# PraveenVora/pinot

Hardware: AMD Instinct MI355X
Metric: rows/sec scanned + %HBM roofline, filter+GROUP BY SUM at 1/2/4/8 GPUs (higher is better)
Workload: dtype int64; 1 GPU; adanalytics_readme_query; rows_per_gpu=1000000000, segments_per_gpu=100, parallelism=segment-sharded dp1, RCCL reduce of partial aggregates, groups=8, matched_docs_rank0=118

## Files before the change

include/pinot_amd.h:

```cpp
#ifndef PINOT_AMD_H_
#define PINOT_AMD_H_

#include <stdint.h>

#ifdef __cplusplus
extern "C" {
#endif

#define PA_ABI_VERSION 5

#define PA_MAX_LEAVES 16
#define PA_MAX_OPS 48
#define PA_MAX_GROUP_BY 8
#define PA_MAX_AGGS 16

#define PA_OK 0
#define PA_EINVAL (-1)
#define PA_EHIP (-2)
#define PA_ENOMEM (-3)
#define PA_EUNSUPPORTED (-4)

#define PA_INT 0
#define PA_LONG 1
#define PA_FLOAT 2
// ... 75 lines not shown
  int64_t group_by_cardinality[PA_MAX_GROUP_BY];
  int32_t num_aggs;
  pa_agg_spec aggs[PA_MAX_AGGS];
  int32_t flags;
  int32_t num_groups_limit;
  int64_t hash_keys_bound;
  int32_t flags2;
  int32_t reserved2;
} pa_query_spec;

#define PA_QF_STAGE_ALL 1
#define PA_QF_FORCE_GLOBAL 2
#define PA_QF_STEPS16 (1 << 4)
#define PA_QF_STEPS32 (1 << 5)
#define PA_QF_NO_LAZY (1 << 6)
#define PA_QF_FORCE_LDS (1 << 7)
#define PA_QF_RING_SHIFT 8
#define PA_QF_WG_SHIFT 12
#define PA_QF_NO_GDENSE_LM (1 << 15)
#define PA_QF_NO_JIT (1u << 31)
#define PA_QF_GD_DRAIN_EACH_TILE (1 << 2)
#define PA_QF_NO_GD_PACK (1 << 3)
#define PA_QF_DEBUG_STREAM_ONLY (1 << 16)
#define PA_QF_NO_LANE_MAJOR (1 << 17)
#define PA_QF_NO_REG_STAGE (1 << 18)
#define PA_QF_NO_BOX_FILTER (1 << 19)
#define PA_QF_BOX_FILTER (1 << 20)
#define PA_QF_NO_PARTITION (1 << 21)
#define PA_QF_NO_SPLIT_EMIT (1 << 24)
#define PA_QF_NO_LIMIT_WALK (1 << 25)
#define PA_QF_NO_LANE_ACC (1 << 26)
#define PA_QF_NO_LANE_HIST (1 << 27)
#define PA_QF_LAZY_POST (1 << 28)
#define PA_QF_NO_DENSE_GROUP (1 << 29)
#define PA_QF_NO_FILTER_STATS (1 << 30)
#define PA_QF2_NO_COUNT_FREE 1
#define PA_QF_PART_SHIFT 22

typedef struct {
  int32_t lo, hi;
  int32_t negate;
  int32_t reserved;
  const uint32_t* lut;
  int64_t ilo, ihi;
  double dlo, dhi;
  const void* values;
  int64_t num_values;
} pa_leaf_params;

typedef struct pa_query pa_query;

pa_query* pa_query_create(const pa_query_spec* spec, int32_t num_segments);

int pa_query_bind_segment(pa_query* q, int32_t index, const pa_segment* seg,
                          const pa_leaf_params* leaf_params, const int32_t* const* group_remaps);

int pa_query_bind_value_remap(pa_query* q, int32_t index, int32_t agg, const int32_t* remap);

int pa_query_set_tuning(pa_query* q, const char* name, int32_t value);
int32_t pa_query_results_invalid(const pa_query* q);

int pa_query_prepare(pa_query* q);

int64_t pa_query_num_keys(const pa_query* q);

int pa_query_execute(pa_query* q, void* stream);
int pa_query_reset(pa_query* q, void* stream);
int pa_query_scan(pa_query* q, void* stream);

#define PA_ACC_COUNT_U64 0
#define PA_ACC_SUM_I64 1
#define PA_ACC_SUM_F64 2
#define PA_ACC_MIN_I64 3
#define PA_ACC_MAX_I64 4
#define PA_ACC_HLL_U8 5
#define PA_ACC_SUM_I64X2 6
#define PA_ACC_DOCS_U64 7
#define PA_ACC_KEYS_I64 8
#define PA_ACC_PRESENCE_U8 9
#define PA_ACC_HIST_U64 10
uint64_t pa_query_accumulator_bytes(const pa_query* q);
int pa_query_set_accumulator_buffer(pa_query* q, void* device_buffer, uint64_t bytes);
int32_t pa_query_num_sections(const pa_query* q);
void* pa_query_section(const pa_query* q, int32_t section, int32_t* kind, int64_t* num_elements);

int64_t pa_query_fetch(pa_query* q, void* stream, int64_t capacity, int64_t* out_keys,
                       int64_t* out_counts, void* const* out_aggs);

int64_t pa_query_fetch_histogram(pa_query* q, void* stream, int32_t agg, int64_t num_groups, int64_t capacity,
                                 int64_t* out_row_ends, int32_t* out_value_ids, int64_t* out_value_counts);

#define PA_MAX_PERCENTILES 64
int pa_query_percentiles(pa_query* q, void* stream, int32_t agg, int64_t num_groups, int32_t num_percentiles,
                         const double* percentiles, int32_t* out_value_ids);

int64_t pa_query_matched_docs(const pa_query* q);

int32_t pa_query_limit_trimming(const pa_query* q);
int64_t pa_query_num_groups_limit_reached(const pa_query* q);

int64_t pa_query_leaf_bitmap_words(const pa_query* q, int32_t segment);
int pa_query_leaf_bitmaps(pa_query* q, int32_t segment, uint32_t* device_out, void* stream);

#define PA_BIT_AND (-1)
#define PA_BIT_OR (-2)
#define PA_BIT_NOT (-3)
#define PA_BIT_PROG_MAX 64
int64_t pa_bitmap_counts_scratch_bytes(int64_t words);
int pa_bitmap_counts(const uint32_t* device_bitmaps, int64_t words, int32_t num_leaves, int64_t num_docs,
                     const int32_t* prog_a, int32_t len_a, const int32_t* prog_b, int32_t len_b, void* device_scratch,
                     int64_t* device_out, void* stream);
int pa_query_filter_counts(pa_query* q, int32_t num_requests, const int32_t* segments, const int32_t* programs,
                           const int32_t* lengths, int64_t* out, void* stream);
int32_t pa_query_leap_leaf(const pa_query* q);
int pa_query_leap_counts(pa_query* q, int64_t* out, void* stream);

#define PA_FOP_EMPTY 0
#define PA_FOP_MATCH_ALL 1
#define PA_FOP_SORTED 2
#define PA_FOP_BITMAP 3
#define PA_FOP_SCAN 4
#define PA_FOP_AND 5
#define PA_FOP_OR 6
#define PA_FOP_NOT 7
#define PA_STATS_NON_SCAN (-1)
#define PA_STATS_HOST (-2)
typedef struct {
  int32_t kind;
  int32_t num_children;
  int32_t mv_column;
  int32_t prog_len;
  int32_t prog[PA_BIT_PROG_MAX];
} pa_filter_op;
int pa_query_execution_stats(pa_query* q, int32_t num_ops, const pa_filter_op* ops, int32_t num_trees,
                             const int32_t* tree_root, const int32_t* segment_tree, int32_t projected_columns,
                             int64_t docs_scanned, int64_t* out, int64_t* segment_in_filter, void* stream);

int64_t pa_query_row_bytes(const pa_query* q);
int pa_query_pack_rows(pa_query* q, int32_t world, void* device_rows, int64_t* counts, void* stream);
int pa_query_merge_rows(pa_query* q, const void* device_rows, int64_t num_rows, int64_t* groups, int64_t* overflow,
                        void* stream);

int pa_query_key_layout(const pa_query* q, int32_t* hashed, int32_t* shifts);
int32_t pa_query_key_words(const pa_query* q);

int pa_query_stats(const pa_query* q, uint64_t* staged_bytes, uint64_t* num_docs,
                   uint64_t* num_tiles);

int32_t pa_query_column_staged(const pa_query* q, int32_t column_id);
int32_t pa_query_num_eager_literals(const pa_query* q);
int32_t pa_query_lane_major(const pa_query* q);
int32_t pa_query_dense_packed(const pa_query* q);
int32_t pa_query_count_free_emit(const pa_query* q);
int32_t pa_query_partition_keys(const pa_query* q);
int pa_query_plan(const pa_query* q, int32_t* strategy, int32_t* steps, int32_t* dma_slots, int32_t* ring,
                  int32_t* wg_per_cu, int32_t* grid, int32_t* lds_bytes);

void pa_query_destroy(pa_query* q);

#ifdef __cplusplus
}
#endif

#endif
```

pinot_amd/_lib.py:

```python
import ctypes
import os

HERE = os.path.dirname(os.path.abspath(__file__))
LIB_PATH = os.path.join(HERE, "libpinot_amd.so")

PA_MAX_LEAVES = 16
PA_MAX_OPS = 48
PA_MAX_GROUP_BY = 8
PA_MAX_AGGS = 16

PA_INT, PA_LONG, PA_FLOAT, PA_DOUBLE, PA_STRING, PA_BYTES = range(6)
PA_LEAF_DICT_RANGE, PA_LEAF_DICT_SET, PA_LEAF_RAW_RANGE, PA_LEAF_MV_DICT_RANGE, PA_LEAF_MV_DICT_SET, PA_LEAF_RAW_SET = range(6)
PA_OP_LEAF, PA_OP_AND, PA_OP_OR, PA_OP_NOT = range(4)
PA_AGG_COUNT, PA_AGG_SUM, PA_AGG_MIN, PA_AGG_MAX, PA_AGG_DISTINCTCOUNTHLL, PA_AGG_COUNT_MV, PA_AGG_DISTINCTCOUNT, \
    PA_AGG_VALUE_HISTOGRAM = range(8)
PA_QF_STAGE_ALL = 1
PA_QF_FORCE_GLOBAL = 2
PA_QF_STEPS16 = 1 << 4
PA_QF_STEPS32 = 1 << 5
PA_QF_NO_LAZY = 1 << 6
PA_QF_FORCE_LDS = 1 << 7
PA_QF_RING_SHIFT = 8
PA_QF_WG_SHIFT = 12
PA_QF_DEBUG_STREAM_ONLY = 1 << 16
PA_QF_NO_LANE_MAJOR = 1 << 17
PA_QF_NO_REG_STAGE = 1 << 18
PA_QF_NO_GDENSE_LM = 1 << 15
PA_QF_NO_GD_PACK = 1 << 3
PA_QF_GD_DRAIN_EACH_TILE = 1 << 2
PA_QF_NO_JIT = 1 << 31
PA_QF_NO_BOX_FILTER = 1 << 19
PA_QF_BOX_FILTER = 1 << 20
PA_QF_NO_PARTITION = 1 << 21
PA_QF_PART_SHIFT = 22
PA_QF_NO_SPLIT_EMIT = 1 << 24
PA_QF_NO_LIMIT_WALK = 1 << 25
PA_QF_NO_LANE_ACC = 1 << 26
PA_QF_NO_LANE_HIST = 1 << 27
PA_QF_LAZY_POST = 1 << 28
PA_QF_NO_DENSE_GROUP = 1 << 29
PA_QF_NO_FILTER_STATS = 1 << 30
PA_QF2_NO_COUNT_FREE = 1 << 32
PA_FOP_EMPTY, PA_FOP_MATCH_ALL, PA_FOP_SORTED, PA_FOP_BITMAP, PA_FOP_SCAN, PA_FOP_AND, PA_FOP_OR, PA_FOP_NOT = range(8)
PA_STATS_NON_SCAN, PA_STATS_HOST = -1, -2
PA_BIT_AND, PA_BIT_OR, PA_BIT_NOT = -1, -2, -3
PA_BIT_PROG_MAX = 64
PA_ACC_COUNT_U64, PA_ACC_SUM_I64, PA_ACC_SUM_F64, PA_ACC_MIN_I64, PA_ACC_MAX_I64, PA_ACC_HLL_U8, \
    PA_ACC_SUM_I64X2, PA_ACC_DOCS_U64, PA_ACC_KEYS_I64, PA_ACC_PRESENCE_U8, PA_ACC_HIST_U64 = range(11)
PA_MAX_PERCENTILES = 64
ABI_VERSION = 5

EXPORTED = [
    "pa_abi_version", "pa_device_count", "pa_set_device", "pa_last_error", "pa_host_alloc", "pa_host_free",
    "pa_segment_create", "pa_segment_add_sv_dict_column", "pa_segment_add_mv_dict_column",
    "pa_segment_add_raw_column", "pa_segment_num_docs", "pa_segment_device_bytes", "pa_segment_destroy",
    "pa_query_create", "pa_query_set_tuning", "pa_query_results_invalid", "pa_query_bind_segment",
    "pa_query_bind_value_remap", "pa_query_prepare", "pa_query_num_keys",
    "pa_query_execute", "pa_query_reset", "pa_query_scan", "pa_query_num_eager_literals", "pa_query_lane_major",
    "pa_query_dense_packed", "pa_query_count_free_emit", "pa_query_partition_keys",
    "pa_query_accumulator_bytes", "pa_query_set_accumulator_buffer", "pa_query_num_sections", "pa_query_section",
    "pa_query_fetch", "pa_query_fetch_histogram", "pa_query_percentiles", "pa_query_matched_docs", "pa_query_key_layout", "pa_query_limit_trimming",
    "pa_query_num_groups_limit_reached", "pa_query_stats", "pa_query_leaf_bitmap_words", "pa_query_leaf_bitmaps",
    "pa_bitmap_counts_scratch_bytes", "pa_bitmap_counts", "pa_query_filter_counts",
    "pa_query_plan", "pa_query_column_staged", "pa_query_leap_leaf", "pa_query_leap_counts",
    "pa_query_execution_stats",
    "pa_query_row_bytes", "pa_query_pack_rows", "pa_query_merge_rows", "pa_query_key_words", "pa_query_destroy",
]


class PinotAmdError(RuntimeError):
    pass


class LeafSpec(ctypes.Structure):
    _fields_ = [("column_id", ctypes.c_int32), ("kind", ctypes.c_int32)]


class AggSpec(ctypes.Structure):
    _fields_ = [("type", ctypes.c_int32), ("column_id", ctypes.c_int32), ("log2m", ctypes.c_int32),
                ("flags", ctypes.c_int32), ("num_values", ctypes.c_int64)]


PA_AGGF_WIDE_SUM = 1


class QuerySpec(ctypes.Structure):
    _fields_ = [
        ("num_leaves", ctypes.c_int32),
        ("leaves", LeafSpec * PA_MAX_LEAVES),
        ("num_ops", ctypes.c_int32),
        ("ops", ctypes.c_int32 * PA_MAX_OPS),
        ("num_group_by", ctypes.c_int32),
        ("group_by_columns", ctypes.c_int32 * PA_MAX_GROUP_BY),
        ("group_by_cardinality", ctypes.c_int64 * PA_MAX_GROUP_BY),
        ("num_aggs", ctypes.c_int32),
        ("aggs", AggSpec * PA_MAX_AGGS),
        ("flags", ctypes.c_int32),
        ("num_groups_limit", ctypes.c_int32),
        ("hash_keys_bound", ctypes.c_int64),
        ("flags2", ctypes.c_int32),
        ("reserved2", ctypes.c_int32),
    ]


class LeafParams(ctypes.Structure):
    _fields_ = [
        ("lo", ctypes.c_int32), ("hi", ctypes.c_int32), ("negate", ctypes.c_int32), ("reserved", ctypes.c_int32),
        ("lut", ctypes.POINTER(ctypes.c_uint32)),
        ("ilo", ctypes.c_int64), ("ihi", ctypes.c_int64),
        ("dlo", ctypes.c_double), ("dhi", ctypes.c_double),
        ("values", ctypes.c_void_p), ("num_values", ctypes.c_int64),
    ]


_lib = None


def _declare(lib):
    vp, i32, i64, u64 = ctypes.c_void_p, ctypes.c_int32, ctypes.c_int64, ctypes.c_uint64
    sig = {
        "pa_abi_version": (ctypes.c_int, []),
        "pa_device_count": (ctypes.c_int, []),
        "pa_set_device": (ctypes.c_int, [ctypes.c_int]),
        "pa_last_error": (ctypes.c_char_p, []),
        "pa_host_alloc": (vp, [u64]),
        "pa_host_free": (None, [vp]),
        "pa_segment_create": (vp, [i32]),
        "pa_segment_add_sv_dict_column": (ctypes.c_int, [vp, i32, vp, u64, i32, i32, i32, vp, vp]),
        "pa_segment_add_mv_dict_column": (ctypes.c_int, [vp, i32, vp, u64, i32, i32, i64, i32, vp, vp]),
        "pa_segment_add_raw_column": (ctypes.c_int, [vp, i32, i32, vp]),
        "pa_segment_num_docs": (i32, [vp]),
        "pa_segment_device_bytes": (u64, [vp]),
        "pa_segment_destroy": (None, [vp]),
        "pa_query_create": (vp, [ctypes.POINTER(QuerySpec), i32]),
        "pa_query_set_tuning": (ctypes.c_int, [vp, ctypes.c_char_p, i32]),
        "pa_query_results_invalid": (i32, [vp]),
        "pa_query_bind_segment": (ctypes.c_int, [vp, i32, vp, ctypes.POINTER(LeafParams), vp]),
        "pa_query_bind_value_remap": (ctypes.c_int, [vp, i32, i32, vp]),
        "pa_query_prepare": (ctypes.c_int, [vp]),
        "pa_query_num_keys": (i64, [vp]),
        "pa_query_execute": (ctypes.c_int, [vp, vp]),
        "pa_query_reset": (ctypes.c_int, [vp, vp]),
        "pa_query_scan": (ctypes.c_int, [vp, vp]),
        "pa_query_num_eager_literals": (i32, [vp]),
        "pa_query_lane_major": (i32, [vp]),
        "pa_query_dense_packed": (i32, [vp]),
        "pa_query_count_free_emit": (i32, [vp]),
        "pa_query_partition_keys": (i32, [vp]),
        "pa_query_accumulator_bytes": (u64, [vp]),
        "pa_query_set_accumulator_buffer": (ctypes.c_int, [vp, vp, u64]),
        "pa_query_num_sections": (i32, [vp]),
        "pa_query_section": (vp, [vp, i32, ctypes.POINTER(i32), ctypes.POINTER(i64)]),
        "pa_query_fetch": (i64, [vp, vp, i64, vp, vp, vp]),
        "pa_query_fetch_histogram": (i64, [vp, vp, i32, i64, i64, vp, vp, vp]),
        "pa_query_percentiles": (ctypes.c_int, [vp, vp, i32, i64, i32, vp, vp]),
        "pa_query_matched_docs": (i64, [vp]),
        "pa_query_key_layout": (ctypes.c_int, [vp, ctypes.POINTER(i32), ctypes.POINTER(i32)]),
        "pa_query_limit_trimming": (i32, [vp]),
        "pa_query_num_groups_limit_reached": (ctypes.c_int64, [vp]),
        "pa_query_stats": (ctypes.c_int, [vp, ctypes.POINTER(u64), ctypes.POINTER(u64), ctypes.POINTER(u64)]),
        "pa_query_leaf_bitmap_words": (ctypes.c_int64, [vp, i32]),
        "pa_query_leaf_bitmaps": (ctypes.c_int, [vp, i32, vp, vp]),
        "pa_bitmap_counts_scratch_bytes": (i64, [i64]),
        "pa_bitmap_counts": (ctypes.c_int, [vp, i64, i32, i64, vp, i32, vp, i32, vp, vp, vp]),
        "pa_query_filter_counts": (ctypes.c_int, [vp, i32, vp, vp, vp, vp, vp]),
        "pa_query_plan": (ctypes.c_int, [vp] + [ctypes.POINTER(i32)] * 7),
        "pa_query_column_staged": (i32, [vp, i32]),
        "pa_query_leap_leaf": (i32, [vp]),
        "pa_query_leap_counts": (ctypes.c_int, [vp, vp, vp]),
        "pa_query_execution_stats": (ctypes.c_int, [vp, i32, vp, i32, vp, vp, i32, i64, vp, vp, vp]),
        "pa_query_row_bytes": (i64, [vp]),
        "pa_query_key_words": (i32, [vp]),
        "pa_query_pack_rows": (ctypes.c_int, [vp, i32, vp, vp, vp]),
        "pa_query_merge_rows": (ctypes.c_int, [vp, vp, i64, vp, vp, vp]),
        "pa_query_destroy": (None, [vp]),
    }
    for name, (res, args) in sig.items():
        f = getattr(lib, name)
        f.restype = res
        f.argtypes = args


def lib():
    global _lib
    if _lib is None:
        if not os.path.exists(LIB_PATH):
            raise PinotAmdError("%s is missing: run `python -m pinot_amd.build` (hipcc, gfx950)" % LIB_PATH)
        _lib = ctypes.CDLL(LIB_PATH)
        _declare(_lib)
        if _lib.pa_abi_version() != ABI_VERSION:
            raise PinotAmdError("ABI version mismatch: %s is stale, rebuild it" % LIB_PATH)
    return _lib


def check(rc, what=""):
    if rc < 0:
        raise PinotAmdError("%s failed (%d): %s" % (what, rc, lib().pa_last_error().decode(errors="replace")))
    return rc


def check_ptr(p, what=""):
    if not p:
        raise PinotAmdError("%s failed: %s" % (what, lib().pa_last_error().decode(errors="replace")))
    return p
```

pinot_amd/csrc/pa_capi.hip:

```cpp
#include "pa_host.h"

extern "C" {

pa_query* pa_query_create(const pa_query_spec* spec, int32_t num_segments) {
  if (!spec || num_segments < 0) {
    fail(PA_EINVAL, "bad query spec");
    return nullptr;
  }
  if (spec->num_leaves < 0 || spec->num_leaves > PA_MAX_LEAVES || spec->num_ops < 0 || spec->num_ops > PA_MAX_OPS ||
      spec->num_group_by < 0 || spec->num_group_by > PA_MAX_GROUP_BY || spec->num_aggs < 0 ||
      spec->num_aggs > PA_MAX_AGGS) {
    fail(PA_EINVAL, "query spec counts out of range");
    return nullptr;
  }
  pa_query* q = new pa_query();
  q->spec = *spec;
  q->nseg = num_segments;
  q->segs.assign(num_segments, nullptr);
  q->leaf_params.resize(num_segments);
  q->luts.resize(num_segments);
  q->remaps.resize(num_segments);
  q->has_remap.resize(num_segments);
  q->vremaps.assign(num_segments, std::vector<std::vector<int32_t>>(spec->num_aggs));
  return q;
}

int pa_query_set_tuning(pa_query* q, const char* name, int32_t value) {
  if (!q) return fail(PA_EINVAL, "null query");
  if (q->prepared) return fail(PA_EINVAL, "query already prepared");
  const TuningDef* d = tuning_named(name);
  if (!d) return fail(PA_EINVAL, std::string("unknown tuning: ") + (name ? name : "(null)"));
  if (value != d->def && (value < d->lo || value > d->hi))
    return fail(PA_EINVAL, std::string("tuning ") + d->name + ": " + std::to_string(value) + " outside " +
                               std::to_string(d->lo) + ".." + std::to_string(d->hi));
  q->tune.*d->value = value;
  return PA_OK;
}

int32_t pa_query_results_invalid(const pa_query* q) { return q ? (tuning_invalidating(q->tune) ? 1 : 0) : -1; }

int pa_query_bind_segment(pa_query* q, int32_t index, const pa_segment* seg, const pa_leaf_params* leaf_params,
                          const int32_t* const* group_remaps) {
  if (!q || !seg || index < 0 || index >= q->nseg) return fail(PA_EINVAL, "bad bind arguments");
  if (q->prepared) return fail(PA_EINVAL, "query already prepared");
  const pa_query_spec& s = q->spec;
  q->segs[index] = seg;
  q->leaf_params[index].assign(leaf_params, leaf_params + s.num_leaves);
  q->luts[index].assign(s.num_leaves, {});
  for (int l = 0; l < s.num_leaves; ++l) {
    const int kind = s.leaves[l].kind;
    if (kind == PA_LEAF_DICT_SET || kind == PA_LEAF_MV_DICT_SET) {
      auto it = seg->cols.find(s.leaves[l].column_id);
      if (it == seg->cols.end()) return fail(PA_EINVAL, "leaf column missing in segment");
      if (!leaf_params[l].lut) return fail(PA_EINVAL, "DICT_SET leaf without lut");
      const size_t words = ((size_t)it->second->cardinality + 31) / 32;
      q->luts[index][l].assign(leaf_params[l].lut, leaf_params[l].lut + words);
    } else if (kind == PA_LEAF_RAW_SET) {
      auto it = seg->cols.find(s.leaves[l].column_id);
      if (it == seg->cols.end()) return fail(PA_EINVAL, "leaf column missing in segment");
      const int64_t n = leaf_params[l].num_values;
      if (n < 0 || n > (int64_t(1) << 30) || (n > 0 && !leaf_params[l].values))
        return fail(PA_EINVAL, "RAW_SET leaf: bad value list");
      const bool integral = it->second->vtype == PA_INT || it->second->vtype == PA_LONG;
      const int64_t* vi = (const int64_t*)leaf_params[l].values;
      const double* vd = (const double*)leaf_params[l].values;
      for (int64_t i = 1; i < n; ++i)
        if (integral ? !(vi[i - 1] < vi[i]) : !(vd[i - 1] < vd[i]))
          return fail(PA_EINVAL, "RAW_SET leaf: values must be strictly ascending");
      const uint32_t* w = (const uint32_t*)leaf_params[l].values;
      q->luts[index][l].assign(w, w + 2 * n);
    }
  }
  q->remaps[index].assign(s.num_group_by, {});
  q->has_remap[index].assign(s.num_group_by, 0);
  for (int j = 0; j < s.num_group_by; ++j) {
    if (group_remaps && group_remaps[j]) {
      auto it = seg->cols.find(s.group_by_columns[j]);
      if (it == seg->cols.end()) return fail(PA_EINVAL, "group-by column missing in segment");
      const int32_t card = it->second->cardinality;
      q->remaps[index][j].assign(group_remaps[j], group_remaps[j] + card);
      for (int32_t v : q->remaps[index][j])
        if (v < 0 || v >= s.group_by_cardinality[j]) return fail(PA_EINVAL, "group remap id outside the key space");
      q->has_remap[index][j] = 1;
    }
  }
  return PA_OK;
}

int pa_query_bind_value_remap(pa_query* q, int32_t index, int32_t agg, const int32_t* remap) {
  if (!q || index < 0 || index >= q->nseg || agg < 0 || agg >= q->spec.num_aggs) return fail(PA_EINVAL, "bad remap arguments");
  if (q->prepared) return fail(PA_EINVAL, "query already prepared");
  if (!q->segs[index]) return fail(PA_EINVAL, "bind the segment before its value remaps");
  const pa_agg_spec& A = q->spec.aggs[agg];
  if (!value_id_agg(A.type))
    return fail(PA_EINVAL, "value remaps belong to DISTINCTCOUNT and VALUE_HISTOGRAM aggregations");
  auto it = q->segs[index]->cols.find(A.column_id);
  if (it == q->segs[index]->cols.end()) return fail(PA_EINVAL, "aggregation column missing in segment");
  q->vremaps[index][agg].clear();
  if (!remap) return PA_OK;
  const int32_t card = it->second->cardinality;
  q->vremaps[index][agg].assign(remap, remap + card);
  for (int32_t v : q->vremaps[index][agg])
    if (v < 0 || v >= A.num_values) return fail(PA_EINVAL, "value remap id outside the table-wide value dictionary");
  return PA_OK;
}

int pa_query_prepare(pa_query* q) {
  if (!q) return fail(PA_EINVAL, "null query");
  if (q->prepared) return PA_OK;
  for (int i = 0; i < q->nseg; ++i)
    if (!q->segs[i]) return fail(PA_EINVAL, "segment " + std::to_string(i) + " not bound");
  Prep P;
  std::memset(&q->hq, 0, sizeof(q->hq));
  int rc = plan_filter(q, P);
  if (!rc) rc = plan_slots(q, P);
  if (!rc) rc = plan_key_space(q, P);
  if (!rc) rc = plan_limit(q, P);
  if (!rc) rc = plan_gdense(q, P);
  if (!rc) rc = build_segments(q, P);
  if (!rc) rc = plan_walk(q, P);
  if (!rc) rc = plan_accumulators(q, P);
  TilePlan plan, count_plan;
  if (!rc) rc = plan_kernels(q, P, plan, count_plan);
  if (rc) return rc;

  void* dummy = nullptr;
  {
    std::vector<char> z(256, 0);
    rc = upload_owned(q, z.data(), z.size(), &dummy);
    if (rc) return rc;
  }
  const int nslots = (int)q->slot_cols.size();
  int64_t total_tiles = 0;
  apply_layout(q->hsegs, plan.steps, nslots, (int)q->literals.size(), dummy, &q->staged_bytes, &total_tiles);
  q->num_tiles = (uint64_t)total_tiles;
  q->lane_major = P.lm ? 1 : 0;
  q->dense_packed = P.gd_packed ? 1 : 0;
  q->plan_ring = plan.ring;
  q->plan_wg = plan.wg_per_cu;
  fill_devquery(q, P, plan, total_tiles);
  rc = plan_leaps(q, P);
  if (rc) return rc;

  int dev = 0, cus = 256;
  if (hipGetDevice(&dev) == hipSuccess) {
    hipDeviceProp_t prop;
    if (hipGetDeviceProperties(&prop, dev) == hipSuccess && prop.multiProcessorCount > 0) cus = prop.multiProcessorCount;
  }
  const int wg_cu = q->split_emit ? std::min(plan.wg_per_cu, q->emit_h_wg) : plan.wg_per_cu;
  const int64_t max_wg = (int64_t)cus * std::max(1, wg_cu);
  const int wpw = q->partitioned ? scan_waves(q->emit_strat) : scan_waves(q->strategy);
  const int64_t want = (total_tiles + wpw - 1) / wpw;
  q->grid = (int)std::max<int64_t>(1, std::min(max_wg, want));

  if (q->partitioned) {
    int64_t ct = 0;
    apply_layout(q->hsegs_count, plan.steps, nslots, (int)q->literals.size(), dummy, nullptr, &ct);
    if (ct != total_tiles) return fail(PA_EINVAL, "internal: count pass tiles differ");
    DevQuery& c = q->hq_count;
    c = q->hq;
    c.strategy = q->count_strat;
    c.count_skip_gb = q->count_skip;
    c.image_dwords_max = count_plan.img_dw;
    c.ring = count_plan.ring;
    c.dma_per_tile = count_plan.dma;
    c.num_staged = 0;
    for (int sl = 0; sl < nslots; ++sl) {
      bool st = false;
      for (const DevSeg& d : q->hsegs_count) st |= d.cols[sl].lds_off >= 0;
      if (st) c.staged_slots[c.num_staged++] = sl;
    }
    c.lds_acc_bytes = (uint32_t)(((size_t)q->hq.num_parts * 4 + 15) & ~(size_t)15);
    q->count_lds = (int)count_plan.lds;
    q->count_ring = count_plan.ring;
    q->count_k = std::max(1, count_plan.wg_per_cu / std::max(1, wg_cu));
    while (q->count_k > 1 && (int64_t)q->grid * q->count_k * kWavesPerWG > total_tiles) --q->count_k;
    q->hq.lds_acc_bytes = (uint32_t)(plan.lds - (size_t)wpw * plan.ring * plan.img_dw * 4);
    if (q->split_emit) {
      DevQuery& e = q->hq_h;
      e = q->hq;
      e.strategy = STRAT_PEMIT;
      e.ring = q->emit_h_ring;
      e.lds_acc_bytes = (uint32_t)((size_t)q->emit_h_lds -
                                   (size_t)scan_waves(q->emit_h_strat) * q->emit_h_ring * plan.img_dw * 4);
      e.part_lo = q->hq.pv;
      e.part_hi = q->hq.num_parts;
    }
    rc = plan_scratch(q, P);
    if (rc) return rc;
  }
  if (q->limit_mode) {
    rc = plan_limit_buffers(q, P, cus, total_tiles);
    if (rc) return rc;
  }
  rc = alloc_leaps(q, P);
  if (rc) return rc;
  rc = upload_descriptors(q);
  if (rc) return rc;
  rc = jit_plan(q, P, cus);
  if (rc) return rc;
  rc = pve_plan(q, P, cus);
  if (rc) return rc;
  PA_HIP(hipDeviceSynchronize());
  q->prepared = true;
  return PA_OK;
}

int64_t pa_query_num_keys(const pa_query* q) { return q ? q->num_keys : -1; }

int pa_query_reset(pa_query* q, void* stream) {
  if (!q || !q->prepared) return fail(PA_EINVAL, "query not prepared");
  hipStream_t st = (hipStream_t)stream;
  PA_HIP(hipMemsetAsync(q->external_acc ? q->external_acc : q->acc.p, 0, q->acc.n, st));
  if (q->hq.leap_mode) PA_HIP(hipMemsetAsync(q->leap_buf.p, 0, leap_header_bytes(q), st));
  for (const Section& sc : q->sections) {
    if (sc.kind == PA_ACC_MIN_I64 || sc.kind == PA_ACC_KEYS_I64) PA_HIP(launch_fill_i64((int64_t*)sc.ptr, sc.n, INT64_MAX, st));
    else if (sc.kind == PA_ACC_MAX_I64) PA_HIP(launch_fill_i64((int64_t*)sc.ptr, sc.n, INT64_MIN, st));
  }
  return PA_OK;
}

int pa_query_scan(pa_query* q, void* stream) {
  if (!q || !q->prepared) return fail(PA_EINVAL, "query not prepared");
  q->scanned_since_fetch = true;
  if (q->num_tiles == 0) return PA_OK;
  hipStream_t st = (hipStream_t)stream;
  if (q->limit_walk) {
    if (q->walk_words > kWalkMaxWords) PA_HIP(hipMemsetAsync(q->lim_admit.p, 0, q->lim_admit.n, st));
    PA_HIP(launch_limit_walk((const DevQuery*)q->dq.p, (const DevSeg*)q->dsegs.p, q->nseg, q->walk_words,
                             q->hq.gb_mv >= 0, q->tune.walk_tab != 0, st));
  }
  if (q->limit_mode) {
    const DevQuery* dq = (const DevQuery*)q->dq.p;
    const DevSeg* ds = (const DevSeg*)q->dsegs.p;
    const LimitDesc& F = q->limit;
    const int64_t H = F.fmask + 1;
    PA_HIP(launch_fill_i64((int64_t*)F.fkeys, H, INT64_MAX, st));
    PA_HIP(launch_fill_i64((int64_t*)F.fpos, H, -1, st));
    PA_HIP(launch_fill_i64((int64_t*)F.thresh, std::max(1, q->nseg), -1, st));
    PA_HIP(launch_fill_i64((int64_t*)F.hist, std::max(1, q->nseg) * 128, 0, st));
    PA_HIP(launch_limit_passes(dq, ds, F, q->limit_grid, 0, st));
    PA_HIP(launch_limit_passes(dq, ds, F, q->limit_grid, 1, st));
    PA_HIP(launch_limit_passes(dq, ds, F, q->limit_grid, 2, st));
    return PA_OK;
  }
  if (q->pve.fn) {
    if (q->part_vk == kVkGeneric) return fail(PA_EINVAL, "internal: chunk lists need a specialised pass C");
    PartScratch ps{};
    char* vb = (char*)q->pve.buf.p;
    ps.base = (uint64_t*)(vb + q->pve.o_base);
    for (pa_query::PveStream* S : {&q->pve, &q->pvh}) {
      if (!S->fn) continue;
      void* pa = S->args.p;
      void* psg = S->segs.p;
      void* params[] = {&pa, &psg};
      PA_HIP(hipModuleLaunchKernel(S->fn, S->grid, 1, 1, S->waves * kWave, 1, 1, S->lds, st, params, nullptr));
      char* b = (char*)S->buf.p;
      uint64_t* base = S == &q->pve ? ps.base : ps.base + q->hq.pv + 1;
      PA_HIP(launch_pve_lists((const uint32_t*)(b + S->o_hist), (uint32_t*)(b + S->o_off), base,
                              (const uint32_t*)(b + S->o_table), (const uint32_t*)(b + S->o_used),
                              (uint32_t*)(b + S->o_index), (uint32_t*)(b + S->o_tot), S->grid, S->parts, S->chunks,
                              S->cr, st));
      if (S == &q->pve) {
        ps.recs_v = (uint32_t*)b;
        ps.chunk_index = (const uint32_t*)(b + S->o_index);
        ps.chunk_shift = __builtin_ctz((unsigned)S->cr);
        ps.chunk_bin_shift = S->bin_shift;
      } else {
        ps.recs_h = (uint32_t*)b;
        ps.chunk_index_h = (const uint32_t*)(b + S->o_index);
        ps.chunk_shift_h = __builtin_ctz((unsigned)S->cr);
        ps.chunk_bin_shift_h = S->bin_shift;
      }
    }
    PA_HIP(launch_part_agg(q->part_vk, (const DevQuery*)q->dq.p, ps, q->pvh.fn ? q->hq.num_parts : q->hq.pv,
                           q->hq.pv, q->hq.v_fmt <= V_FMT_ID, q->tune.passc_v16, q->part_lds_c, st));
    return PA_OK;
  }
  if (q->partitioned) {
    ScratchArena* a = arena_for(q->scratch_dev);
    std::lock_guard<std::mutex> g(a->mu);
    int rc = arena_grow(a, q->sc_bytes);
    if (rc) return rc;
    if (a->used && a->last_stream != st) PA_HIP(hipStreamWaitEvent(st, a->last, 0));
    const PartScratch ps = scratch_of(q, a->p);
    const LmSegPlan* plans = (const LmSegPlan*)q->dplans.p;
    PA_HIP(launch_scan(q->count_strat, q->steps, 0, q->grid * q->count_k, q->count_lds, (const DevQuery*)q->dq_count.p,
                       (const DevSeg*)q->dsegs_count.p, plans, ps, st));
    PA_HIP(launch_part_offsets(&q->hq, ps, q->grid, q->count_k, st));
    PA_HIP(launch_scan(q->emit_strat, q->steps, 0, q->grid, q->lds_bytes, (const DevQuery*)q->dq.p,
                       (const DevSeg*)q->dsegs.p, plans, ps, st));
    if (q->split_emit)
      PA_HIP(launch_scan(q->emit_h_strat, q->steps, 0, q->grid, q->emit_h_lds, (const DevQuery*)q->dq_h.p,
                         (const DevSeg*)q->dsegs.p, plans, ps, st));
    PA_HIP(launch_part_agg(q->part_vk, (const DevQuery*)q->dq.p, ps, q->hq.num_parts, q->hq.pv, q->hq.v_fmt <= V_FMT_ID,
                           q->tune.passc_v16, q->part_lds_c, st));
    PA_HIP(hipEventRecord(a->last, st));
    a->last_stream = st;
    a->used = true;
    return PA_OK;
  }
  if (q->jit_fn) {
    void* pa = q->jit_args.p;
    void* ps = q->jit_segs.p;
    void* params[] = {&pa, &ps};
    PA_HIP(hipModuleLaunchKernel(q->jit_fn, q->jit_grid, 1, 1, q->jit_waves * kWave, 1, 1, q->jit_lds, st, params,
                                 nullptr));
    return PA_OK;
  }
  PartScratch none{};
  PA_HIP(launch_scan(q->strategy, q->steps, q->lane_major, q->grid, q->lds_bytes, (const DevQuery*)q->dq.p,
                     (const DevSeg*)q->dsegs.p, (const LmSegPlan*)q->dplans.p, none, st));
  q->leap_searched = false;
  return PA_OK;
}

int pa_query_execute(pa_query* q, void* stream) {
  const int rc = pa_query_reset(q, stream);
  return rc ? rc : pa_query_scan(q, stream);
}

uint64_t pa_query_accumulator_bytes(const pa_query* q) { return q ? (uint64_t)q->acc.n : 0; }

int pa_query_set_accumulator_buffer(pa_query* q, void* device_buffer, uint64_t bytes) {
  if (!q || !q->prepared) return fail(PA_EINVAL, "query not prepared");
  if (!device_buffer || bytes < q->acc.n) return fail(PA_EINVAL, "accumulator buffer too small");
  if (((uintptr_t)device_buffer & 255) != 0) return fail(PA_EINVAL, "accumulator buffer must be 256-byte aligned");
  char* old = (char*)(q->external_acc ? q->external_acc : q->acc.p);
  char* nb = (char*)device_buffer;
  for (Section& s : q->sections) s.ptr = nb + ((char*)s.ptr - old);
  auto relocate = [&](DevQuery& h) {
    h.count = (unsigned long long*)(nb + ((char*)h.count - old));
    h.matched_docs = (unsigned long long*)(nb + ((char*)h.matched_docs - old));
    if (q->hashed) h.ht_keys = (long long*)(nb + ((char*)h.ht_keys - old));
    for (int a = 0; a < h.num_aggs; ++a) {
      if (q->agg_section[a] < 0) continue;
      void* p = q->sections[q->agg_section[a]].ptr;
      h.aggs[a].acc_i64 = (int64_t*)p;
      h.aggs[a].acc_f64 = (double*)p;
      h.aggs[a].acc_hll = (uint8_t*)p;
    }
  };
  relocate(q->hq);
  if (q->limit_mode) q->limit.reached = q->hq.matched_docs + 2;
  PA_HIP(hipMemcpy(q->dq.p, &q->hq, sizeof(DevQuery), hipMemcpyHostToDevice));
  if (q->jit_fn) {
    JitArgs a;
    PA_HIP(hipMemcpy(&a, q->jit_args.p, sizeof(a), hipMemcpyDeviceToHost));
    jit_fill_pointers(q, a);
    PA_HIP(hipMemcpy(q->jit_args.p, &a, sizeof(a), hipMemcpyHostToDevice));
  }
  for (pa_query::PveStream* S : {&q->pve, &q->pvh}) {
    if (!S->fn) continue;
    PveArgs a;
    PA_HIP(hipMemcpy(&a, S->args.p, sizeof(a), hipMemcpyDeviceToHost));
    pve_fill_pointers(*S, q->hq.matched_docs, a);
    PA_HIP(hipMemcpy(S->args.p, &a, sizeof(a), hipMemcpyHostToDevice));
  }
  if (q->partitioned) {
    relocate(q->hq_count);
    PA_HIP(hipMemcpy(q->dq_count.p, &q->hq_count, sizeof(DevQuery), hipMemcpyHostToDevice));
    if (q->split_emit) {
      relocate(q->hq_h);
      PA_HIP(hipMemcpy(q->dq_h.p, &q->hq_h, sizeof(DevQuery), hipMemcpyHostToDevice));
    }
  }
  if (!q->external_acc) {
    const size_t n = q->acc.n;
    dev_free(q->acc);
    q->acc.n = n;
  }
  q->external_acc = device_buffer;
  return PA_OK;
}

int32_t pa_query_num_sections(const pa_query* q) { return q ? (int32_t)q->sections.size() : -1; }

void* pa_query_section(const pa_query* q, int32_t section, int32_t* kind, int64_t* num_elements) {
  if (!q || section < 0 || section >= (int32_t)q->sections.size()) {
    fail(PA_EINVAL, "bad section");
    return nullptr;
  }
  if (kind) *kind = q->sections[section].kind;
  if (num_elements) *num_elements = q->sections[section].n;
  return q->sections[section].ptr;
}

int pa_query_stats(const pa_query* q, uint64_t* staged_bytes, uint64_t* num_docs, uint64_t* num_tiles) {
  if (!q) return fail(PA_EINVAL, "null query");
  if (staged_bytes) *staged_bytes = q->staged_bytes;
  if (num_docs) *num_docs = q->num_docs;
  if (num_tiles) *num_tiles = q->num_tiles;
  return PA_OK;
}

int pa_query_plan(const pa_query* q, int32_t* strategy, int32_t* steps, int32_t* dma_slots, int32_t* ring,
                  int32_t* wg_per_cu, int32_t* grid, int32_t* lds_bytes) {
  if (!q || !q->prepared) return fail(PA_EINVAL, "query not prepared");
  if (strategy)
    *strategy = q->jit_fn ? (q->jit_waves >= 16 ? STRAT_GDENSE_LM16 : STRAT_GDENSE_LM8)
                          : (q->partitioned ? STRAT_PEMIT : q->strategy);
  if (steps) *steps = q->steps;
  if (dma_slots) *dma_slots = q->dma_slots;
  if (ring) *ring = q->plan_ring;
  if (wg_per_cu) *wg_per_cu = q->plan_wg;
  if (grid) *grid = q->grid;
  if (lds_bytes) *lds_bytes = q->lds_bytes;
  return PA_OK;
}

int32_t pa_query_num_eager_literals(const pa_query* q) { return q && q->prepared ? q->num_eager : -1; }

int32_t pa_query_lane_major(const pa_query* q) { return q && q->prepared ? q->lane_major : -1; }
int32_t pa_query_count_free_emit(const pa_query* q) { return q && q->prepared ? (q->pve.fn ? (q->pvh.fn ? 2 : 1) : 0) : -1; }
int32_t pa_query_partition_keys(const pa_query* q) {
  if (!q || !q->prepared) return -1;
  if (!q->partitioned || q->hq.pv == 0) return 0;
  return q->hq.part_kr_v ? q->hq.part_kr_v : (int32_t)1 << q->hq.kshift_v;
}
int32_t pa_query_dense_packed(const pa_query* q) {
  return q && q->prepared ? (q->jit_fn ? 2 : (q->dense_packed ? 1 : 0)) : -1;
}

int32_t pa_query_column_staged(const pa_query* q, int32_t column_id) {
  if (!q || !q->prepared || q->nseg == 0) return -1;
  for (size_t sl = 0; sl < q->slot_cols.size(); ++sl)
    if (q->slot_cols[sl] == column_id) {
      if (q->jit_fn) return std::count(q->jit_cols.begin(), q->jit_cols.end(), (int)sl) ? 1 : 0;
      return q->hsegs[0].cols[sl].lds_off >= 0 ? 1 : 0;
    }
  return -1;
}

int64_t pa_query_matched_docs(const pa_query* q) { return q && q->prepared ? q->last_matched : -1; }

int32_t pa_query_limit_trimming(const pa_query* q) {
  return q && q->prepared ? (q->limit_mode ? 1 : (q->limit_walk ? 2 : 0)) : -1;
}

int64_t pa_query_num_groups_limit_reached(const pa_query* q) { return q && q->prepared ? q->last_reached : -1; }

int pa_query_key_layout(const pa_query* q, int32_t* hashed, int32_t* shifts) {
  if (!q || !q->prepared) return fail(PA_EINVAL, "query not prepared");
  if (hashed) *hashed = q->hashed ? 1 : 0;
  if (shifts)
    for (int j = 0; j < q->spec.num_group_by; ++j) shifts[j] = q->hashed ? q->key_shift[j] : 0;
  return PA_OK;
}

int32_t pa_query_key_words(const pa_query* q) { return q && q->prepared ? (q->hashed ? q->key_words : 1) : -1; }

void pa_query_destroy(pa_query* q) { delete q; }

}
```

pinot_amd/csrc/pa_device.h:

```cpp
#pragma once
#include <stdint.h>
#include "../../include/pinot_amd.h"

namespace pa {

constexpr int kWave = 64;
constexpr int kWavesPerWG = 4;
constexpr int kWGSize = kWave * kWavesPerWG;
constexpr int kSteps = 32;
constexpr int kWTileDocs = kWave * kSteps;
constexpr int kMaxSlots = 12;
constexpr int kGuardWords = 4;

enum ColKind : int32_t { COL_NONE = 0, COL_SV_DICT = 1, COL_SV_RAW = 2, COL_MV_DICT = 3 };
enum Strategy : int32_t {
  STRAT_LDS = 0, STRAT_GLOBAL = 1, STRAT_PEMIT = 2, STRAT_PCOUNT = 3, STRAT_LANE = 4,
  STRAT_LANE_CNT = 5, STRAT_LANE_RAW = 6, STRAT_LANE_DICT = 7, STRAT_GDENSE = 8, STRAT_GDENSE8 = 9,
  STRAT_GDENSE12 = 10,
  STRAT_GDENSE_RS12 = 11, STRAT_GDENSE_RS8 = 12,
  STRAT_PCOUNT_MV = 13,
  STRAT_GDENSE_LM8 = 14, STRAT_GDENSE_LM16 = 15
};
__host__ __device__ constexpr bool is_pcount(int s) { return s == STRAT_PCOUNT || s == STRAT_PCOUNT_MV; }
__host__ __device__ constexpr bool is_gdense(int s) {
// ... 153 lines not shown
  int32_t has_mv;
  int32_t xcd_major;
  unsigned long long* matched_docs;
  int32_t hashed;
  int32_t key_words;
  int32_t gb_word[PA_MAX_GROUP_BY];
  int64_t ht_mask;
  long long* ht_keys;
  int32_t num_parts;
  int32_t pv;
  int32_t kshift_v;
  int32_t kshift_h;
  int32_t part_kr_v;
  int32_t v_fmt;
  int32_t rec_words_v;
  int32_t bs_v, bs_h;
  int32_t h_first;
  int32_t hll_agg;
  int32_t emit_val_agg;
  int32_t gb_mv;
  int32_t count_skip_gb;
  int32_t part_lo, part_hi;
  int32_t debug_emit;
  uint32_t lds_cnt, lds_done, lds_front, lds_back, lds_start;
  uint32_t lds_slack, pad_slack;
  uint32_t lds_bins_v, lds_bins_h;
  const uint64_t* vdict;
  int32_t staged_slots[kMaxSlots];
  int32_t gb_slot[PA_MAX_GROUP_BY];
  int64_t gb_stride[PA_MAX_GROUP_BY];
  int64_t num_keys;
  int64_t total_wtiles;
  unsigned long long* count;
  uint32_t lds_count_off;
  uint32_t lds_acc_bytes;
  DevAgg aggs[PA_MAX_AGGS];
  int64_t num_groups_limit;
  int32_t vop_sum, vop_min, vop_max;
  int32_t v_id_order;
  int32_t v_affine, pad_affine;
  int64_t v_base, v_step;
  uint64_t v_maxabs;
  int32_t lds_raw_slot, pad_raw;
  int32_t gd_rp_log2;
  int32_t gd_nkeys;
  int32_t gd_lo[PA_MAX_GROUP_BY];
  int32_t gd_span[PA_MAX_GROUP_BY];
  int32_t gd_ls[PA_MAX_GROUP_BY];
  int32_t gd_tab[PA_MAX_GROUP_BY];
  int32_t gd_tab_n[PA_MAX_GROUP_BY];
  int32_t gd_tables;
  int32_t gd_pk_base;
  int32_t gd_lut[PA_MAX_LEAVES];
  int32_t gd_lut_words[PA_MAX_LEAVES];
  const uint32_t* gd_plans;
  int32_t leap_mode;
  int32_t leap_lds_cap;
  unsigned long long* leap_out;
  int64_t leap_cap;
  int64_t leap_slices;
};
constexpr int kGdMaxGb = 3;
constexpr int kGdMaxAgg = 6;
constexpr int kGdRs12MaxGb = 2, kGdRs12MaxAgg = 2;
constexpr int kGdPlanDw = 192;
struct GdSegPlan {
  int32_t ngb, nagg, rpl, pad;
  struct {
    int32_t reg, nbits;
    int32_t tab;
    int32_t lo, span, ls;
  } gb[kGdMaxGb];
  struct {
    int32_t vs, op;
    int32_t reg, nbits;
    int32_t acc, tab;
  } ag[kGdMaxAgg];
  int32_t box;
  int32_t pad1[5];
};
static_assert(sizeof(GdSegPlan) == 256, "one dword per lane");
constexpr int kGdBoxDword = 58;
constexpr int kGdRsMaxIns = 12;
struct GdRsPlan {
  int32_t ins, pad;
  struct {
    uint32_t src_lo, src_hi;
    uint32_t stride;
    uint32_t lanes;
    uint32_t dst;
  } in[kGdRsMaxIns];
  int32_t pad1[2];
};
static_assert(sizeof(GdRsPlan) == 256, "one dword per lane");
struct GdLmIssue {
  int32_t ncols;
  struct {
    uint32_t src_lo, src_hi;
    uint32_t stride;
    uint32_t chunks;
    uint32_t dst;
  } col[kMaxSlots];
  int32_t pad1[3];
};
static_assert(sizeof(GdLmIssue) == 256, "one dword per lane");

constexpr int kGdLmLeaves = 6;
constexpr int kGdlMaxCols = 6;
struct GdLmPlan {
  int32_t nleaves;
  int32_t num_docs;
  int32_t packed;
  int32_t pk_cnt;
  int32_t pk_drain;
  int32_t pk_base;
  int32_t pk_off[kGdMaxAgg];
  int32_t key_leaf;
  int32_t key_in_box;
  int32_t pad0[2];
  struct {
    uint32_t code;
    uint32_t region;
    uint32_t lo_t, hi_t;
    int32_t lut_lds;
    uint32_t lut_lo, lut_hi;
  } lf[kGdLmLeaves];
  int32_t pad1[6];
};
static_assert(sizeof(GdLmPlan) == 256, "one dword per lane");

constexpr int kVkGeneric = -1;
__host__ __device__ constexpr int vk_code(int sum_kind, bool mn, bool mx) { return sum_kind | (mn ? 4 : 0) | (mx ? 8 : 0); }

struct PartScratch {
  uint32_t* hist;
  uint32_t* off;
  uint64_t* base;
  uint32_t* recs_v;
  uint32_t* recs_h;
  const uint32_t* chunk_index;
  int32_t chunk_shift, chunk_bin_shift;
  const uint32_t* chunk_index_h;
  int32_t chunk_shift_h, chunk_bin_shift_h;
};

constexpr int kLmStaged = 4;
constexpr int kLmEager = 4;
struct LmSegPlan {
  int32_t nstaged;
  int32_t neager;
  int32_t num_docs;
  int32_t num_wtiles;
  uint32_t dummy_lo, dummy_hi;
  int32_t pad0[2];
  struct {
    uint32_t lo, hi;
    int32_t nbits;
    int32_t lds_off;
  } st[kLmStaged];
  struct {
    int32_t kind;
    int32_t nbits;
    int32_t lds_off;
    uint32_t lo, span;
    int32_t flags;
    uint32_t lut_lo, lut_hi;
  } lf[kLmEager];
  int32_t pad1[8];
};
static_assert(sizeof(LmSegPlan) == 256, "one dword per lane");

__host__ __device__ inline int64_t f64_order_encode(double d) {
  int64_t b = __builtin_bit_cast(int64_t, d);
  return b >= 0 ? b : (b ^ 0x7FFFFFFFFFFFFFFFLL);
}
__host__ __device__ inline double f64_order_decode(int64_t e) {
  int64_t b = e >= 0 ? e : (e ^ 0x7FFFFFFFFFFFFFFFLL);
  return __builtin_bit_cast(double, b);
}

__host__ __device__ inline int32_t murmur_hash_long(int64_t data) {
  const uint32_t m = 0x5bd1e995u;
  const int r = 24;
  uint32_t h = 0;
  uint32_t k = (uint32_t)data * m;
  k ^= k >> r;
  h ^= k * m;
  k = (uint32_t)(data >> 32) * m;
  k ^= k >> r;
  h *= m;
  h ^= k * m;
  h ^= h >> 13;
  h *= m;
  h ^= h >> 15;
  return (int32_t)h;
}

__host__ __device__ inline uint32_t hll_slot_rank(int32_t hashed, int32_t log2m) {
  uint32_t h = (uint32_t)hashed;
  uint32_t j = h >> (32 - log2m);
  uint32_t x = (h << log2m) | ((1u << (log2m - 1)) + 1u);
  uint32_t r = (uint32_t)__builtin_clz(x) + 1u;
  return (j << 8) | r;
}

}
```

pinot_amd/csrc/pa_host.h:

```cpp
#pragma once
#include <hip/hip_runtime.h>
#include <hip/hiprtc.h>

#include <algorithm>
#include <array>
#include <cstdio>
#include <cstdlib>
#include <cmath>
#include <cstring>
#include <functional>
#include <map>
#include <mutex>
#include <numeric>
#include <string>
#include <utility>
#include <vector>

#include "pa_device.h"
#include "pa_launch.h"
#include "pa_jit_abi.h"
#include "pa_tuning.h"

using namespace pa;


inline thread_local std::string g_err;

inline int fail(int code, const std::string& msg) {
  g_err = msg;
  return code;
}

enum { LOG_PLAN = 1, LOG_JIT = 2 };
inline bool log_on(int what) {
  static const int on = (std::getenv("PA_DEBUG_PLAN") ? LOG_PLAN : 0) | (std::getenv("PA_JIT_LOG") ? LOG_JIT : 0);
  return (on & what) != 0;
}
#define PLAN_LOG(...)                                  \
  do {                                                 \
    if (log_on(LOG_PLAN)) {                            \
      std::fprintf(stderr, "[pa plan] " __VA_ARGS__); \
      std::fputc('\n', stderr);                       \
    }                                                  \
  } while (0)

#define PA_HIP(call)                                                                  \
  do {                                                                                \
    hipError_t e_ = (call);                                                           \
    if (e_ != hipSuccess) return fail(PA_EHIP, std::string(#call ": ") + hipGetErrorString(e_)); \
  } while (0)

#define PA_HIP_NULL(call)                                                             \
  do {                                                                                \
    hipError_t e_ = (call);                                                           \
    if (e_ != hipSuccess) { fail(PA_EHIP, std::string(#call ": ") + hipGetErrorString(e_)); return nullptr; } \
  } while (0)

struct DevBuf {
  void* p = nullptr;
  size_t n = 0;
};

inline int dev_alloc(DevBuf& b, size_t bytes) {
  b.n = bytes;
  if (bytes == 0) bytes = 16;
  hipError_t e = hipMalloc(&b.p, bytes);
  if (e != hipSuccess) return fail(PA_ENOMEM, std::string("hipMalloc(") + std::to_string(bytes) + "): " + hipGetErrorString(e));
  return PA_OK;
}

inline void dev_free(DevBuf& b) {
  if (b.p) (void)hipFree(b.p);
  b.p = nullptr;
  b.n = 0;
}

inline int64_t wtiles_for(int64_t num_docs) { return (num_docs + kWTileDocs - 1) / kWTileDocs; }

struct Column {
  int32_t kind = COL_NONE;
  int32_t vtype = PA_INT;
  int32_t nbits = 0;
  int32_t cardinality = 0;
  int64_t total_values = 0;
  int32_t max_values = 1;
  bool fits_int32 = false;
  bool dict_sorted = false;
  std::vector<uint64_t> hvals;
  uint64_t dict_hash = 0;
  DevBuf words;
  DevBuf raw;
  DevBuf dict;
  DevBuf hashes;
  DevBuf mv_off;
  ~Column() {
    dev_free(mv_off);
    dev_free(words);
    dev_free(raw);
    dev_free(dict);
    dev_free(hashes);
  }
};


struct pa_segment {
  int32_t num_docs = 0;
  std::map<int32_t, Column*> cols;
  uint64_t bytes = 0;
  ~pa_segment() {
    for (auto& kv : cols) delete kv.second;
  }
};

inline int64_t value_order_key(uint64_t bits, int32_t vtype) {
  return (vtype == PA_FLOAT || vtype == PA_DOUBLE) ? f64_order_encode(__builtin_bit_cast(double, bits))
                                                    : (int64_t)bits;
}

struct Literal {
  int leaf;
  bool neg;
};
using Clause = std::vector<Literal>;

constexpr size_t kFetchWholeBlockBytes = 1 << 20;
constexpr size_t kPartLdsChoices[4] = {144 * 1024, 64 * 1024, 96 * 1024, 144 * 1024};
constexpr int64_t kMinParts = 256;
constexpr int64_t kMaxParts = 4096;
constexpr int64_t kDirectMaxKeys = int64_t(1) << 27;
constexpr uint64_t kMaxHashSlots = uint64_t(1) << 28;
constexpr uint64_t kWalkMaxBitmapBytes = uint64_t(4) << 30;
constexpr size_t kLdsBudget = 160 * 1024;

struct Section {
  int32_t kind;
  void* ptr;
  int64_t n;
};

struct ScratchArena {
  std::mutex mu;
  void* p = nullptr;
  size_t n = 0;
  hipEvent_t last = nullptr;
  hipStream_t last_stream = nullptr;
  bool used = false;
};

inline ScratchArena* arena_for(int dev) {
  static std::mutex m;
  static std::map<int, ScratchArena*> arenas;
  std::lock_guard<std::mutex> g(m);
  ScratchArena*& a = arenas[dev];
  if (!a) a = new ScratchArena();
  return a;
}

inline int arena_grow(ScratchArena* a, size_t bytes) {
  if (a->n >= bytes) return PA_OK;
  if (a->used) PA_HIP(hipEventSynchronize(a->last));
  if (a->p) PA_HIP(hipFree(a->p));
  a->p = nullptr;
  a->n = 0;
  hipError_t e = hipMalloc(&a->p, bytes);
  if (e != hipSuccess) {
    a->p = nullptr;
    return fail(PA_ENOMEM, "scratch arena hipMalloc(" + std::to_string(bytes) + "): " + hipGetErrorString(e));
  }
  a->n = bytes;
  if (!a->last) PA_HIP(hipEventCreateWithFlags(&a->last, hipEventDisableTiming));
  return PA_OK;
}

inline int64_t presence_stride(const pa_agg_spec& A) { return (A.num_values + 15) & ~int64_t(15); }
inline int64_t hist_stride(const pa_agg_spec& A) { return (A.num_values + 1) & ~int64_t(1); }
inline bool value_id_agg(int32_t type) { return type == PA_AGG_DISTINCTCOUNT || type == PA_AGG_VALUE_HISTOGRAM; }
inline size_t section_es(int32_t kind) { return (kind == PA_ACC_HLL_U8 || kind == PA_ACC_PRESENCE_U8) ? 1 : 8; }

struct pa_query {
  pa_query_spec spec;
  int32_t nseg = 0;
  std::vector<const pa_segment*> segs;
  std::vector<std::vector<pa_leaf_params>> leaf_params;
  std::vector<std::vector<std::vector<uint32_t>>> luts;
  std::vector<std::vector<std::vector<int32_t>>> remaps;
  std::vector<std::vector<char>> has_remap;
  std::vector<std::vector<std::vector<int32_t>>> vremaps;
  std::vector<std::vector<int32_t>> vremap_host;
  bool prepared = false;
  Tuning tune;

  std::vector<int32_t> slot_cols;
  std::vector<Literal> literals;
  std::vector<int> clause_end;
  int64_t num_keys = 1;
  int strategy = STRAT_GLOBAL;
  int grid = 0;
  int steps = 32;
  int dma_slots = 8;
  int num_eager = 0;
  int plan_ring = 2;
  int plan_wg = 1;
  int lds_bytes = 0;
  uint64_t staged_bytes = 0;
  uint64_t num_docs = 0;
  uint64_t num_tiles = 0;

  DevQuery hq;
  std::vector<DevSeg> hsegs;
  DevBuf dq, dsegs, dplans;
  void* host_acc = nullptr;
  DevBuf fetch_blocks, fetch_stage;
  void* fetch_host = nullptr;
  int lane_major = 0;
  int dense_packed = 0;
  hipFunction_t jit_fn = nullptr;
  int jit_waves = 0, jit_grid = 0, jit_lds = 0, jit_nd = 16, jit_nseg = 0, jit_classes = 0, jit_slots = 0;
  std::vector<int> jit_cols;
  DevBuf jit_args, jit_segs;
  struct PveStream {
    hipFunction_t fn = nullptr;
    int waves = 0, grid = 0, lds = 0, cr = 0, parts = 0, bin_shift = 5;
    int64_t chunks = 0;
    DevBuf args, segs, buf;
    size_t o_table = 0, o_hist = 0, o_used = 0, o_off = 0, o_base = 0, o_index = 0, o_tot = 0;
  } pve, pvh;
  int has_mv = 0;
  bool hashed = false;
  int key_words = 1;
  int64_t ht_slots = 0;
  int key_shift[PA_MAX_GROUP_BY] = {0};
  int keys_section = -1;
  bool partitioned = false;
  DevQuery hq_count;
  std::vector<DevSeg> hsegs_count;
  DevBuf dq_count, dsegs_count;
  int count_lds = 0, count_ring = 0, part_lds_c = 0;
  int part_vk = -1;
  int v_id_bits = 0;
  int emit_strat = 0;
  bool split_emit = false;
  DevQuery hq_h;
  DevBuf dq_h;
  int emit_h_strat = 0, emit_h_lds = 0, emit_h_ring = 0, emit_h_wg = 0;
  int count_k = 1;
  int count_skip = -1;
  int count_strat = STRAT_PCOUNT;
  size_t sc_hist = 0, sc_off = 0, sc_base = 0, sc_recs_v = 0, sc_recs_h = 0, sc_bytes = 0;
  int scratch_dev = 0;
  int64_t last_matched = -1;
  int64_t last_reached = -1;
  bool limit_mode = false;
  LimitDesc limit{};
  bool limit_walk = false;
  int64_t walk_words = 0;
  DevBuf lim_admit;
  int limit_grid = 0;
  DevBuf lim_keys, lim_pos, lim_hist, lim_sel, lim_thresh;
  DevBuf stat_buf;
  DevBuf hist_buf, hist_pairs;
  DevBuf merge_buf;
  DevBuf leap_buf;
  int leap_leaf = -1;
  bool leap_searched = true;
  bool scanned_since_fetch = false;
  int64_t leap_slices = 0;
  std::vector<LmSegPlan> hplans;
  std::vector<uint32_t> gdplans;
  DevBuf dgdplans;
  std::vector<DevBuf> owned;
  DevBuf acc;
  void* external_acc = nullptr;
  std::vector<Section> sections;
  std::vector<int> agg_section;

  ~pa_query() {
    dev_free(dq);
    dev_free(dsegs);
    dev_free(dplans);
    dev_free(dq_count);
    dev_free(dq_h);
    dev_free(dsegs_count);
    dev_free(lim_keys);
    dev_free(lim_pos);
    dev_free(lim_hist);
    dev_free(lim_sel);
    dev_free(lim_thresh);
    dev_free(stat_buf);
    dev_free(leap_buf);
    dev_free(merge_buf);
    dev_free(hist_buf);
    dev_free(hist_pairs);
    dev_free(lim_admit);
    dev_free(dgdplans);
    dev_free(jit_args);
    dev_free(jit_segs);
    for (PveStream* p : {&pve, &pvh}) {
      dev_free(p->args);
      dev_free(p->segs);
      dev_free(p->buf);
    }
    if (host_acc) (void)hipHostFree(host_acc);
    dev_free(fetch_blocks);
    dev_free(fetch_stage);
    if (fetch_host) (void)hipHostFree(fetch_host);
    dev_free(acc);
    for (auto& b : owned) dev_free(b);
  }
};

struct Prep {
  std::vector<char> clause_mv;
  double post_density = 1.0;
  double first_clause_sel = 1.0;
  bool has_filter = false;
  bool dense = true;
  bool stage_all = false, stage_post = false;
  std::vector<int> leaf_slot, gb_slot, agg_slot;
  std::vector<char> slot_eager, slot_post, slot_gb;
  std::vector<int64_t> stride;
  std::vector<int> gb_word;
  std::vector<char> gb_raw;
  uint64_t limit_pairs = 0;
  int limit_eb = 0;
  std::vector<char> limit_bind;
  std::vector<int> agg_src;
  std::vector<char> val_fast, agg_mv;
  bool gb_mv = false;
  bool lm = false;
  size_t lds_acc = 0;
  std::vector<size_t> agg_lds;
  bool gdense = false;
  std::vector<char> gd_stage_raw;
  size_t gd_lds = 0;
  int gd_rp_log2 = 0, gd_nkeys = 0, gd_tables = 0;
  bool gd_box = false;
  bool gd_box_ok = false;
  std::vector<int> gd_lut, gd_lut_words;
  int gd_lo[PA_MAX_GROUP_BY] = {0}, gd_span[PA_MAX_GROUP_BY] = {0}, gd_ls[PA_MAX_GROUP_BY] = {0};
  int gd_tab[PA_MAX_GROUP_BY] = {0}, gd_tab_n[PA_MAX_GROUP_BY] = {0};
  std::vector<int> gd_vs, gd_op, gd_acc, gd_tab_a, gd_tab_an;
  std::vector<int64_t> gd_base, gd_step;
  std::vector<std::vector<const void*>> gd_src;
  bool gd_pk_ok = false, gd_packed = false;
  int gd_pk_c = 0;
  std::vector<int> gd_pk_w;
  std::vector<char> gd_pk_t32u;
  std::vector<int64_t> gd_pk_base;
};

struct TilePlan {
  int steps = 0, dma = 0, ring = 0, wg_per_cu = 0, img_dw = 0;
  size_t lds = 0;
  double score = -1;
};

int upload_owned(pa_query* q, const void* host, size_t bytes, void** dev);
int mv_group_component(const pa_query* q);
int plan_filter(pa_query* q, Prep& P);
int plan_slots(pa_query* q, Prep& P);
int plan_key_space(pa_query* q, Prep& P);
int plan_limit(pa_query* q, Prep& P);
int plan_gdense(pa_query* q, Prep& P);
int build_segments(pa_query* q, Prep& P);
int plan_accumulators(pa_query* q, Prep& P);
bool affine_dictionary(const std::vector<uint64_t>& v, int32_t vtype, int64_t* base, int64_t* step);
void apply_layout(std::vector<DevSeg>& segs, int steps, int nslots, int nleaves, const void* dummy,
// ... 17 lines not shown
```

pinot_amd/csrc/pa_kernels.hip:

```cpp
#include "pa_scan.h"

namespace pa {


__device__ __forceinline__ bool doc_passes(const DevQuery* __restrict__ q, const DevSeg* __restrict__ seg, int64_t doc) {
  bool ok = true, any = false;
  for (int li = 0; li < q->num_leaves; ++li) {
    const DevLeaf& L = seg->leaves[li];
    if (ok && !any) any = leaf_match_doc(L, doc);
    if (L.clause_end) {
      ok = ok && any;
      any = false;
    }
  }
  return ok;
}

template <class F>
__device__ __forceinline__ void for_each_key(const DevQuery* __restrict__ q, const DevSeg* __restrict__ seg, int64_t doc,
                                             F&& f) {
  int64_t base[2] = {0, 0};
  int nmv = 0;
  int mv_gb[PA_MAX_GROUP_BY];
  int32_t mv_s[PA_MAX_GROUP_BY], mv_n[PA_MAX_GROUP_BY];
// ... 796 lines not shown

int64_t bit_count_blocks(int64_t num_docs) { return ((num_docs + 31) / 32 + kBitBlockWords - 1) / kBitBlockWords; }

int64_t bit_count_scratch_words(int64_t words) { return 10 * ((words + kBitBlockWords - 1) / kBitBlockWords); }

hipError_t launch_bit_counts_batch(const BitJob* jobs, int nj, int64_t total_blocks, bool any_b, int32_t* table,
                                   hipStream_t s) {
  if (nj == 0 || total_blocks == 0) return hipSuccess;
  if (total_blocks > INT32_MAX) return hipErrorInvalidValue;
  bit_block_table_kernel<<<nj, 256, 0, s>>>(jobs, table);
  if (any_b) {
    bit_last_batch_kernel<<<(int)total_blocks, 256, 0, s>>>(jobs, table);
    bit_carry_batch_kernel<<<nj, 1024, 0, s>>>(jobs);
  }
  bit_count_batch_kernel<<<(int)total_blocks, 256, 0, s>>>(jobs, table);
  bit_sum_batch_kernel<<<nj, 1024, 0, s>>>(jobs);
  return hipGetLastError();
}

constexpr int kLeafStepsPerWave = 128;
constexpr int kLeafBatch = 16;

__device__ __forceinline__ void leaf_bitmap_batch(const DevLeaf& L, int64_t n, int flip, uint32_t* out, int64_t s0,
                                                  int lane) {
  if (s0 * kWave >= n) return;
  if (L.kind == PA_LEAF_DICT_RANGE || L.kind == PA_LEAF_DICT_SET) {
    uint32_t id[kLeafBatch];
#pragma unroll
    for (int k = 0; k < kLeafBatch; ++k) id[k] = decode_global(L.words, (s0 + k) * kWave + lane, L.nbits);
    bool m[kLeafBatch];
    if (L.kind == PA_LEAF_DICT_RANGE) {
      const int sh = 32 - L.nbits;
      const uint32_t lo = (uint32_t)L.lo >> sh;
      const uint32_t span = (uint32_t)(((uint64_t)(uint32_t)L.span + 1u) >> sh);
#pragma unroll
      for (int k = 0; k < kLeafBatch; ++k) m[k] = (id[k] - lo) < span;
    } else {
#pragma unroll
      for (int k = 0; k < kLeafBatch; ++k) m[k] = (gp(L.lut)[id[k] >> 5] >> (id[k] & 31u)) & 1u;
    }
#pragma unroll
    for (int k = 0; k < kLeafBatch; ++k) {
      const int64_t st = s0 + k;
      const int64_t doc = st * kWave + lane;
      const uint64_t b = __ballot(doc < n && (m[k] != ((L.negate != 0) != (flip != 0))));
      if (st * kWave < n && lane < 2) gp(out)[2 * st + lane] = (uint32_t)(b >> (32 * lane));
    }
    return;
  }
  for (int k = 0; k < kLeafBatch; ++k) {
    const int64_t st = s0 + k;
    const int64_t doc = st * kWave + lane;
    if (st * kWave >= n) break;
    const bool m = doc < n && (leaf_match_doc(L, doc) != (flip != 0));
    const uint64_t b = __ballot(m);
    if (lane < 2) gp(out)[2 * st + lane] = (uint32_t)(b >> (32 * lane));
  }
}


constexpr int kLeafTilesPerWave = 4;

__device__ __forceinline__ void leaf_bitmap_tiles_lm(const DevLeaf& L, int64_t n, int flip, uint32_t* out,
                                                     int64_t t0, int lane, uint32_t* region) {
  const int nb = L.nbits;
  const uint32_t region_lds = lds_addr(region);
  for (int64_t t = t0; t < t0 + kLeafTilesPerWave; ++t) {
    const int64_t base = t * kWTileDocs;
    if (base >= n) return;
    const AS1 u32x4* src = (const AS1 u32x4*)(gp(L.words) + t * (int64_t)(kWave * nb));
    for (int c = lane; c < 16 * nb; c += kWave) ((lds_u32x4_t*)lds_ptr(region))[c] = src[c];
    asm volatile("s_waitcnt lgkmcnt(0)" ::: "memory");
    uint32_t bits = leaf_lm_any(nb, L.kind, region_lds, lane, (uint32_t)L.lo, (uint32_t)L.span, L.lut);
    if ((L.negate != 0) != (flip != 0)) bits = ~bits;
    const int64_t left = n - (base + 32 * lane);
    bits &= left >= 32 ? 0xffffffffu : (left <= 0 ? 0u : ((1u << left) - 1u));
    if (t * kWave + lane < (n + 127) / 128 * 4) gp(out)[t * kWave + lane] = bits;
    asm volatile("" ::: "memory");
  }
}

__global__ void __launch_bounds__(256) leaf_bitmaps_batch_kernel(const LeafJob* __restrict__ jobs, int nj) {
  __shared__ LeafJob SJ;
  __shared__ DevLeaf SL;
  __shared__ u32x4 regions[4][kWave * 32 / 4];
  if (threadIdx.x == 0) {
    int lo = 0, hi = nj - 1;
    while (lo < hi) {
      const int mid = (lo + hi + 1) >> 1;
      if (jobs[mid].first_block <= (int64_t)blockIdx.x) lo = mid;
      else hi = mid - 1;
    }
    SJ = jobs[lo];
  }
  __syncthreads();
  if (threadIdx.x < sizeof(DevLeaf) / 4)
    ((uint32_t*)&SL)[threadIdx.x] = gp((const uint32_t*)&SJ.seg->leaves[SJ.li])[threadIdx.x];
  __syncthreads();
  const DevLeaf L = SL;
  const int64_t n = SJ.num_docs;
  uint32_t* out = SJ.out;
  const int flip = SJ.flip;
  const int lane = threadIdx.x & 63;
  const int64_t blk = (int64_t)blockIdx.x - SJ.first_block;
  if (L.kind == PA_LEAF_DICT_RANGE || L.kind == PA_LEAF_DICT_SET) {
    leaf_bitmap_tiles_lm(L, n, flip, out, (blk * 4 + (threadIdx.x >> 6)) * kLeafTilesPerWave, lane,
                         (uint32_t*)regions[threadIdx.x >> 6]);
    return;
  }
  const int64_t sw = (blk * 4 + (threadIdx.x >> 6)) * kLeafStepsPerWave;
  for (int64_t s0 = sw; s0 < sw + kLeafStepsPerWave; s0 += kLeafBatch) leaf_bitmap_batch(L, n, flip, out, s0, lane);
}

static_assert(kLeafStepsPerWave * kWave == kLeafTilesPerWave * kWTileDocs, "one work split for both leaf paths");

int64_t leaf_bitmap_blocks(int64_t num_docs) {
  return ((num_docs + kWave - 1) / kWave + 4 * kLeafStepsPerWave - 1) / (4 * kLeafStepsPerWave);
}

hipError_t launch_leaf_bitmaps_batch(const LeafJob* jobs, int nj, int64_t total_blocks, hipStream_t s) {
  if (nj == 0 || total_blocks == 0) return hipSuccess;
  if (total_blocks > INT32_MAX) return hipErrorInvalidValue;
  leaf_bitmaps_batch_kernel<<<(int)total_blocks, 256, 0, s>>>(jobs, nj);
  return hipGetLastError();
}

__global__ void bswap_words_kernel(uint32_t* w, int64_t n) {
  for (int64_t i = blockIdx.x * (int64_t)blockDim.x + threadIdx.x; i < n; i += (int64_t)gridDim.x * blockDim.x)
    w[i] = __builtin_bswap32(w[i]);
}

__global__ void hll_lut_numeric_kernel(const int64_t* di, const double* dd, int32_t vtype, int32_t card,
                                       int32_t log2m, uint32_t* lut) {
  for (int i = blockIdx.x * blockDim.x + threadIdx.x; i < card; i += gridDim.x * blockDim.x) {
    int64_t x;
    switch (vtype) {
      case PA_INT: case PA_LONG: x = di[i]; break;
      case PA_FLOAT: x = __builtin_bit_cast(int32_t, (float)dd[i]); break;
      default: x = __builtin_bit_cast(int64_t, dd[i]); break;
    }
    lut[i] = hll_slot_rank(murmur_hash_long(x), log2m);
  }
}

__global__ void hll_lut_hashes_kernel(const int32_t* hashes, int32_t card, int32_t log2m, uint32_t* lut) {
  for (int i = blockIdx.x * blockDim.x + threadIdx.x; i < card; i += gridDim.x * blockDim.x)
    lut[i] = hll_slot_rank(hashes[i], log2m);
}

__global__ void fill_i64_kernel(int64_t* p, int64_t n, int64_t v) {
  for (int64_t i = blockIdx.x * (int64_t)blockDim.x + threadIdx.x; i < n; i += (int64_t)gridDim.x * blockDim.x) p[i] = v;
}

__global__ void gather_kernel(const void* src, int esize, int64_t per, const int64_t* keys, int64_t n, void* out) {
  const int64_t total = n * per;
  for (int64_t i = blockIdx.x * (int64_t)blockDim.x + threadIdx.x; i < total; i += (int64_t)gridDim.x * blockDim.x) {
    const int64_t r = i / per, j = i - r * per;
    const int64_t s = keys[r] * per + j;
    if (esize == 8) ((uint64_t*)out)[i] = ((const uint64_t*)src)[s];
    else ((uint32_t*)out)[i] = ((const uint32_t*)src)[s];
  }
}


constexpr int kCompactKeys = 2048;

__device__ __forceinline__ uint32_t block_exclusive_scan_256(uint32_t v, uint32_t* sh, uint32_t* total) {
  const int t = threadIdx.x;
  sh[t] = v;
  __syncthreads();
  for (int o = 1; o < 256; o <<= 1) {
    const uint32_t add = t >= o ? sh[t - o] : 0u;
    __syncthreads();
    sh[t] += add;
    __syncthreads();
  }
  const uint32_t incl = sh[t];
  if (total) *total = sh[255];
  __syncthreads();
  return incl - v;
}

__global__ void __launch_bounds__(256) compact_count_kernel(const unsigned long long* count, int64_t K, int all,
                                                            uint32_t* block_sums) {
  __shared__ uint32_t sh[256];
  const int64_t k0 = (int64_t)blockIdx.x * kCompactKeys + 8 * threadIdx.x;
  uint32_t c = 0;
  for (int j = 0; j < 8; ++j) c += (k0 + j < K) && (all || count[k0 + j] != 0);
  uint32_t total;
  block_exclusive_scan_256(c, sh, &total);
  if (threadIdx.x == 0) block_sums[blockIdx.x] = total;
}

__global__ void __launch_bounds__(256) compact_scan_kernel(uint32_t* v, int64_t n) {
  __shared__ uint32_t sh[256];
  uint32_t carry = 0;
  for (int64_t base = 0; base < n; base += 256) {
    const int64_t i = base + threadIdx.x;
    const uint32_t x = i < n ? v[i] : 0u;
    uint32_t tot;
    const uint32_t ex = block_exclusive_scan_256(x, sh, &tot);
    if (i < n) v[i] = carry + ex;
    carry += tot;
  }
  if (threadIdx.x == 0) v[n] = carry;
}

__global__ void __launch_bounds__(256) compact_gather_kernel(const unsigned long long* count, int64_t K, int all,
                                                             const uint32_t* block_off, int64_t cap,
                                                             CompactDesc d) {
  __shared__ uint32_t sh[256];
  const int64_t k0 = (int64_t)blockIdx.x * kCompactKeys + 8 * threadIdx.x;
  uint32_t c = 0;
  for (int j = 0; j < 8; ++j) c += (k0 + j < K) && (all || count[k0 + j] != 0);
  int64_t pos = (int64_t)block_off[blockIdx.x] + block_exclusive_scan_256(c, sh, nullptr);
  for (int j = 0; j < 8; ++j) {
    const int64_t k = k0 + j;
    if (k >= K || !(all || count[k] != 0)) continue;
    if (pos < cap) {
      d.keys[pos] = k;
      for (int si = 0; si < d.nsec; ++si) {
        const int64_t per = d.per[si];
        if (d.es[si] == 8) {
          const uint64_t* src = (const uint64_t*)d.src[si] + k * per;
          uint64_t* dst = (uint64_t*)d.dst[si] + pos * per;
          for (int64_t e = 0; e < per; ++e) dst[e] = src[e];
        } else if (d.es[si] == 1) {
          const u32x4* src = (const u32x4*)((const uint8_t*)d.src[si] + k * per);
          u32x4* dst = (u32x4*)((uint8_t*)d.dst[si] + pos * per);
          for (int64_t e = 0; e < per / 16; ++e) dst[e] = src[e];
        } else {
          const uint32_t* src = (const uint32_t*)d.src[si] + k * per;
          uint32_t* dst = (uint32_t*)d.dst[si] + pos * per;
          for (int64_t e = 0; e < per; ++e) dst[e] = src[e];
        }
      }
    }
    ++pos;
  }
}

__device__ double i128_to_double(int64_t hi, uint64_t lo) {
  const bool neg = hi < 0;
  uint64_t mh = (uint64_t)hi, ml = lo;
  if (neg) {
    ml = ~ml + 1ull;
    mh = ~mh + (ml == 0 ? 1ull : 0ull);
  }
  if (mh == 0 && ml < (1ull << 53)) return neg ? -(double)ml : (double)ml;
  const int msb = mh ? 127 - __builtin_clzll(mh) : 63 - __builtin_clzll(ml);
  const int s = msb - 52;
  auto bit = [&](int i) -> uint64_t { return i >= 64 ? (mh >> (i - 64)) & 1ull : (ml >> i) & 1ull; };
  uint64_t sig = s >= 64 ? mh >> (s - 64) : ((ml >> s) | (mh << (64 - s)));
  sig &= (1ull << 53) - 1ull;
  sig |= 1ull << 52;
  const uint64_t half = bit(s - 1);
  bool sticky;
  const int t = s - 1;
  if (t <= 0) sticky = false;
  else if (t >= 64) sticky = ml != 0 || (t > 64 && (mh & ((1ull << (t - 64)) - 1ull)) != 0);
  else sticky = (ml & ((1ull << t) - 1ull)) != 0;
  int e = s;
  if (half && (sticky || (sig & 1ull))) {
    ++sig;
    if (sig == (1ull << 53)) {
      sig >>= 1;
      ++e;
    }
  }
  const double d = ldexp((double)sig, e);
  return neg ? -d : d;
}

__global__ void __launch_bounds__(256) compact_final_kernel(const unsigned long long* count, int64_t K, int all,
                                                            const uint32_t* block_off, int64_t cap, FinalDesc d) {
  __shared__ uint32_t sh[256];
  __shared__ uint32_t pos[kCompactKeys];
  const int64_t kb = (int64_t)blockIdx.x * kCompactKeys;
  const int64_t k0 = kb + 8 * threadIdx.x;
  uint32_t c = 0;
  for (int j = 0; j < 8; ++j) c += (k0 + j < K) && (all || count[k0 + j] != 0);
  uint32_t p = block_exclusive_scan_256(c, sh, nullptr);
  for (int j = 0; j < 8; ++j) {
    const bool on = (k0 + j < K) && (all || count[k0 + j] != 0);
    pos[8 * threadIdx.x + j] = on ? p : 0xffffffffu;
    p += on ? 1u : 0u;
  }
  __syncthreads();
  const int64_t base = block_off[blockIdx.x];
  for (int j = 0; j < kCompactKeys / 256; ++j) {
    const int kl = threadIdx.x + 256 * j;
    const uint32_t pl = pos[kl];
    if (pl == 0xffffffffu) continue;
    const int64_t r = base + pl;
    if (r >= cap) continue;
    const int64_t k = kb + kl;
    const unsigned long long cnt = count[k];
    d.keys[r] = k;
    d.counts[r] = (int64_t)cnt;
    for (int a = 0; a < d.nagg; ++a) {
      const int t = d.type[a];
      if (t == PA_AGG_VALUE_HISTOGRAM) continue;
      if (t == PA_AGG_DISTINCTCOUNTHLL || t == PA_AGG_DISTINCTCOUNT) {
        const int64_t per = d.per[a];
        const u32x4* src = (const u32x4*)((const uint8_t*)d.sec[a] + k * per);
        u32x4* dst = (u32x4*)((uint8_t*)d.out[a] + r * per);
// ... 441 lines not shown
      pa[j] = ok[j] ? pi : 0ull;
    }
#pragma unroll
    for (int j = 0; j < kB; ++j) w[j] = __builtin_nontemporal_load(recs + pa[j]);
#pragma unroll
    for (int j = 0; j < kB; ++j)
      if (!ok[j]) w[j] = kSentinel;
    if (cix) cidv = load_cids(b0 + span);
    uint32_t rk[kB], sh[kB], old[kB];
    uint32_t* wp[kB];
#pragma unroll
    for (int j = 0; j < kB; ++j) {
      const bool ok = w[j] != kSentinel;
      const uint32_t lk = w[j] >> (lg + 6);
      rk[j] = ok ? (w[j] >> 1) & 31u : 0u;
      const uint32_t idx = (lk << lg) | ((w[j] >> 6) & rmask);
      wp[j] = regw + (rk[j] != 0 ? (idx >> 2) : 0u);
      sh[j] = (idx & 3u) * 8u;
      if (ok && first && (w[j] & 1u)) atomicAdd(cnt + lk, 1u);
    }
#pragma unroll
    for (int j = 0; j < kB; ++j) old[j] = rk[j] != 0 ? __hip_atomic_load(wp[j], WG_RLX) : 0u;
    bool done[kB];
#pragma unroll
    for (int j = 0; j < kB; ++j) {
      done[j] = ((old[j] >> sh[j]) & 0xffu) >= rk[j];
      if (!done[j]) {
        const uint32_t nw = (old[j] & ~(0xffu << sh[j])) | (rk[j] << sh[j]);
        done[j] = __hip_atomic_compare_exchange_strong(wp[j], &old[j], nw, __ATOMIC_RELAXED, __ATOMIC_RELAXED,
                                                       __HIP_MEMORY_SCOPE_WORKGROUP);
      }
    }
#pragma unroll
    for (int j = 0; j < kB; ++j) {
      if (done[j]) continue;
      uint32_t o = old[j];
      while (((o >> sh[j]) & 0xffu) < rk[j]) {
        const uint32_t nw = (o & ~(0xffu << sh[j])) | (rk[j] << sh[j]);
        if (__hip_atomic_compare_exchange_strong(wp[j], &o, nw, __ATOMIC_RELAXED, __ATOMIC_RELAXED,
                                                 __HIP_MEMORY_SCOPE_WORKGROUP))
          break;
      }
    }
  }
  __syncthreads();
  AS1 u32x4* g = (AS1 u32x4*)(H.acc_hll + ((size_t)kbase << lg));
  const u32x4* l = (const u32x4*)lds;
  for (int64_t i = threadIdx.x; i < (nk << lg) / 16; i += NT) g[i] = l[i];
  if (first)
    for (int64_t lk = threadIdx.x; lk < nk; lk += NT) gp(q->count)[kbase + lk] = cnt[lk];
}

template <int VK>
__global__ void __launch_bounds__(kPartAggThreads) part_agg_kernel(const DevQuery* __restrict__ q, PartScratch ps) {
  extern __shared__ __attribute__((aligned(16))) uint32_t smem[];
  if constexpr (VK == kVkGeneric) part_agg_v(q, ps, (int)blockIdx.x, (unsigned char*)smem);
  else part_agg_v_fast<VK>(q, ps, (int)blockIdx.x, (unsigned char*)smem);
}

constexpr int kPartAggHThreads = 1024;
__global__ void __launch_bounds__(kPartAggHThreads) part_agg_h_kernel(const DevQuery* __restrict__ q, PartScratch ps) {
  extern __shared__ __attribute__((aligned(16))) uint32_t smem[];
  part_agg_h<kPartAggHThreads, 16>(q, ps, (int)blockIdx.x, (unsigned char*)smem);
}
template <int VK>
__global__ void __launch_bounds__(kPartAggHThreads) part_agg_v16_kernel(const DevQuery* __restrict__ q, PartScratch ps) {
  extern __shared__ __attribute__((aligned(16))) uint32_t smem[];
  part_agg_v_fast<VK, kPartAggHThreads>(q, ps, (int)blockIdx.x, (unsigned char*)smem);
}
static const void* part_agg_v16_variant(int vk) {
  switch (vk) {
#define PA_VK(c) case c: return (const void*)part_agg_v16_kernel<c>;
    PA_VK(0) PA_VK(1) PA_VK(2) PA_VK(3) PA_VK(4) PA_VK(5) PA_VK(6) PA_VK(7)
    PA_VK(8) PA_VK(9) PA_VK(10) PA_VK(11) PA_VK(12) PA_VK(13) PA_VK(14) PA_VK(15)
#undef PA_VK
    default: return nullptr;
  }
}
template <int VK>
static const void* part_agg_fn() { return (const void*)part_agg_kernel<VK>; }
static const void* part_agg_variant(int vk) {
  switch (vk) {
#define PA_VK(c) case c: return part_agg_fn<c>();
    PA_VK(0) PA_VK(1) PA_VK(2) PA_VK(3) PA_VK(4) PA_VK(5) PA_VK(6) PA_VK(7)
    PA_VK(8) PA_VK(9) PA_VK(10) PA_VK(11) PA_VK(12) PA_VK(13) PA_VK(14) PA_VK(15)
#undef PA_VK
    default: return part_agg_fn<kVkGeneric>();
  }
}

hipError_t launch_part_offsets(const DevQuery* hq, const PartScratch& ps, int G, int k, hipStream_t s) {
  const int P = hq->num_parts, pv = hq->pv;
  part_scan_kernel<<<P, 256, 0, s>>>(ps.hist, ps.off, G, k, P, pv, (uint32_t)hq->bs_v, (uint32_t)hq->bs_h, ps.base);
  if (pv > 0) scan_u64_kernel<<<1, 256, 0, s>>>(ps.base, pv);
  if (P > pv) scan_u64_kernel<<<1, 256, 0, s>>>(ps.base + pv + 1, P - pv);
  return hipGetLastError();
}

hipError_t set_part_agg_lds_limit(int vk, int lds_bytes) {
  hipError_t e = hipFuncSetAttribute((const void*)part_agg_h_kernel, hipFuncAttributeMaxDynamicSharedMemorySize,
                                     lds_bytes);
  if (e != hipSuccess) return e;
  if (const void* f = part_agg_v16_variant(vk)) {
    e = hipFuncSetAttribute(f, hipFuncAttributeMaxDynamicSharedMemorySize, lds_bytes);
    if (e != hipSuccess) return e;
  }
  return hipFuncSetAttribute(part_agg_variant(vk), hipFuncAttributeMaxDynamicSharedMemorySize, lds_bytes);
}

hipError_t launch_part_agg(int vk, const DevQuery* q, const PartScratch& ps, int P, int pv, bool one_word,
                           int force_v16, int lds_bytes, hipStream_t s) {
  void* args[] = {(void*)&q, (void*)&ps};
  const bool v16 = (force_v16 < 0 ? one_word : force_v16 != 0) && part_agg_v16_variant(vk) != nullptr;
  if (pv > 0) {
    hipError_t e = v16 ? hipLaunchKernel(part_agg_v16_variant(vk), dim3(pv), dim3(kPartAggHThreads), args,
                                         (size_t)lds_bytes, s)
                       : hipLaunchKernel(part_agg_variant(vk), dim3(pv), dim3(kPartAggThreads), args, (size_t)lds_bytes, s);
    if (e != hipSuccess) return e;
  }
  if (pv >= P) return hipSuccess;
  return hipLaunchKernel((const void*)part_agg_h_kernel, dim3(P - pv), dim3(kPartAggHThreads), args, (size_t)lds_bytes,
                         s);
}

static int grid_for(int64_t n, int block) {
  int64_t g = (n + block - 1) / block;
  if (g < 1) g = 1;
  if (g > 4096) g = 4096;
  return (int)g;
}


hipError_t launch_bswap_words(uint32_t* w, int64_t n, hipStream_t s) {
  bswap_words_kernel<<<grid_for(n, 256), 256, 0, s>>>(w, n);
  return hipGetLastError();
}

hipError_t launch_hll_lut_numeric(const int64_t* di, const double* dd, int32_t vtype, int32_t card, int32_t log2m,
                                  uint32_t* lut, hipStream_t s) {
  hll_lut_numeric_kernel<<<grid_for(card, 256), 256, 0, s>>>(di, dd, vtype, card, log2m, lut);
  return hipGetLastError();
}

hipError_t launch_hll_lut_hashes(const int32_t* hashes, int32_t card, int32_t log2m, uint32_t* lut, hipStream_t s) {
  hll_lut_hashes_kernel<<<grid_for(card, 256), 256, 0, s>>>(hashes, card, log2m, lut);
  return hipGetLastError();
}

hipError_t launch_fill_i64(int64_t* p, int64_t n, int64_t v, hipStream_t s) {
  fill_i64_kernel<<<grid_for(n, 256), 256, 0, s>>>(p, n, v);
  return hipGetLastError();
}

hipError_t launch_gather(const void* src, int esize, int64_t per, const int64_t* keys, int64_t n, void* out,
                         hipStream_t s) {
  gather_kernel<<<grid_for(n * per, 256), 256, 0, s>>>(src, esize, per, keys, n, out);
  return hipGetLastError();
}

constexpr int kLeapThreads = 1024;

__global__ void __launch_bounds__(kLeapThreads) leap_search_kernel(const DevQuery* __restrict__ q,
                                                                   const DevSeg* __restrict__ segs) {
  extern __shared__ uint32_t pre[];
  __shared__ uint32_t part[kLeapThreads];
  const int t = threadIdx.x, lane = t & (kWave - 1);
  const int64_t nseg = q->num_segments, S = q->leap_slices, cap = q->leap_cap;
  const AS1 unsigned long long* hdr = gp(q->leap_out) + 3 * nseg;
  if (hdr[0]) return;
  const int64_t per = (S + kLeapThreads - 1) / kLeapThreads;
  const int64_t s0 = min(S, (int64_t)t * per), s1 = min(S, s0 + per);
  uint32_t sum = 0;
  for (int64_t w = s0; w < s1; ++w) sum += (uint32_t)hdr[1 + w];
  part[t] = sum;
  __syncthreads();
  for (int o = 1; o < kLeapThreads; o <<= 1) {
    const uint32_t v = t >= o ? part[t - o] : 0u;
    __syncthreads();
    part[t] += v;
    __syncthreads();
  }
  uint32_t run = part[t] - sum;
  for (int64_t w = s0; w < s1; ++w) {
    pre[w] = run;
    run += (uint32_t)hdr[1 + w];
  }
  if (t == kLeapThreads - 1) pre[S] = part[t];
  __syncthreads();
  const int64_t total = pre[S];
  const AS1 unsigned long long* lists = hdr + 1 + S;
  const int64_t waves = ((int64_t)gridDim.x * kLeapThreads) >> 6;
  for (int64_t g = (int64_t)blockIdx.x * (kLeapThreads >> 6) + (t >> 6); g < total + nseg; g += waves) {
    if (g < total) {
      int64_t lo = 0, hi = S;
      while (hi - lo > 1) {
        const int64_t mid = (lo + hi) >> 1;
        if ((int64_t)pre[mid] <= g) lo = mid;
        else hi = mid;
      }
      const uint64_t ent = lists[lo * cap + (g - (int64_t)pre[lo])];
      const int si = (int)(ent >> 40);
      const int64_t doc = (int64_t)((ent >> 1) & ((1ull << 39) - 1ull));
      uint32_t leaps = 0u, gave = 0u;
      const uint32_t succ = leap_search(segs + si, doc + 1, 1, lane);
      leaps += succ == 1u;
      gave |= succ == 4u;
      if (!(ent & 1ull)) {
        const uint32_t pred = leap_search(segs + si, doc - 1, -1, lane);
        leaps += pred == 1u;
        gave |= pred == 4u;
      }
      leap_add(q, si, 0u, leaps, gave, lane);
    } else {
      const int si = (int)(g - total);
      const uint32_t first = leap_search(segs + si, 0, 1, lane);
      leap_add(q, si, 0u, first == 1u ? 1u : 0u, first == 4u ? 1u : 0u, lane);
    }
  }
}

hipError_t launch_leap_search(const DevQuery* q, const DevSeg* segs, int64_t slices, hipStream_t s) {
  const size_t lds = (size_t)(slices + 1) * 4;
  hipError_t e = hipFuncSetAttribute((const void*)leap_search_kernel, hipFuncAttributeMaxDynamicSharedMemorySize, (int)lds);
  if (e != hipSuccess) return e;
  hipLaunchKernelGGL(leap_search_kernel, dim3(512), dim3(kLeapThreads), lds, s, q, segs);
  return hipGetLastError();
}

static const void* scan_fn(int strategy, int steps, int lm) {
  if (const void* f = scan_fn_std(strategy, steps, lm)) return f;
  if (const void* f = scan_fn_gdense(strategy, lm)) return f;
  if (const void* f = scan_fn_part_a(strategy)) return f;
  if (const void* f = scan_fn_part_mv(strategy)) return f;
  return scan_fn_part_b(strategy);
}

hipError_t set_scan_lds_limit(int strategy, int steps, int lm, int bytes) {
  return hipFuncSetAttribute(scan_fn(strategy, steps, lm), hipFuncAttributeMaxDynamicSharedMemorySize, bytes);
}

hipError_t scan_occupancy(int strategy, int steps, int lm, int lds_bytes, int* blocks_per_cu) {
  return hipOccupancyMaxActiveBlocksPerMultiprocessor(blocks_per_cu, scan_fn(strategy, steps, lm), scan_waves(strategy) * kWave,
                                                      (size_t)lds_bytes);
}

hipError_t launch_scan(int strategy, int steps, int lm, int grid, int lds_bytes, const DevQuery* q, const DevSeg* segs,
                       const LmSegPlan* plans, const PartScratch& ps, hipStream_t s) {
  PartScratch pcopy = ps;
  void* args[] = {(void*)&q, (void*)&segs, (void*)&plans, (void*)&pcopy};
  return hipLaunchKernel(scan_fn(strategy, steps, lm), dim3(grid), dim3(scan_waves(strategy) * kWave), args,
                         (size_t)lds_bytes, s);
}

}
```

pinot_amd/csrc/pa_launch.h:

```cpp
#pragma once
#include <hip/hip_runtime.h>
#include "pa_device.h"

namespace pa {
constexpr int kMaxCompactSections = PA_MAX_AGGS + 2;
struct CompactDesc {
  int32_t nsec;
  int32_t es[kMaxCompactSections];
  int64_t per[kMaxCompactSections];
  const void* src[kMaxCompactSections];
  void* dst[kMaxCompactSections];
  int64_t* keys;
};
struct FinalDesc {
  int32_t nagg;
  int32_t type[PA_MAX_AGGS];
  int32_t src[PA_MAX_AGGS];
  int64_t per[PA_MAX_AGGS];
  const void* sec[PA_MAX_AGGS];
  void* out[PA_MAX_AGGS];
  int64_t* keys;
  int64_t* counts;
};
hipError_t launch_compact_final(const unsigned long long* count, int64_t K, int all, const uint32_t* block_off,
                                int64_t cap, const FinalDesc* d, hipStream_t s);
hipError_t launch_leaf_bitmap(const DevSeg* seg, int li, int flip, int64_t num_docs, uint32_t* out, hipStream_t s);
constexpr int kBitProgMax = 64;
constexpr int kBitProgStack = 16;
constexpr int kBitGroups = 2;
struct BitJob {
  const uint32_t* bm;
  int64_t words, num_docs;
  int64_t first_block, nb;
  const int32_t* tok;
  int32_t len_a, len_b;
  int32_t nu, pad;
  int32_t uleaf[4];
  uint32_t* scratch;
  unsigned long long* part;
  unsigned long long* out;
};
struct LeafJob {
  const DevSeg* seg;
  uint32_t* out;
  int64_t num_docs, first_block;
  int32_t li, flip;
};
int64_t leaf_bitmap_blocks(int64_t num_docs);
int64_t bit_count_blocks(int64_t num_docs);
int64_t bit_count_scratch_words(int64_t words);
hipError_t launch_bit_counts_batch(const BitJob* jobs, int nj, int64_t total_blocks, bool any_b, int32_t* table,
                                   hipStream_t s);
hipError_t launch_leaf_bitmaps_batch(const LeafJob* jobs, int nj, int64_t total_blocks, hipStream_t s);
hipError_t launch_compact(const unsigned long long* count, int64_t K, int all, uint32_t* block_sums, int64_t cap,
                          const CompactDesc* d, int phase, hipStream_t s);
struct LimitDesc {
  long long* fkeys;
  unsigned long long* fpos;
  int64_t fmask;
  uint32_t* hist;
  unsigned long long* prefix;
  long long* rank;
  unsigned long long* thresh;
  unsigned long long* reached;
  int64_t limit;
  int32_t eb;
  int32_t pos_bits;
  int32_t nseg;
  int32_t pad;
};
hipError_t launch_limit_passes(const DevQuery* q, const DevSeg* segs, const LimitDesc& F, int grid, int phase,
                               hipStream_t s);
constexpr int64_t kWalkMaxWords = 40000;
hipError_t launch_limit_walk(const DevQuery* q, const DevSeg* segs, int nseg, int64_t words, bool mv, bool use_tab,
                             hipStream_t s);
hipError_t launch_bswap_words(uint32_t* w, int64_t n, hipStream_t s);
hipError_t launch_hll_lut_numeric(const int64_t* di, const double* dd, int32_t vtype, int32_t card, int32_t log2m,
                                  uint32_t* lut, hipStream_t s);
hipError_t launch_hll_lut_hashes(const int32_t* hashes, int32_t card, int32_t log2m, uint32_t* lut, hipStream_t s);
hipError_t launch_fill_i64(int64_t* p, int64_t n, int64_t v, hipStream_t s);
hipError_t launch_gather(const void* src, int esize, int64_t per, const int64_t* keys, int64_t n, void* out,
                         hipStream_t s);
hipError_t launch_part_offsets(const DevQuery* hq, const PartScratch& ps, int G, int k, hipStream_t s);
hipError_t set_part_agg_lds_limit(int vk, int lds_bytes);
hipError_t launch_part_agg(int vk, const DevQuery* q, const PartScratch& ps, int P, int pv, bool one_word,
                           int force_v16, int lds_bytes, hipStream_t s);
enum RowOp : int32_t { ROW_ADD_U64 = 0, ROW_ADD_F64 = 1, ROW_MIN_I64 = 2, ROW_MAX_I64 = 3, ROW_MAX_U8 = 4, ROW_KEY = 5 };
constexpr int kMaxRowSecs = PA_MAX_AGGS + 2;
struct RowSec {
  int32_t op;
  int32_t pad;
  int64_t slot_bytes;
  int64_t row_off;
  void* base;
};
struct RowDesc {
  int32_t nsec;
  int32_t key_words;
  int64_t row_bytes;
  int64_t num_slots;
  int64_t ht_mask;
  int64_t key_off;
  const unsigned long long* count;
  long long* keys;
  RowSec sec[kMaxRowSecs];
};
hipError_t launch_pack_index(const RowDesc& d, int world, int phase, unsigned long long* counts,
                             unsigned long long* cursor, int64_t* row_slot, hipStream_t s);
hipError_t launch_pack_copy(const RowDesc& d, const int64_t* row_slot, int64_t rows, unsigned char* out, hipStream_t s);
hipError_t launch_merge_rows(const RowDesc& d, const unsigned char* rows, int64_t n, int64_t* row_slot,
                             unsigned long long* counters, hipStream_t s);
hipError_t launch_leap_search(const DevQuery* q, const DevSeg* segs, int64_t slices, hipStream_t s);
constexpr int64_t kLeapMaxSlices = 16384;
constexpr int kStatMaskWordsPerThread = 4;
constexpr int kLfMaxK = 8;
constexpr int kLfMaxSub = 8;
constexpr int64_t kLfChunkDocs = 2048;
enum : int32_t { LF_DOCS = 0, LF_SCAN = 1, LF_OR = 2 };
struct StatMaskJob {
  const uint32_t* bm;
  uint32_t* out;
  int64_t words, num_docs, first_block;
  int32_t tok_off, len;
};
struct StatCountJob {
  const uint32_t* mask;
  const int32_t* wt;
  unsigned long long* out;
  int64_t words, first_block;
};
struct LfJob {
  int32_t K, nsub;
  int32_t kind[kLfMaxK];
  int32_t sub_first[kLfMaxK], sub_count[kLfMaxK];
  int32_t sub_kind[kLfMaxSub];
  int32_t cell_words, pad;
  const uint32_t* emask[kLfMaxK];
  const int32_t* ewt[kLfMaxK];
  const uint32_t* smask[kLfMaxSub];
  const int32_t* swt[kLfMaxSub];
  int64_t num_docs, nchunks, first_lane;
  uint32_t* cells;
  unsigned long long* out;
};
constexpr int kRpMaxNodes = 24;
constexpr int kRpMaxDepth = 6;
enum : int32_t { RP_EMPTY = 0, RP_ALL = 1, RP_DOCS = 2, RP_SCAN = 3, RP_AND = 4, RP_OR = 5, RP_NOT = 6 };
struct RpNode {
  int32_t kind, nchild, first, depth;
  const uint32_t* mask;
  const int32_t* wt;
};
struct RpJob {
  int64_t num_docs;
  int32_t nnodes, root;
  int32_t kids[kRpMaxNodes];
  RpNode node[kRpMaxNodes];
  unsigned long long* out;
};
hipError_t launch_stat_replay(const RpJob* jobs, int nj, hipStream_t s);
int64_t stat_mask_blocks(int64_t words);
hipError_t launch_stat_masks(const StatMaskJob* jobs, int nj, int64_t blocks, const int32_t* toks, hipStream_t s);
hipError_t launch_stat_counts(const StatCountJob* jobs, int nj, int64_t blocks, hipStream_t s);
hipError_t launch_leapfrogs(const LfJob* jobs, int nj, int64_t lanes, hipStream_t s);
hipError_t launch_pve_lists(const uint32_t* hist, uint32_t* off, uint64_t* base, const uint32_t* table,
                            const uint32_t* used, uint32_t* index, uint32_t* tot, int G, int P, int64_t C, int cr,
                            hipStream_t s);
hipError_t set_scan_lds_limit(int strategy, int steps, int lm, int bytes);
hipError_t scan_occupancy(int strategy, int steps, int lm, int lds_bytes, int* blocks_per_cu);
hipError_t launch_scan(int strategy, int steps, int lm, int grid, int lds_bytes, const DevQuery* q, const DevSeg* segs,
                       const LmSegPlan* plans, const PartScratch& ps, hipStream_t s);
}
```

pinot_amd/csrc/pa_plan_kernels.hip:

```cpp
#include "pa_host.h"


TilePlan plan_tiles(const pa_query* q, const std::vector<DevSeg>& segs, int strat, bool use_lm, size_t acc_b,
                    bool only16) {
  const int wpw = scan_waves(strat);
  const pa_query_spec& s = q->spec;
  const int force_ring = (s.flags >> PA_QF_RING_SHIFT) & 15;
  const int force_wg = (s.flags >> PA_QF_WG_SHIFT) & 7;
  TilePlan best;
  for (int steps : {32, 16}) {
    if (use_lm && steps != 32) continue;
    if (only16 && steps != 16) continue;
    if ((s.flags & PA_QF_STEPS16) && steps != 16) continue;
    if ((s.flags & PA_QF_STEPS32) && steps != 32) continue;
    int img_dw = kGuardWords, dma = 0;
    for (const DevSeg& d : segs) {
      int dw = kGuardWords, n = 0;
      for (int k = 0; k < d.num_staged; ++k) {
        const int nb = d.stage[k].nbits;
        dw += 2 * steps * nb + kGuardWords;
        n += ((steps / 2) * nb + 63) / 64;
      }
      img_dw = std::max(img_dw, dw);
      dma = std::max(dma, n);
    }
    const size_t img_bytes = (size_t)img_dw * 4;
    for (int wg : {4, 3, 2, 1}) {
      if (force_wg && wg != force_wg) continue;
      const size_t per_wg = kLdsBudget / wg;
      if (per_wg <= acc_b) continue;
      int ring = (int)((per_wg - acc_b) / (wpw * img_bytes));
      ring = std::min(ring, 8);
      if (force_ring) {
        if (force_ring > ring) continue;
        ring = force_ring;
      }
      if (ring < 2) continue;
      const size_t lds = acc_b + (size_t)wpw * ring * img_bytes;
      int resident = 0;
      if (set_scan_lds_limit(strat, steps, use_lm, (int)kLdsBudget) != hipSuccess ||
          scan_occupancy(strat, steps, use_lm, (int)lds, &resident) != hipSuccess)
        resident = wg;
      if (resident < wg) continue;
      const double inflight = (double)wg * wpw * (ring - 1) * img_bytes;
      const double score = 1e7 * wg * wpw / kWavesPerWG + (steps == 32 ? 1e6 : 0) + std::min(inflight, 128.0 * 1024);
      if (score > best.score) best = TilePlan{steps, dma, ring, wg, img_dw, lds, score};
    }
  }
  return best;
}

uint64_t max_abs_value(const std::vector<uint64_t>& v, int32_t vtype) {
  if (vtype != PA_INT && vtype != PA_LONG) return 0;
  uint64_t m = 0;
  for (uint64_t x : v) {
    const int64_t y = (int64_t)x;
    if (y == INT64_MIN) return 0;
    m = std::max<uint64_t>(m, (uint64_t)(y < 0 ? -y : y));
  }
  return m;
}

bool affine_dictionary(const std::vector<uint64_t>& v, int32_t vtype, int64_t* base, int64_t* step) {
  if (v.empty() || (vtype != PA_INT && vtype != PA_LONG)) return false;
  const int64_t b = (int64_t)v[0];
  const int64_t st = v.size() > 1 ? (int64_t)(v[1] - v[0]) : 0;
  for (size_t i = 1; i < v.size(); ++i)
    if ((uint64_t)v[i] - (uint64_t)v[i - 1] != (uint64_t)st) return false;
  *base = b;
  *step = st;
  return true;
}

int value_dictionary(pa_query* q, const Prep& P, int a, const uint64_t** vdict) {
  const pa_query_spec& s = q->spec;
  const int32_t cid = s.aggs[a].column_id;
  const Column* c0 = q->segs[0]->cols.at(cid);
  if (c0->kind != COL_SV_DICT || c0->hvals.empty()) return -1;
  bool same = true;
  for (int si = 0; si < q->nseg; ++si) {
    const Column* c = q->segs[si]->cols.at(cid);
    if (c->kind != COL_SV_DICT || c->hvals.empty() || c->vtype != c0->vtype) return -1;
    same = same && (c == c0 || (c->dict_hash == c0->dict_hash && c->hvals == c0->hvals));
  }
  for (int si = 0; si < q->nseg; ++si) q->hsegs[si].vremap = nullptr;
  q->vremap_host.assign(q->nseg, {});
  q->hq.v_affine = 0;
  q->hq.v_maxabs = 0;
  if (same) {
    *vdict = (const uint64_t*)c0->dict.p;
    q->hq.v_maxabs = max_abs_value(c0->hvals, c0->vtype);
    int64_t b = 0, st = 0;
    if (affine_dictionary(c0->hvals, c0->vtype, &b, &st)) {
      q->hq.v_affine = 1;
      q->hq.v_base = b;
      q->hq.v_step = st;
    }
    return std::max(1, 32 - __builtin_clz((uint32_t)std::max(1, c0->cardinality - 1)));
  }
  const int32_t vt = c0->vtype;
  std::vector<std::pair<int64_t, uint64_t>> all;
  for (int si = 0; si < q->nseg; ++si)
    for (uint64_t v : q->segs[si]->cols.at(cid)->hvals) all.push_back({value_order_key(v, vt), v});
  std::sort(all.begin(), all.end());
  all.erase(std::unique(all.begin(), all.end(), [](const auto& x, const auto& y) { return x.first == y.first; }),
            all.end());
  if (all.size() > (size_t)INT32_MAX) return -1;
  std::vector<uint64_t> uni(all.size());
  std::vector<int64_t> keys(all.size());
  for (size_t i = 0; i < all.size(); ++i) {
    keys[i] = all[i].first;
    uni[i] = all[i].second;
  }
  void* dp = nullptr;
  if (upload_owned(q, uni.data(), uni.size() * 8, &dp)) return -2;
  *vdict = (const uint64_t*)dp;
  q->hq.v_maxabs = max_abs_value(uni, vt);
  {
    int64_t b = 0, st = 0;
    if (affine_dictionary(uni, vt, &b, &st)) {
      q->hq.v_affine = 1;
      q->hq.v_base = b;
      q->hq.v_step = st;
    }
  }
  for (int si = 0; si < q->nseg; ++si) {
    const Column* c = q->segs[si]->cols.at(cid);
    std::vector<int32_t> rm(c->hvals.size());
    for (size_t i = 0; i < rm.size(); ++i)
      rm[i] = (int32_t)(std::lower_bound(keys.begin(), keys.end(), value_order_key(c->hvals[i], vt)) - keys.begin());
    void* rp = nullptr;
    if (upload_owned(q, rm.data(), rm.size() * 4, &rp)) return -2;
    q->hsegs[si].vremap = (const int32_t*)rp;
    q->vremap_host[si] = std::move(rm);
  }
  (void)P;
  return std::max(1, 64 - __builtin_clzll((unsigned long long)std::max<size_t>(1, uni.size() - 1)));
}

std::vector<DevSeg> count_pass_segments(const pa_query* q, const Prep& P) {
  std::vector<DevSeg> out = q->hsegs;
  const int nslots = (int)q->slot_cols.size();
  for (DevSeg& d : out) {
    d.num_staged = 0;
    for (int sl = 0; sl < nslots; ++sl) {
      DevCol& dc = d.cols[sl];
      if (dc.lds_off < 0) continue;
      bool filter_col = false;
      for (size_t li = 0; li < q->literals.size(); ++li) filter_col |= d.leaves[li].slot == sl;
      bool gb_col = false;
      for (int j = 0; j < q->spec.num_group_by; ++j) gb_col |= P.gb_slot[j] == sl && j != q->count_skip;
      if (gb_col || filter_col) {
        d.stage[d.num_staged++] = StageDesc{dc.words, dc.nbits, 0};
// ... 674 lines not shown
    if (ok && slot >= 0) {
      auto it = q->segs[0]->cols.find(q->slot_cols[slot]);
      if (it != q->segs[0]->cols.end() && it->second->kind == COL_SV_RAW) h.lds_raw_slot = slot;
    }
  }
  if (!q->partitioned) {
    h.hll_agg = -1;
    h.pv = 0;
    h.num_parts = 0;
  }
  for (int a = 0; a < s.num_aggs; ++a) {
    DevAgg& A = h.aggs[a];
    A.type = s.aggs[a].type;
    A.slot = P.agg_slot[a];
    A.log2m = s.aggs[a].log2m;
    A.src = P.agg_src[a];
    A.nvals = s.aggs[a].type == PA_AGG_DISTINCTCOUNT ? presence_stride(s.aggs[a])
              : s.aggs[a].type == PA_AGG_VALUE_HISTOGRAM ? hist_stride(s.aggs[a]) : 0;
    if (is_gdense(q->strategy)) {
      A.gd_vs = P.gd_vs[a];
      A.gd_op = P.gd_op[a];
      A.gd_acc = P.gd_acc[a];
      A.gd_tab = P.gd_tab_a[a];
      A.gd_tab_n = P.gd_tab_an[a];
      A.gd_base = P.gd_base[a];
      A.gd_step = P.gd_step[a];
    }
    if (!q->partitioned) {
      A.lds_off = (int32_t)P.agg_lds[a];
      A.pay_off = 0;
    }
    if (q->agg_section[a] >= 0) {
      void* p = q->sections[q->agg_section[a]].ptr;
      A.acc_i64 = (int64_t*)p;
      A.acc_f64 = (double*)p;
      A.acc_hll = (uint8_t*)p;
    }
  }
}

int plan_scratch(pa_query* q, const Prep& P) {
  const DevQuery& h = q->hq;
  const size_t G = (size_t)q->grid, Pn = (size_t)h.num_parts;
  uint64_t vrecs = 0, hrecs = 0;
  if (h.pv > 0) {
    vrecs = q->num_docs;
    if (mv_group_component(q) >= 0) {
      vrecs = 0;
      for (const pa_segment* seg : q->segs)
        vrecs += (uint64_t)seg->cols.at(q->spec.group_by_columns[mv_group_component(q)])->total_values;
    }
    vrecs += (uint64_t)G * h.pv * (h.bs_v - 1);
  }
  if (h.hll_agg >= 0) {
    const int32_t cid = q->spec.aggs[h.hll_agg].column_id;
    for (const pa_segment* seg : q->segs) {
      const Column* c = seg->cols.at(cid);
      hrecs += c->kind == COL_MV_DICT ? (uint64_t)c->total_values : (uint64_t)seg->num_docs;
    }
    hrecs += (uint64_t)G * (Pn - h.pv) * (h.bs_h - 1);
  }
  auto al = [](size_t x) { return (x + 255) & ~(size_t)255; };
  size_t o = 0;
  q->sc_hist = o; o += al(G * (size_t)q->count_k * Pn * 4);
  q->sc_off = o; o += al(G * Pn * 4);
  q->sc_base = o; o += al((Pn + 2) * 8);
  q->sc_recs_v = o; o += al((size_t)vrecs * h.rec_words_v * 4);
  q->sc_recs_h = o; o += al((size_t)hrecs * 4);
  q->sc_bytes = std::max<size_t>(o, 256);
  (void)P;
  if (hipGetDevice(&q->scratch_dev) != hipSuccess) q->scratch_dev = 0;
  ScratchArena* a = arena_for(q->scratch_dev);
  std::lock_guard<std::mutex> g(a->mu);
  return arena_grow(a, q->sc_bytes);
}

int plan_walk(pa_query* q, const Prep& P) {
  if (!q->limit_walk) return PA_OK;
  int64_t n = 0;
  for (int si = 0; si < q->nseg; ++si) n += P.limit_bind[si] ? 1 : 0;
  int rc = dev_alloc(q->lim_admit, (size_t)std::max<int64_t>(1, n) * (size_t)q->walk_words * 4);
  if (rc) return rc;
  int64_t k = 0;
  for (int si = 0; si < q->nseg; ++si)
    q->hsegs[si].admit = P.limit_bind[si] ? (const uint32_t*)q->lim_admit.p + (k++) * q->walk_words : nullptr;
  return PA_OK;
}

int plan_limit_buffers(pa_query* q, const Prep& P, int cus, int64_t total_tiles) {
  const pa_query_spec& s = q->spec;
  uint64_t H = 1024;
  while (H < 2 * P.limit_pairs && H <= (uint64_t(1) << 30)) H <<= 1;
  if (H > (uint64_t(1) << 30))
    return fail(PA_EUNSUPPORTED, "numGroupsLimit trimming: more than 2^29 distinct (segment, group) pairs possible");
  const size_t hb = (size_t)H * 8;
  int rc = dev_alloc(q->lim_keys, hb);
  if (!rc) rc = dev_alloc(q->lim_pos, hb);
  const size_t ns = (size_t)std::max(1, q->nseg);
  if (!rc) rc = dev_alloc(q->lim_hist, ns * 256 * 4);
  if (!rc) rc = dev_alloc(q->lim_sel, ns * 16);
  if (!rc) rc = dev_alloc(q->lim_thresh, ns * 8);
  if (rc) return rc;
  LimitDesc& F = q->limit;
  F.fkeys = (long long*)q->lim_keys.p;
  F.fpos = (unsigned long long*)q->lim_pos.p;
  F.fmask = (int64_t)H - 1;
  F.hist = (uint32_t*)q->lim_hist.p;
  F.prefix = (unsigned long long*)q->lim_sel.p;
  F.rank = (long long*)q->lim_sel.p + ns;
  F.nseg = q->nseg;
  {
    int64_t maxd = 1;
    for (int si = 0; si < q->nseg; ++si) maxd = std::max<int64_t>(maxd, q->segs[si]->num_docs);
    int b = 0;
    while (b < 63 && (int64_t(1) << b) < maxd) ++b;
    F.pos_bits = std::max(8, b + P.limit_eb);
  }
  F.thresh = (unsigned long long*)q->lim_thresh.p;
  F.reached = q->hq.matched_docs + 2;
  F.limit = s.num_groups_limit;
  F.eb = P.limit_eb;
  q->limit_grid = (int)std::max<int64_t>(1, std::min<int64_t>((int64_t)cus * 16, total_tiles));
  return PA_OK;
}

int upload_descriptors(pa_query* q) {
  int rc;
  if (is_gdense(q->strategy)) {
    rc = dev_alloc(q->dgdplans, sizeof(uint32_t) * q->gdplans.size());
    if (rc) return rc;
    PA_HIP(hipMemcpy(q->dgdplans.p, q->gdplans.data(), sizeof(uint32_t) * q->gdplans.size(), hipMemcpyHostToDevice));
    q->hq.gd_plans = (const uint32_t*)q->dgdplans.p;
  }
  rc = dev_alloc(q->dq, sizeof(DevQuery));
  if (rc) return rc;
  rc = dev_alloc(q->dsegs, sizeof(DevSeg) * std::max(1, q->nseg));
  if (rc) return rc;
  PA_HIP(hipMemcpy(q->dq.p, &q->hq, sizeof(DevQuery), hipMemcpyHostToDevice));
  if (q->nseg) PA_HIP(hipMemcpy(q->dsegs.p, q->hsegs.data(), sizeof(DevSeg) * q->nseg, hipMemcpyHostToDevice));
  if (q->partitioned) {
    rc = dev_alloc(q->dq_count, sizeof(DevQuery));
    if (!rc) rc = dev_alloc(q->dsegs_count, sizeof(DevSeg) * std::max(1, q->nseg));
    if (rc) return rc;
    PA_HIP(hipMemcpy(q->dq_count.p, &q->hq_count, sizeof(DevQuery), hipMemcpyHostToDevice));
    if (q->split_emit) {
      rc = dev_alloc(q->dq_h, sizeof(DevQuery));
      if (rc) return rc;
      PA_HIP(hipMemcpy(q->dq_h.p, &q->hq_h, sizeof(DevQuery), hipMemcpyHostToDevice));
    }
    if (q->nseg)
      PA_HIP(hipMemcpy(q->dsegs_count.p, q->hsegs_count.data(), sizeof(DevSeg) * q->nseg, hipMemcpyHostToDevice));
  }
  q->hplans.assign(std::max(1, q->nseg), LmSegPlan{});
  if (q->lane_major) {
    for (int si = 0; si < q->nseg; ++si) {
      const DevSeg& d = q->hsegs[si];
      LmSegPlan& P = q->hplans[si];
      std::memset(&P, 0, sizeof(P));
      P.nstaged = d.num_staged;
      P.neager = q->num_eager;
      P.num_docs = d.num_docs;
      P.num_wtiles = d.num_wtiles;
      P.dummy_lo = (uint32_t)(uintptr_t)d.dummy_src;
      P.dummy_hi = (uint32_t)((uint64_t)(uintptr_t)d.dummy_src >> 32);
      for (int k = 0; k < d.num_staged; ++k) {
        P.st[k].lo = (uint32_t)(uintptr_t)d.stage[k].words;
        P.st[k].hi = (uint32_t)((uint64_t)(uintptr_t)d.stage[k].words >> 32);
        P.st[k].nbits = d.stage[k].nbits;
        P.st[k].lds_off = d.stage[k].lds_off;
      }
      for (int li = 0; li < q->num_eager; ++li) {
        const DevLeaf& L = d.leaves[li];
        if (L.lds_off < 0) return fail(PA_EINVAL, "internal: eager literal on an unstaged column");
        P.lf[li].kind = L.kind;
        P.lf[li].nbits = L.nbits;
        P.lf[li].lds_off = L.lds_off;
        P.lf[li].lo = (uint32_t)L.lo;
        P.lf[li].span = (uint32_t)L.span;
        P.lf[li].flags = (L.negate ? 1 : 0) | (L.clause_end ? 2 : 0);
        P.lf[li].lut_lo = (uint32_t)(uintptr_t)L.lut;
        P.lf[li].lut_hi = (uint32_t)((uint64_t)(uintptr_t)L.lut >> 32);
      }
    }
  }
  rc = dev_alloc(q->dplans, sizeof(LmSegPlan) * q->hplans.size());
  if (rc) return rc;
  PA_HIP(hipMemcpy(q->dplans.p, q->hplans.data(), sizeof(LmSegPlan) * q->hplans.size(), hipMemcpyHostToDevice));
  if (q->partitioned) {
    PA_HIP(set_scan_lds_limit(q->emit_strat, q->steps, 0, q->lds_bytes));
    if (q->split_emit) PA_HIP(set_scan_lds_limit(q->emit_h_strat, q->steps, 0, q->emit_h_lds));
    PA_HIP(set_scan_lds_limit(q->count_strat, q->steps, 0, q->count_lds));
    PA_HIP(set_part_agg_lds_limit(q->part_vk, q->part_lds_c));
  } else {
    PA_HIP(set_scan_lds_limit(q->strategy, q->steps, q->lane_major, q->lds_bytes));
  }
  return PA_OK;
}

PartScratch scratch_of(const pa_query* q, void* base) {
  char* b = (char*)base;
  return PartScratch{(uint32_t*)(b + q->sc_hist), (uint32_t*)(b + q->sc_off), (uint64_t*)(b + q->sc_base),
                     (uint32_t*)(b + q->sc_recs_v), (uint32_t*)(b + q->sc_recs_h)};
}


size_t leap_header_bytes(const pa_query* q) {
  return ((size_t)std::max(1, q->nseg) * 3 + 1 + (size_t)q->leap_slices) * sizeof(unsigned long long);
}

int plan_leaps(pa_query* q, const Prep& P) {
  const pa_query_spec& s = q->spec;
  q->leap_leaf = -1;
  q->hq.leap_mode = 0;
  q->hq.leap_out = nullptr;
  if ((s.flags & PA_QF_NO_FILTER_STATS) || q->literals.size() != 2 || q->num_eager != 1) return PA_OK;
  if (!q->clause_end[0] || !q->clause_end[1] || q->literals[0].neg || q->literals[1].neg) return PA_OK;
  for (const Literal& lit : q->literals) {
    const int k = s.leaves[lit.leaf].kind;
    if (k == PA_LEAF_MV_DICT_RANGE || k == PA_LEAF_MV_DICT_SET) return PA_OK;
  }
  if (q->partitioned || q->limit_mode || q->limit_walk || is_gdense(q->strategy)) return PA_OK;
  if (P.first_clause_sel > 1.0 / 256.0) return PA_OK;
  q->hq.leap_mode = 1;
  q->leap_leaf = q->literals[0].leaf;
  return PA_OK;
}

int alloc_leaps(pa_query* q, const Prep& P) {
  if (!q->hq.leap_mode) return PA_OK;
  const int64_t slices = (int64_t)q->grid * scan_waves(q->strategy);
  const int64_t cap = (int64_t)(16.0 * P.first_clause_sel * (double)q->num_docs / (double)slices) + 256;
  q->leap_slices = slices;
  if (slices > kLeapMaxSlices) {
    q->hq.leap_mode = 0;
    q->leap_leaf = -1;
    return PA_OK;
  }
  q->hq.leap_lds_cap = 0;
  {
    const int wpw = scan_waves(q->strategy);
    const int want = (int)std::min<int64_t>(cap, 128);
    const size_t extra = (size_t)wpw * want * 8;
    if (q->plan_wg > 0 && ((size_t)q->lds_bytes + extra) * (size_t)q->plan_wg <= kLdsBudget) {
      q->hq.leap_lds_cap = want;
      q->lds_bytes += (int)extra;
    }
  }
  const size_t words = (size_t)std::max(1, q->nseg) * 3 + 1 + (size_t)slices + (size_t)slices * (size_t)cap;
  int rc = dev_alloc(q->leap_buf, words * sizeof(unsigned long long));
  if (rc) return rc;
  PA_HIP(hipMemset(q->leap_buf.p, 0, leap_header_bytes(q)));
  q->hq.leap_out = (unsigned long long*)q->leap_buf.p;
  q->hq.leap_cap = cap;
  q->hq.leap_slices = slices;
  return PA_OK;
}
```

pinot_amd/csrc/pa_scan.h:

```cpp
#pragma once
#include <hip/hip_runtime.h>
#include "pa_device.h"
#include "pa_launch.h"
#include "pa_keys.h"

namespace pa {

typedef __attribute__((address_space(3))) uint32_t lds_u32_t;
typedef const __attribute__((address_space(4))) struct DevSeg CSegT;
typedef const __attribute__((address_space(4))) struct DevQuery CQ;

#define AS1 __attribute__((address_space(1)))
template <class T>
__device__ __forceinline__ AS1 T* gp(T* p) { return (AS1 T*)p; }
template <class T>
__device__ __forceinline__ const AS1 T* gp(const T* p) { return (const AS1 T*)p; }
#define RLX __ATOMIC_RELAXED, __HIP_MEMORY_SCOPE_AGENT
typedef uint32_t u32x4 __attribute__((ext_vector_type(4)));

__device__ __forceinline__ void vm_wait_all() { asm volatile("s_waitcnt vmcnt(0)" ::: "memory"); }

__device__ __forceinline__ uint32_t nbits_mask(int nb) { return nb >= 32 ? 0xffffffffu : ((1u << nb) - 1u); }

__device__ __forceinline__ uint32_t decode_lds(const uint32_t* region, int doc_local, int nb) {
  const uint32_t e1 = (uint32_t)doc_local * (uint32_t)nb + (uint32_t)(nb - 1);
  const int we = (int)(e1 >> 5);
  const uint32_t lo = region[we];
  const uint32_t hi = region[we - 1];
  return __builtin_amdgcn_alignbit(hi, lo, (~e1) & 31u) & nbits_mask(nb);
}

__device__ __forceinline__ uint32_t decode_global(const uint32_t* words, int64_t doc, int nb) {
  const uint64_t e1 = (uint64_t)doc * (uint64_t)nb + (uint64_t)(nb - 1);
  const int64_t we = (int64_t)(e1 >> 5);
  const uint32_t lo = gp(words)[we];
  const uint32_t hi = gp(words)[we - 1];
  return __builtin_amdgcn_alignbit(hi, lo, (~(uint32_t)e1) & 31u) & nbits_mask(nb);
}

template <bool G = false>
__device__ __forceinline__ uint32_t decode_dict_id(const DevCol& c, const uint32_t* img, int doc_local,
                                                   int64_t doc) {
  if constexpr (G) return decode_global(c.words, doc, c.nbits);
  return c.lds_off >= 0 ? decode_lds(img + c.lds_off, doc_local, c.nbits) : decode_global(c.words, doc, c.nbits);
}

template <int N>
__device__ __forceinline__ void vm_wait() {
  static_assert(N >= 0 && N < 64, "vmcnt is 6 bits");
  asm volatile("s_waitcnt vmcnt(%0)" ::"n"(N) : "memory");
}

__device__ __forceinline__ uint32_t lds_addr(const void* p) {
  return (uint32_t)(uintptr_t)(const __attribute__((address_space(3))) void*)p;
}

typedef __attribute__((address_space(3))) uint64_t lds_u64_t;
typedef __attribute__((address_space(3))) u32x4 lds_u32x4_t;
__device__ __forceinline__ lds_u32_t* lds_ptr(const void* p) { return (lds_u32_t*)(uintptr_t)lds_addr(p); }

#define WG_RLX __ATOMIC_RELAXED, __HIP_MEMORY_SCOPE_WORKGROUP


__device__ __forceinline__ void dma16(const void* src, uint32_t lds_base) {
  uint32_t keep;
  lds_base = (uint32_t)__builtin_amdgcn_readfirstlane((int)lds_base);
  asm volatile(
      "s_mov_b32 %0, m0\n\t"
      "s_mov_b32 m0, %2\n\t"
      "s_nop 0\n\t"
      "global_load_lds_dwordx4 %1, off\n\t"
      "s_mov_b32 m0, %0"
      : "=&s"(keep)
      : "v"(src), "s"(lds_base));
}

__device__ __forceinline__ void dma16_masked(const void* src, uint32_t lds_base, uint64_t mask) {
  uint32_t keep;
  uint64_t save;
  lds_base = (uint32_t)__builtin_amdgcn_readfirstlane((int)lds_base);
  asm volatile(
      "s_mov_b64 %1, exec\n\t"
      "s_mov_b64 exec, %4\n\t"
      "s_mov_b32 %0, m0\n\t"
      "s_mov_b32 m0, %3\n\t"
      "s_nop 0\n\t"
      "global_load_lds_dwordx4 %2, off\n\t"
      "s_mov_b32 m0, %0\n\t"
      "s_mov_b64 exec, %1"
      : "=&s"(keep), "=&s"(save)
      : "v"(src), "s"(lds_base), "s"(mask));
}

template <int STEPS>
__device__ __forceinline__ void stage_tile(const DevSeg* __restrict__ seg, int64_t wt, uint32_t* img, int lane,
                                           const int D) {
  const int ns = seg->num_staged;
  int issued = 0;
  for (int si = 0; si < ns; ++si) {
    const StageDesc& c = seg->stage[si];
    const int nb = c.nbits;
    const uint32_t* src = c.words + wt * (int64_t)(2 * STEPS * nb);
    const uint32_t dst = lds_addr(img + c.lds_off);
    const int chunks = (STEPS / 2) * nb;
    for (int c0 = 0; c0 < chunks; c0 += 64) {
      if (c0 + lane < chunks) dma16(src + 4 * (c0 + lane), dst + 16 * c0);
      ++issued;
    }
  }
  for (; issued < D; ++issued) {
    if (lane == 0) dma16(seg->dummy_src, lds_addr(img));
  }
}

__device__ __forceinline__ int64_t wave_sum_i64(int64_t v) {
#pragma unroll
  for (int o = 32; o > 0; o >>= 1) v += __shfl_xor(v, o);
  return v;
}
__device__ __forceinline__ double wave_sum_f64(double v) {
#pragma unroll
  for (int o = 32; o > 0; o >>= 1) v += __shfl_xor(v, o);
  return v;
}
__device__ __forceinline__ int64_t wave_min_i64(int64_t v) {
#pragma unroll
  for (int o = 32; o > 0; o >>= 1) { const int64_t w = __shfl_xor(v, o); v = w < v ? w : v; }
  return v;
}
__device__ __forceinline__ int64_t wave_max_i64(int64_t v) {
#pragma unroll
  for (int o = 32; o > 0; o >>= 1) { const int64_t w = __shfl_xor(v, o); v = w > v ? w : v; }
  return v;
}

struct AggValue {
  int64_t i;
  double d;
};

template <bool G = false>
__device__ __forceinline__ AggValue agg_value(const DevAgg& A, int a, const DevSeg* __restrict__ seg,
                                              const uint32_t* img, int doc_local, int64_t doc) {
  AggValue out{0, 0.0};
  const DevCol& c = seg->cols[A.slot];
  if (c.kind == COL_SV_DICT) {
    const uint32_t id = decode_dict_id<G>(c, img, doc_local, doc);
    if (A.type == PA_AGG_DISTINCTCOUNTHLL) {
      out.i = gp(seg->hll_lut[a])[id];
    } else if (A.type == PA_AGG_DISTINCTCOUNT || A.type == PA_AGG_VALUE_HISTOGRAM) {
      out.i = seg->hll_lut[a] != nullptr ? gp(seg->hll_lut[a])[id] : id;
    } else if (A.src != SRC_DOUBLE) {
      out.i = gp(c.dict_i64)[id];
    } else {
      out.d = gp(c.dict_f64)[id];
    }
  } else {
    int64_t iv = 0;
    double dv = 0.0;
    switch (c.vtype) {
      case PA_INT: iv = gp((const int32_t*)c.raw)[doc]; dv = (double)iv; break;
      case PA_LONG: iv = gp((const int64_t*)c.raw)[doc]; dv = (double)iv; break;
      case PA_FLOAT: { const float f = gp((const float*)c.raw)[doc]; dv = f; iv = __builtin_bit_cast(int32_t, f); } break;
      default: dv = gp((const double*)c.raw)[doc]; iv = __builtin_bit_cast(int64_t, dv); break;
    }
    if (A.type == PA_AGG_DISTINCTCOUNTHLL) {
      out.i = hll_slot_rank(murmur_hash_long(iv), A.log2m);
    } else if (A.src != SRC_DOUBLE) {
      out.i = iv;
    } else {
      out.d = dv;
    }
  }
  return out;
}

__device__ __forceinline__ void atomic_max_u8(uint8_t* p, uint32_t v) {
  AS1 uint32_t* w = (AS1 uint32_t*)((uintptr_t)p & ~(uintptr_t)3);
  const uint32_t sh = ((uint32_t)(uintptr_t)p & 3u) * 8u;
  uint32_t old = __hip_atomic_load(w, RLX);
  while (((old >> sh) & 0xffu) < v) {
    const uint32_t nw = (old & ~(0xffu << sh)) | (v << sh);
    if (__hip_atomic_compare_exchange_strong(w, &old, nw, __ATOMIC_RELAXED, __ATOMIC_RELAXED, __HIP_MEMORY_SCOPE_AGENT))
      break;
  }
}

template <int STRAT>
struct Acc {
  const DevQuery* q;
  unsigned char* lds;
  const PartScratch* ps;

  __device__ __forceinline__ void add_count(int64_t key, uint32_t n) const {
    if (STRAT == STRAT_LDS) atomicAdd((uint32_t*)(lds + q->lds_count_off) + key, n);
    else __hip_atomic_fetch_add(gp(q->count) + key, (unsigned long long)n, RLX);
  }
  __device__ __forceinline__ void add_i64(const DevAgg& A, int64_t key, int64_t v) const {
    if (STRAT == STRAT_LDS) atomicAdd((unsigned long long*)(lds + A.lds_off) + key, (unsigned long long)v);
    else __hip_atomic_fetch_add(gp((unsigned long long*)A.acc_i64) + key, (unsigned long long)v, RLX);
  }
  __device__ __forceinline__ void add_f64(const DevAgg& A, int64_t key, double v) const {
    if (STRAT == STRAT_LDS) atomicAdd((double*)(lds + A.lds_off) + key, v);
    else __hip_atomic_fetch_add(gp(A.acc_f64) + key, v, RLX);
  }
  __device__ __forceinline__ void min_i64(const DevAgg& A, int64_t key, int64_t v) const {
    if (STRAT == STRAT_LDS) atomicMin((long long*)(lds + A.lds_off) + key, (long long)v);
    else __hip_atomic_fetch_min(gp((long long*)A.acc_i64) + key, (long long)v, RLX);
  }
  __device__ __forceinline__ void max_i64(const DevAgg& A, int64_t key, int64_t v) const {
    if (STRAT == STRAT_LDS) atomicMax((long long*)(lds + A.lds_off) + key, (long long)v);
    else __hip_atomic_fetch_max(gp((long long*)A.acc_i64) + key, (long long)v, RLX);
  }
  __device__ __forceinline__ void set_presence(const DevAgg& A, int64_t key, int64_t v) const {
    if (STRAT == STRAT_LDS) ((uint8_t*)(lds + A.lds_off))[key * A.nvals + v] = 1;
    else gp(A.acc_hll)[key * A.nvals + v] = 1;
  }
  __device__ __forceinline__ void add_hist(const DevAgg& A, int64_t key, int64_t v) const {
    if (STRAT == STRAT_LDS) atomicAdd((uint32_t*)(lds + A.lds_off) + key * A.nvals + v, 1u);
    else __hip_atomic_fetch_add(gp((unsigned long long*)A.acc_i64) + key * A.nvals + v, 1ull, RLX);
  }
  __device__ __forceinline__ void max_hll(const DevAgg& A, int64_t key, uint32_t jr) const {
    const int64_t idx = (key << A.log2m) + (jr >> 8);
    if (STRAT == STRAT_LDS) atomicMax((uint32_t*)(lds + A.lds_off) + idx, jr & 0xffu);
    else atomic_max_u8(A.acc_hll + idx, jr & 0xffu);
  }
};

template <bool G = false>
__device__ __forceinline__ uint64_t gb_component(const DevCol& c, const int32_t* remap, const uint32_t* img,
                                                 int doc_local, int64_t doc) {
  if (c.kind == COL_SV_RAW) {
    switch (c.vtype) {
      case PA_INT: return (uint64_t)(uint32_t)gp((const int32_t*)c.raw)[doc];
      case PA_FLOAT: return (uint64_t)gp((const uint32_t*)c.raw)[doc];
      default: return (uint64_t)gp((const int64_t*)c.raw)[doc];
    }
  }
  uint32_t id = decode_dict_id<G>(c, img, doc_local, doc);
  if (remap != nullptr) id = (uint32_t)gp(remap)[id];
  return id;
}

__device__ __forceinline__ int64_t key_slot(const DevQuery* __restrict__ q, int64_t k0, int64_t k1 = 0) {
  if (!q->hashed) return k0;
// ... 2024 lines not shown
    for (int i = 0; i < STEPS; ++i) {
      const uint32_t bit = 1u << i;
      if (__ballot((m & bit) != 0) == 0) continue;
      const int64_t doc = doc_base + local(i);
      bool ok = (m & bit) != 0;
      bool any = false;
      for (int li = neager; li < nleaves; ++li) {
        const DevLeaf& L = seg->leaves[li];
        if (ok && !any) any = leaf_match_doc(L, doc);
        if (L.clause_end) {
          ok = ok && any;
          any = false;
        }
      }
      if (!ok) m &= ~bit;
    }
    if constexpr (!is_pcount(STRAT) && !is_pemit(STRAT))
      if (q->leap_mode) leap_tile<LM>(q, seg, doc_base, eager, m, lane, la.leap_slice, la.leap_n, la.leap_lds);
    if (__ballot(m != 0) == 0) return 0;
  }
  const uint32_t scanned = m;
  if (seg->admit != nullptr && q->gb_mv < 0) {
    m = admitted_docs<LM, STEPS>(q, seg, img, doc_base, m, lane);
    if (__ballot(m != 0) == 0) return (uint32_t)__builtin_popcount(scanned);
  }
  if constexpr (is_lane(STRAT)) {
    if constexpr (STRAT != STRAT_LANE_CNT) lane_acc_tile<LM, STEPS, STRAT>(q, seg, img, doc_base, m, lane, la, lds);
  } else if constexpr (is_pcount(STRAT) || is_pemit(STRAT)) {
    part_tile<STRAT, STEPS, LM>(q, seg, img, doc_base, m, lane, lds, ps);

  } else if (q->has_mv) {
    for (int i = 0; i < STEPS; ++i)
      if ((m >> i) & 1u) accumulate_doc_mv<STRAT>(q, seg, img, local(i), doc_base + local(i), acc);
  } else if constexpr (STRAT == STRAT_LDS && LM) {
    uint32_t tot = (uint32_t)__builtin_popcount(m);
#pragma unroll
    for (int o = 1; o < kWave; o <<= 1) tot += (uint32_t)__shfl_xor((int)tot, o, kWave);
    const int rs = q->hashed ? -1 : q->lds_raw_slot;
    if (tot > 256u && rs >= 0 && seg->cols[rs].kind == COL_SV_RAW) {
      const int vt = seg->cols[rs].vtype;
      if (vt == PA_INT || vt == PA_FLOAT) accumulate_lds_raw_dense<4>(q, seg, img, doc_base, m, lane, lds);
      else accumulate_lds_raw_dense<8>(q, seg, img, doc_base, m, lane, lds);
    } else if (tot > 512u) {
      accumulate_lds_lm<8>(q, seg, img, doc_base, m, lane, lds);
    } else {
      accumulate_lds_lm<4>(q, seg, img, doc_base, m, lane, lds);
    }
  } else if (q->has_mv) {
    for (int i = 0; i < STEPS; ++i)
      if ((m >> i) & 1u) accumulate_doc_mv<STRAT>(q, seg, img, local(i), doc_base + local(i), acc);
  } else {
    for (int i = 0; i < STEPS; ++i) {
      const uint64_t sm = __ballot((m >> i) & 1u);
      if (sm == 0) continue;
      accumulate_step<STRAT>(q, seg, img, local(i), doc_base + local(i), sm, lane, acc);
    }
  }
  __builtin_amdgcn_s_waitcnt((7 << 4) | (15 << 8));
  return (uint32_t)__builtin_popcount(scanned);
}

template <int STRAT, int STEPS>
__device__ __forceinline__ void process_tile(const DevQuery* __restrict__ q, const DevSeg* __restrict__ seg,
                                             int64_t wt, const uint32_t* img, int lane, const Acc<STRAT>& acc,
                                             uint32_t& matched, LaneAcc& la) {
  const int64_t doc_base = wt * (STEPS * kWave);
  const int64_t rem = (int64_t)seg->num_docs - doc_base;
  constexpr uint32_t kFull = STEPS == 32 ? 0xffffffffu : ((1u << STEPS) - 1u);
  uint32_t valid;
  if (rem >= (STEPS * kWave)) {
    valid = kFull;
  } else {
    const int64_t n = rem > lane ? (rem - lane + kWave - 1) / kWave : 0;
    valid = n >= 32 ? 0xffffffffu : ((1u << n) - 1u);
  }
  uint32_t m = valid;
  uint32_t clause = 0;
  const int neager = q->num_eager;
  for (int li = 0; li < neager; ++li) {
    const DevLeaf& L = seg->leaves[li];
    clause |= leaf_bits<STEPS>(L, img, doc_base, lane);
    if (L.clause_end) {
      m &= clause;
      clause = 0;
      if (__ballot(m != 0) == 0) return;
    }
  }
  if (__ballot(m != 0) == 0) return;
  matched += tile_survivors<STRAT, STEPS, 0>(q, seg, img, doc_base, m, lane, acc.lds, *acc.ps, la);
}



__device__ __forceinline__ uint32_t rl(uint32_t v, int k) { return (uint32_t)__builtin_amdgcn_readlane((int)v, k); }

template <int NB>
__device__ __forceinline__ uint32_t leaf_lm(int kind, uint32_t region_lds, int lane, uint32_t lo_t, uint32_t hi_t,
                                            const uint32_t* lut) {
  const lds_u32_t* p = (const lds_u32_t*)(uintptr_t)(region_lds + (uint32_t)lane * (uint32_t)(NB * 4));
  constexpr int H = NB > 16 ? 2 : 1;
  constexpr int DPH = 32 / H;
  uint32_t nm = 0, bits = 0;
#pragma unroll
  for (int h = H - 1; h >= 0; --h) {
    constexpr int WMAX = (DPH * NB + 31) / 32 + 1;
    const int wlo = (h * DPH * NB) >> 5;
    uint32_t w[WMAX];
#pragma unroll
    for (int j = 0; j < WMAX; ++j) w[j] = (wlo + j < NB) ? p[wlo + j] : 0u;
    auto top = [&](int i) -> uint32_t {
      const int s = i * NB, j = (s >> 5) - wlo, o = s & 31;
      if (o + NB <= 32) return w[j] << o;
      return __builtin_amdgcn_alignbit(w[j], w[(j + 1 < WMAX) ? j + 1 : j], 32 - o);
    };
    if (kind == PA_LEAF_DICT_RANGE) {
#pragma unroll
      for (int i = (h + 1) * DPH - 1; i >= h * DPH; --i) {
        const uint32_t t = top(i);
        uint32_t u;
        asm("v_sub_u32_e64 %[u], %[t], %[lo]\n\t"
            "v_sub_co_u32_e32 %[u], vcc, %[hi], %[u]\n\t"
            "v_addc_co_u32_e32 %[nm], vcc, %[nm], %[nm], vcc"
            : [nm] "+v"(nm), [u] "=&v"(u)
            : [t] "v"(t), [lo] "s"(lo_t), [hi] "s"(hi_t)
            : "vcc");
      }
    } else {
      const AS1 uint32_t* lt = gp(lut);
#pragma unroll
      for (int i = h * DPH; i < (h + 1) * DPH; ++i) {
        const uint32_t id = top(i) >> (32 - NB);
        bits |= ((lt[id >> 5] >> (id & 31u)) & 1u) << i;
      }
    }
  }
  return kind == PA_LEAF_DICT_RANGE ? ~nm : bits;
}

__device__ __forceinline__ uint32_t leaf_lm_any(int nb, int kind, uint32_t region_lds, int lane, uint32_t lo_t,
                                                uint32_t hi_t, const uint32_t* lut) {
  switch (nb) {
#define PA_LM_CASE(N) \
  case N: return leaf_lm<N>(kind, region_lds, lane, lo_t, hi_t, lut);
    PA_LM_CASE(1) PA_LM_CASE(2) PA_LM_CASE(3) PA_LM_CASE(4) PA_LM_CASE(5) PA_LM_CASE(6) PA_LM_CASE(7) PA_LM_CASE(8)
    PA_LM_CASE(9) PA_LM_CASE(10) PA_LM_CASE(11) PA_LM_CASE(12) PA_LM_CASE(13) PA_LM_CASE(14) PA_LM_CASE(15)
    PA_LM_CASE(16) PA_LM_CASE(17) PA_LM_CASE(18) PA_LM_CASE(19) PA_LM_CASE(20) PA_LM_CASE(21) PA_LM_CASE(22)
    PA_LM_CASE(23) PA_LM_CASE(24) PA_LM_CASE(25) PA_LM_CASE(26) PA_LM_CASE(27) PA_LM_CASE(28) PA_LM_CASE(29)
    PA_LM_CASE(30) PA_LM_CASE(31) PA_LM_CASE(32)
#undef PA_LM_CASE
    default: return 0;
  }
}

__device__ __forceinline__ void stage_tile_lm(uint32_t ip, int64_t wt, uint32_t img_lds, int lane, const int D) {
  const int ns = (int)rl(ip, 0);
  int issued = 0;
  for (int c = 0; c < ns; ++c) {
    const uint64_t words = ((uint64_t)rl(ip, 9 + 4 * c) << 32) | rl(ip, 8 + 4 * c);
    const int nb = (int)rl(ip, 10 + 4 * c);
    const uint32_t dst = img_lds + 4u * rl(ip, 11 + 4 * c);
    const char* src = (const char*)words + wt * (int64_t)(256 * nb) + 16 * lane;
    const int chunks = 16 * nb;
    for (int c0 = 0; c0 < chunks; c0 += 64) {
      if (c0 + lane < chunks) dma16(src + 16 * c0, dst + 16 * c0);
      ++issued;
    }
  }
  const void* dummy = (const void*)(((uint64_t)rl(ip, 5) << 32) | rl(ip, 4));
  for (; issued < D; ++issued) {
    if (lane == 0) dma16(dummy, img_lds);
  }
}

template <int STRAT>
__device__ __forceinline__ void process_tile_lm(const DevQuery* __restrict__ q, const DevSeg* __restrict__ seg,
                                                uint32_t pp, int64_t wt, const uint32_t* img, uint32_t img_lds,
                                                int lane, const Acc<STRAT>& acc, uint32_t& matched, LaneAcc& la) {
  const int64_t doc_base = wt * kWTileDocs;
  const int64_t rem = (int64_t)(int32_t)rl(pp, 2) - doc_base;
  uint32_t valid = 0xffffffffu;
  if (rem < kWTileDocs) {
    const int64_t n = rem - 32 * lane;
    valid = n >= 32 ? 0xffffffffu : (n <= 0 ? 0u : ((1u << n) - 1u));
  }
  uint32_t m = valid;
  uint32_t clause = 0;
  const int neager = (int)rl(pp, 1);
  for (int l = 0; l < neager; ++l) {
    const int b = 24 + 8 * l;
    const int flags = (int)rl(pp, b + 5);
    const uint32_t* lut = (const uint32_t*)(((uint64_t)rl(pp, b + 7) << 32) | rl(pp, b + 6));
    uint32_t bits = leaf_lm_any((int)rl(pp, b + 1), (int)rl(pp, b), img_lds + 4u * rl(pp, b + 2), lane,
                                rl(pp, b + 3), rl(pp, b + 4), lut);
    if (flags & 1) bits = ~bits;
    clause |= bits;
    if (flags & 2) {
      m &= clause;
      clause = 0;
      if (__ballot(m != 0) == 0) return;
    }
  }
  if (__ballot(m != 0) == 0) return;
  matched += tile_survivors<STRAT, 32, 1>(q, seg, img, doc_base, m, lane, acc.lds, *acc.ps, la);
}

__device__ __forceinline__ int find_segment(const DevSeg* __restrict__ segs, int nseg, int64_t t) {
  int lo = 0, hi = nseg - 1;
  while (lo < hi) {
    const int mid = (lo + hi + 1) >> 1;
    if (segs[mid].first_wtile <= t) lo = mid;
    else hi = mid - 1;
  }
  while (t >= segs[lo].first_wtile + segs[lo].num_wtiles) ++lo;
  return lo;
}

template <int N>
__device__ __forceinline__ void vm_wait_token(uint32_t& token) {
  static_assert(N >= 0 && N < 64, "vmcnt is 6 bits");
  token = (uint32_t)__builtin_amdgcn_readfirstlane((int)token);
  asm volatile("s_waitcnt vmcnt(%1)" : "+s"(token) : "n"(N));
}

template <int LO, int HI>
__device__ __forceinline__ void vm_wait_n(uint32_t& token, int n) {
  if constexpr (LO == HI) {
    vm_wait_token<LO>(token);
  } else {
    constexpr int MID = (LO + HI) / 2;
    if (n <= MID) vm_wait_n<LO, MID>(token, n);
    else vm_wait_n<MID + 1, HI>(token, n);
  }
}

__device__ __forceinline__ void wait_tile(int younger, int D, uint32_t& token) {
  const int n = younger * D;
  vm_wait_n<0, 63>(token, n < 63 ? n : 63);
}

struct LmIssue {
  const char* base[kLmStaged];
  int64_t stride[kLmStaged];
  uint32_t off[kLmStaged];
  int nfull[kLmStaged];
  uint64_t tail[kLmStaged];
  int nst;
  const void* dummy;
};

__device__ __forceinline__ void lm_wait_issue(const LmIssue& I, uint32_t& slot_off, int R, int D, int64_t younger,
                                              uint32_t dst0, int64_t it, uint32_t lane_off) {
  if (R == 2) vm_wait_token<0>(slot_off);
  else wait_tile((int)younger, D, slot_off);
  int issued = 0;
#pragma unroll
  for (int c = 0; c < kLmStaged; ++c) {
    if (c < I.nst) {
      const char* src = I.base[c] + it * I.stride[c] + lane_off;
      const uint32_t dst = dst0 + I.off[c];
      for (int k = 0; k < I.nfull[c]; ++k) dma16(src + 1024 * k, dst + 1024 * k);
      issued += I.nfull[c];
      if (I.tail[c]) {
        dma16_masked(src + 1024 * I.nfull[c], dst + 1024 * I.nfull[c], I.tail[c]);
        ++issued;
      }
    }
  }
  for (; issued < D; ++issued) dma16_masked(I.dummy, dst0, 1ull);
}

__device__ __forceinline__ int64_t xcd_major_block(int64_t b, int64_t G) {
  constexpr int kXcds = 8;
  const int64_t x = b % kXcds, j = b / kXcds, per = G / kXcds, extra = G % kXcds;
  return x * per + (x < extra ? x : extra) + j;
}

__host__ __device__ constexpr bool emit_v_wide(int s) {
  return is_pemit(s) && !pemit_hh(s) && !pemit_big(s) && pemit_vf(s) != V_FMT_GEN;
}

template <int STRAT, int STEPS, int LM>
__global__ void __launch_bounds__(scan_waves(STRAT) * kWave, emit_v_wide(STRAT) ? 2 : (scan_waves(STRAT) == kWavesPerWG ? 4 : 1)) scan_kernel(const DevQuery* __restrict__ q,
                                                       const DevSeg* __restrict__ segs,
                                                       const LmSegPlan* __restrict__ plans, PartScratch ps) {
  static_assert(!LM || STEPS == 32, "lane-major tiles are 2048 docs");
  constexpr int WPW = scan_waves(STRAT);
  constexpr int WGS = WPW * kWave;
  extern __shared__ __attribute__((aligned(16))) uint32_t smem[];
  const int lane = threadIdx.x & 63;
  const int wave = __builtin_amdgcn_readfirstlane(threadIdx.x >> 6);
  unsigned char* lds_acc = (unsigned char*)smem;
  const uint32_t acc_dwords = STRAT != STRAT_GLOBAL ? (q->lds_acc_bytes >> 2) : 0u;
  const int img_dw = q->image_dwords_max;
  uint32_t* ring = smem + acc_dwords + wave * q->ring * img_dw;
  Acc<STRAT> acc{q, lds_acc, &ps};

  if (STRAT == STRAT_LDS) {
    const int64_t K = q->num_keys;
    uint32_t* cnt = (uint32_t*)(lds_acc + q->lds_count_off);
    for (int64_t k = threadIdx.x; k < K; k += WGS) cnt[k] = 0;
    for (int a = 0; a < q->num_aggs; ++a) {
      const DevAgg& A = q->aggs[a];
      if (A.type == PA_AGG_COUNT) continue;
      if (A.type == PA_AGG_DISTINCTCOUNTHLL) {
        uint32_t* r = (uint32_t*)(lds_acc + A.lds_off);
        for (int64_t k = threadIdx.x; k < (K << A.log2m); k += WGS) r[k] = 0;
      } else if (A.type == PA_AGG_DISTINCTCOUNT) {
        uint32_t* r = (uint32_t*)(lds_acc + A.lds_off);
        for (int64_t k = threadIdx.x; k < K * A.nvals / 4; k += WGS) r[k] = 0;
      } else if (A.type == PA_AGG_VALUE_HISTOGRAM) {
        uint32_t* r = (uint32_t*)(lds_acc + A.lds_off);
        for (int64_t k = threadIdx.x; k < K * A.nvals; k += WGS) r[k] = 0;
      } else {
        int64_t* r = (int64_t*)(lds_acc + A.lds_off);
        const int64_t init = A.type == PA_AGG_MIN ? INT64_MAX : (A.type == PA_AGG_MAX ? INT64_MIN : 0);
        const int64_t n = (A.type == PA_AGG_SUM && A.src == SRC_LONG) ? 2 * K : K;
        for (int64_t k = threadIdx.x; k < n; k += WGS) r[k] = init;
      }
    }
    __syncthreads();
  } else if (is_pcount(STRAT)) {
    uint32_t* hist = (uint32_t*)lds_acc;
    for (int p = threadIdx.x; p < q->num_parts; p += WGS) hist[p] = 0u;
    __syncthreads();
  } else if (is_pemit(STRAT)) {
    const BinState B = bin_state(q, lds_acc);
    const int64_t lbi = q->xcd_major ? xcd_major_block(blockIdx.x, gridDim.x) : (int64_t)blockIdx.x;
    const int P = q->num_parts, pv = q->pv;
    for (int p = q->part_lo + threadIdx.x; p < q->part_hi; p += WGS) {
      B.cnt[p] = 0u;
      B.done[p] = 0u;
      B.front[p] = 0u;
      if (p >= pv) B.slk[p] = 0u;
      B.back[p] = gp(ps.hist)[lbi * P + p];
      B.start[p] = gp(ps.base)[p < pv ? p : p + 1] + gp(ps.off)[lbi * P + p];
    }
    __syncthreads();
  }

  uint32_t matched = 0;
  LaneAcc la;
  la.leap_slice = (uint32_t)((q->xcd_major ? xcd_major_block(blockIdx.x, gridDim.x) : (int64_t)blockIdx.x) * WPW + wave);
  la.leap_n = 0u;
  la.leap_lds = lds_addr(smem + acc_dwords + (uint32_t)WPW * (uint32_t)q->ring * (uint32_t)img_dw) +
                (uint32_t)wave * (uint32_t)q->leap_lds_cap * 8u;
  if constexpr (is_lane(STRAT) && STRAT != STRAT_LANE_CNT) lane_acc_init(q, la, smem, WGS);
  if constexpr (STRAT == STRAT_LANE_DICT) {
    for (int a = 0; a < q->num_aggs; ++a) {
      const int hc = q->aggs[a].hist_card;
      if (hc <= 0) continue;
      uint32_t* h = (uint32_t*)(lds_acc + q->aggs[a].hist_off);
      for (int i = threadIdx.x; i < hc; i += WGS) h[i] = 0u;
    }
    __syncthreads();
  }
  const int64_t T = q->total_wtiles;
  const int64_t W = (int64_t)gridDim.x * WPW;
  const int64_t lb = q->xcd_major ? xcd_major_block(blockIdx.x, gridDim.x) : (int64_t)blockIdx.x;
  const int64_t gw = lb * WPW + wave;
  const int64_t t0 = gw * T / W;
  const int64_t t1 = (gw + 1) * T / W;
  if (t0 < t1) {
    const int R = q->ring;
    const int D = q->dma_per_tile;
    int isi = find_segment(segs, q->num_segments, t0);
    int64_t ifirst = segs[isi].first_wtile;
    int64_t iend = ifirst + segs[isi].num_wtiles;
    uint32_t ip = LM ? ((const uint32_t*)(plans + isi))[lane] : 0u;
    int64_t ti = t0;
    int islot = 0;
    const uint32_t ring_lds = lds_addr(ring);
    auto issue_next = [&]() {
      while (ti >= iend) {
        ++isi;
        ifirst = segs[isi].first_wtile;
        iend = ifirst + segs[isi].num_wtiles;
        if (LM) ip = ((const uint32_t*)(plans + isi))[lane];
      }
      if constexpr (LM) stage_tile_lm(ip, ti - ifirst, ring_lds + 4u * (uint32_t)(islot * img_dw), lane, D);
      else stage_tile<STEPS>(segs + isi, ti - ifirst, ring + islot * img_dw, lane, D);
      ++ti;
      islot = islot + 1 == R ? 0 : islot + 1;
    };
    for (int k = 0; k < R - 1 && ti < t1; ++k) issue_next();

    int si = find_segment(segs, q->num_segments, t0);
    int pslot = 0;
    int64_t t = t0;
    while (t < t1) {
      const DevSeg* seg = segs + si;
      const uint32_t matched_seg0 = matched;
      const int64_t seg_first = seg->first_wtile;
      const int64_t seg_end = min(t1, seg_first + (int64_t)seg->num_wtiles);
      const uint32_t pp = LM ? ((const uint32_t*)(plans + si))[lane] : 0u;
      const bool stream_only = q->debug_stream_only != 0;
      if constexpr (LM) {
        if (!stream_only && isi == si) {
          LmIssue I;
          I.nst = (int)rl(pp, 0);
#pragma unroll
          for (int c = 0; c < kLmStaged; ++c) {
            const int nb = c < I.nst ? (int)rl(pp, 10 + 4 * c) : 0;
            I.base[c] = (const char*)(((uint64_t)rl(pp, 9 + 4 * c) << 32) | rl(pp, 8 + 4 * c));
            I.stride[c] = 256 * (int64_t)nb;
            I.off[c] = 4u * rl(pp, 11 + 4 * c);
            I.nfull[c] = (16 * nb) / 64;
            const int tail = (16 * nb) % 64;
            I.tail[c] = tail ? ((1ull << tail) - 1ull) : 0ull;
          }
          I.dummy = (const void*)(((uint64_t)rl(pp, 5) << 32) | rl(pp, 4));
          const int64_t issue_end = min(iend, t1);
          const bool single_range = (int)rl(pp, 1) == 1 && (int)rl(pp, 24) == PA_LEAF_DICT_RANGE && (rl(pp, 29) & 2u);
          if (single_range) {
            const int nb0 = (int)rl(pp, 25);
            const uint32_t off0 = 4u * rl(pp, 26), lo0 = rl(pp, 27), hi0 = rl(pp, 28);
            const bool neg0 = (rl(pp, 29) & 1u) != 0;
            const int64_t full_tiles = (int64_t)(int32_t)rl(pp, 2) / kWTileDocs;
            while (t < seg_end && ti < issue_end) {
              uint32_t slot_off = (uint32_t)(pslot * img_dw);
              lm_wait_issue(I, slot_off, R, D, ti - (t + 1), ring_lds + 4u * (uint32_t)(islot * img_dw), ti - ifirst,
                            16u * (uint32_t)lane);
              ++ti;
              islot = islot + 1 == R ? 0 : islot + 1;
              if (t - seg_first < full_tiles) {
                uint32_t m = leaf_lm_any(nb0, PA_LEAF_DICT_RANGE, ring_lds + 4u * slot_off + off0, lane, lo0, hi0,
                                         nullptr);
                if (neg0) m = ~m;
                if (__ballot(m != 0) != 0)
                  matched += tile_survivors<STRAT, 32, 1>(q, seg, ring + slot_off, (t - seg_first) * kWTileDocs, m,
                                                          lane, acc.lds, *acc.ps, la);
              } else {
                process_tile_lm<STRAT>(q, seg, pp, t - seg_first, ring + slot_off, ring_lds + 4u * slot_off, lane, acc,
                                       matched, la);
              }
              pslot = pslot + 1 == R ? 0 : pslot + 1;
              ++t;
            }
          } else {
            while (t < seg_end && ti < issue_end) {
              uint32_t slot_off = (uint32_t)(pslot * img_dw);
              lm_wait_issue(I, slot_off, R, D, ti - (t + 1), ring_lds + 4u * (uint32_t)(islot * img_dw), ti - ifirst,
                            16u * (uint32_t)lane);
              ++ti;
              islot = islot + 1 == R ? 0 : islot + 1;
              process_tile_lm<STRAT>(q, seg, pp, t - seg_first, ring + slot_off, ring_lds + 4u * slot_off, lane, acc,
                                     matched, la);
              pslot = pslot + 1 == R ? 0 : pslot + 1;
              ++t;
            }
          }
        }
      }
      for (; t < seg_end; ++t) {
        uint32_t slot_off = (uint32_t)(pslot * img_dw);
        wait_tile((int)(ti - (t + 1)), D, slot_off);
        if (ti < t1) issue_next();
        if (!stream_only) {
          if constexpr (LM) process_tile_lm<STRAT>(q, seg, pp, t - seg_first, ring + slot_off, ring_lds + 4u * slot_off, lane, acc, matched, la);
          else process_tile<STRAT, STEPS>(q, seg, t - seg_first, ring + slot_off, lane, acc, matched, la);
        }
        pslot = pslot + 1 == R ? 0 : pslot + 1;
      }
      if constexpr (is_lane(STRAT) && STRAT != STRAT_LANE_CNT) lane_acc_segment_end(q, seg, la, matched != matched_seg0);
      if (t < t1) {
        ++si;
        while (t >= segs[si].first_wtile + segs[si].num_wtiles) ++si;
      }
    }
  }

  if constexpr (!is_pcount(STRAT) && !is_pemit(STRAT))
    if (q->leap_mode) {
      const uint32_t nl = min(la.leap_n, (uint32_t)q->leap_lds_cap);
      AS1 unsigned long long* list = gp(q->leap_out) + 3 * (int64_t)q->num_segments + 1 + (int64_t)q->leap_slices +
                                     (int64_t)la.leap_slice * (int64_t)q->leap_cap;
      const lds_u64_t* ll = (const lds_u64_t*)(uintptr_t)la.leap_lds;
      for (uint32_t k = (uint32_t)lane; k < nl; k += kWave) list[k] = ll[k];
      if (lane == 0) gp(q->leap_out)[3 * (int64_t)q->num_segments + 1 + la.leap_slice] = la.leap_n;
    }
  if (!is_pemit(STRAT)) {
    const int64_t wm = wave_sum_i64((int64_t)matched);
    if (lane == 0 && wm != 0) __hip_atomic_fetch_add(gp(q->matched_docs), (unsigned long long)wm, RLX);
    if constexpr (is_lane(STRAT)) {
      if (lane == 0 && wm != 0) __hip_atomic_fetch_add(gp(q->count), (unsigned long long)wm, RLX);
      if constexpr (STRAT == STRAT_LANE_DICT) {
        __syncthreads();
        for (int a = 0; a < q->num_aggs; ++a) {
          const DevAgg& A = q->aggs[a];
          if (A.hist_card <= 0) continue;
          const uint32_t* h = (const uint32_t*)(lds_acc + A.hist_off);
          const DevCol& c = segs[0].cols[A.slot];
          int64_t r0, r1;
          la_get(la, a, r0, r1);
          for (int i = threadIdx.x; i < A.hist_card; i += WGS) {
            const uint32_t n = h[i];
            if (n == 0) continue;
            if (A.src == SRC_DOUBLE) {
              r0 = __builtin_bit_cast(int64_t, __builtin_bit_cast(double, r0) + (double)n * gp(c.dict_f64)[i]);
            } else {
              const int64_t v = gp(c.dict_i64)[i];
              if (A.src == SRC_INT) {
                r0 += (int64_t)n * v;
              } else {
                r0 += (int64_t)n * (int64_t)(uint32_t)v;
                r1 += (int64_t)n * (v >> 32);
              }
            }
          }
          la_set(la, a, r0, r1);
        }
      }
      if constexpr (STRAT != STRAT_LANE_CNT) lane_acc_flush(q, la, lane);
    }
  }
  if (is_pcount(STRAT)) {
    __syncthreads();
    const uint32_t* hist = (const uint32_t*)lds_acc;
    for (int p = threadIdx.x; p < q->num_parts; p += WGS) gp(ps.hist)[lb * q->num_parts + p] = hist[p];
  }
  if (is_pemit(STRAT)) {
    __syncthreads();
    const BinState B = bin_state(q, lds_acc);
    const int P = q->num_parts, pv = q->pv;
    for (int p = q->part_lo + threadIdx.x; p < q->part_hi; p += WGS) {
      const bool isv = p < pv;
      const uint32_t nw = isv ? (uint32_t)q->rec_words_v : 1u;
      const uint32_t BS = (uint32_t)(isv ? q->bs_v : q->bs_h);
      const lds_u32_t* bin = isv ? lds_ptr(lds_acc + q->lds_bins_v) + (uint32_t)p * BS * nw
                                 : lds_ptr(lds_acc + q->lds_bins_h) + (uint32_t)(p - pv) * (BS + (uint32_t)kDocVals);
      AS1 uint32_t* recs = gp(isv ? ps.recs_v : ps.recs_h);
      const uint32_t n = B.cnt[p], o = B.front[p];
      const uint32_t h = gp(ps.hist)[lb * P + p];
      if ((n >= BS || o + n != B.back[p]) && !q->debug_emit)
        __hip_atomic_fetch_add(gp(q->matched_docs) + 3, 1ull, RLX);
      AS1 uint32_t* d = recs + (B.start[p] + o) * (uint64_t)nw;
      const uint32_t nn = n < BS ? n : BS;
      for (uint32_t e = 0; e < nn * nw; ++e) d[e] = bin[e];
      const uint32_t padded = (h + BS - 1u) / BS * BS;
      AS1 uint32_t* z = recs + (B.start[p] + h) * (uint64_t)nw;
      for (uint32_t e = 0; e < (padded - h) * nw; ++e) z[e] = (e % nw) == 0 ? kSentinel : 0u;
    }
  }
  if (STRAT == STRAT_LDS) {
    __syncthreads();
    const int64_t K = q->num_keys;
    const uint32_t* cnt = (const uint32_t*)(lds_acc + q->lds_count_off);
    for (int64_t k = threadIdx.x; k < K; k += WGS) {
      const uint32_t c = cnt[k];
      if (c == 0) continue;
      __hip_atomic_fetch_add(gp(q->count) + k, (unsigned long long)c, RLX);
      for (int a = 0; a < q->num_aggs; ++a) {
        const DevAgg& A = q->aggs[a];
        switch (A.type) {
          case PA_AGG_SUM:
            if (A.src == SRC_INT) {
              __hip_atomic_fetch_add(gp((unsigned long long*)A.acc_i64) + k, ((const unsigned long long*)(lds_acc + A.lds_off))[k], RLX);
            } else if (A.src == SRC_LONG) {
              const unsigned long long* r = (const unsigned long long*)(lds_acc + A.lds_off);
              __hip_atomic_fetch_add(gp((unsigned long long*)A.acc_i64) + 2 * k, r[2 * k], RLX);
              __hip_atomic_fetch_add(gp((unsigned long long*)A.acc_i64) + 2 * k + 1, r[2 * k + 1], RLX);
            } else {
              __hip_atomic_fetch_add(gp(A.acc_f64) + k, ((const double*)(lds_acc + A.lds_off))[k], RLX);
            }
            break;
          case PA_AGG_COUNT_MV:
            __hip_atomic_fetch_add(gp((unsigned long long*)A.acc_i64) + k, ((const unsigned long long*)(lds_acc + A.lds_off))[k], RLX);
            break;
          case PA_AGG_MIN: __hip_atomic_fetch_min(gp((long long*)A.acc_i64) + k, ((const long long*)(lds_acc + A.lds_off))[k], RLX); break;
          case PA_AGG_MAX: __hip_atomic_fetch_max(gp((long long*)A.acc_i64) + k, ((const long long*)(lds_acc + A.lds_off))[k], RLX); break;
          case PA_AGG_DISTINCTCOUNT: {
            const uint32_t* r = (const uint32_t*)(lds_acc + A.lds_off + k * A.nvals);
            AS1 uint8_t* g = gp(A.acc_hll) + k * A.nvals;
            for (int64_t j = 0; j < A.nvals / 4; ++j) {
              const uint32_t w = r[j];
              if (w == 0) continue;
              for (int b = 0; b < 4; ++b)
                if ((w >> (8 * b)) & 0xffu) g[4 * j + b] = 1;
            }
          } break;
          case PA_AGG_DISTINCTCOUNTHLL: {
            const uint32_t* r = (const uint32_t*)(lds_acc + A.lds_off) + (k << A.log2m);
            uint8_t* g = A.acc_hll + (k << A.log2m);
            for (int j = 0; j < (1 << A.log2m); ++j)
              if (r[j] != 0) atomic_max_u8(g + j, r[j]);
          } break;
          default: break;
        }
      }
    }
    for (int a = 0; a < q->num_aggs; ++a) {
      const DevAgg& A = q->aggs[a];
      if (A.type != PA_AGG_VALUE_HISTOGRAM) continue;
      const uint32_t* r = (const uint32_t*)(lds_acc + A.lds_off);
      AS1 unsigned long long* g = gp((unsigned long long*)A.acc_i64);
      for (int64_t i = threadIdx.x; i < K * A.nvals; i += WGS)
// ... 14 lines not shown
```

pinot_amd/csrc/pa_tuning.h:

```cpp
#pragma once
#include <cstdint>
#include <cstring>

#define PA_TUNINGS(X)                                                                                                  \
                                                                                  \
  X(gdl_w, -1, 8, 16, 0)                                                                                               \
  X(gdl_nd, -1, 8, 16, 0)                                                                                              \
  X(gdl_rs, -1, 1, 2, 0)                                                                                               \
                                                                                        \
  X(gdl_rr, -1, 1, 64, 0)                                                                                              \
                    \
  X(gdl_ring, -1, 2, 4, 0)                                                                                             \
         \
  X(gdl_dbg, 0, 0, 3, 1)                                                                                               \
                                      \
  X(pve_nd, -1, 8, 16, 0)                                                                                              \
         \
  X(pve_bs, -1, 16, 32, 0)                                                                                             \
                                                                              \
  X(pve_q, -1, 0, 1, 0)                                                                                                \
   \
  X(pve_ring, -1, 2, 4, 0)                                                                                             \
              \
  X(pve_hrun, -1, 0, 1, 0)                                                                                             \
                       \
  X(pve_hb, -1, 1, 8, 0)                                                                                               \
                                    \
  X(pve_dbg, 0, 0, 2, 1)                                                                                               \
                                                               \
  X(passc_v16, -1, 0, 1, 0)                                                                                            \
                                                                      \
  X(walk_tab, 1, 0, 1, 0)                                                                                              \
               \
  X(debug_emit, 0, 0, 127, 1)

struct Tuning {
#define X(name, def, lo, hi, inv) int32_t name = def;
  PA_TUNINGS(X)
#undef X
};

struct TuningDef {
  const char* name;
  int32_t Tuning::*value;
  int32_t def, lo, hi;
  bool results_invalid;
};
inline constexpr TuningDef kTunings[] = {
#define X(name, def, lo, hi, inv) {#name, &Tuning::name, def, lo, hi, inv != 0},
    PA_TUNINGS(X)
#undef X
};

inline const TuningDef* tuning_named(const char* name) {
  for (const TuningDef& d : kTunings)
    if (name && std::strcmp(d.name, name) == 0) return &d;
  return nullptr;
}

inline const char* tuning_invalidating(const Tuning& t) {
  for (const TuningDef& d : kTunings)
    if (d.results_invalid && t.*d.value != d.def) return d.name;
  return nullptr;
}
```

pinot_amd/engine.py:

```python
import ctypes
import dataclasses
import threading
from dataclasses import dataclass, field
from typing import Dict, List, Optional

import numpy as np

from . import _lib as L
from . import predicate as P
from . import query as Q
from .hll import HyperLogLog, hash_value
from .java_hash import java_hash_code
from .optimizer import optimize_filter
from .segment import Segment

_VTYPE = {"INT": L.PA_INT, "LONG": L.PA_LONG, "FLOAT": L.PA_FLOAT, "DOUBLE": L.PA_DOUBLE, "STRING": L.PA_STRING}


class UnsupportedQuery(L.PinotAmdError):
    pass


def column_ids_for(segment: Segment) -> Dict[str, int]:
    return {name: i for i, name in enumerate(sorted(segment.columns))}
# ... 337 lines not shown
            spec.leaves[li].kind = kind
        spec.num_ops = len(ops)
        for i, op in enumerate(ops):
            spec.ops[i] = op

        self.global_dicts = []
        self.remaps = []
        spec.num_group_by = len(q.group_by)
        if spec.num_group_by > L.PA_MAX_GROUP_BY:
            raise UnsupportedQuery("too many group-by columns")
        self.raw_group_by = []
        for j, name in enumerate(q.group_by):
            has_dict = [s.column(name).has_dictionary for s in self.segs]
            if not any(has_dict):
                self.global_dicts.append(None)
                self.raw_group_by.append(seg0.column(name).data_type)
                spec.group_by_columns[j] = ids[name]
                spec.group_by_cardinality[j] = 0
                continue
            if not all(has_dict):
                raise UnsupportedQuery("group-by column %s is dictionary-encoded in some segments only" % name)
            self.raw_group_by.append(None)
            dicts = [s.column(name).dictionary for s in self.segs]
            if name in self.table_dicts:
                gd = np.asarray(self.table_dicts[name])
                if not all(np.isin(d, gd).all() for d in dicts):
                    raise ValueError("table dictionary of %s misses values of a bound segment" % name)
            else:
                first = dicts[0]
                same = all(d is first or (len(d) == len(first) and np.array_equal(d, first)) for d in dicts)
                gd = first if same else np.unique(np.concatenate(dicts))
            self.global_dicts.append(gd)
            spec.group_by_columns[j] = ids[name]
            spec.group_by_cardinality[j] = len(gd)
        for seg in self.segs:
            rm = []
            for j, name in enumerate(q.group_by):
                d = seg.column(name).dictionary
                gd = self.global_dicts[j]
                if gd is None or d is gd or (len(d) == len(gd) and np.array_equal(d, gd)):
                    rm.append(None)
                else:
                    rm.append(np.searchsorted(gd, d).astype(np.int32))
            self.remaps.append(rm)
        spec.flags = ((self.flags & 0xffffffff) ^ 0x80000000) - 0x80000000
        spec.flags2 = (self.flags >> 32) & 0x7fffffff if self.flags >= 0 else 0
        spec.hash_keys_bound = self.hash_keys_bound

        spec.num_groups_limit = int(min(q.num_groups_limit, 2**31 - 1)) if (q.group_by and self.enforce_num_groups_limit) else 0

        self.spec = spec
        self.handle = L.check_ptr(lib.pa_query_create(ctypes.byref(spec), len(self.segs)), "pa_query_create")
        for name, value in self.tuning.items():
            L.check(lib.pa_query_set_tuning(self.handle, name.encode(), int(value)), "pa_query_set_tuning")
        self._keep = []
        for si, (g, params) in enumerate(zip(self.gsegs, per_seg)):
            arr = (L.LeafParams * max(1, len(params)))()
            for li, p in enumerate(params):
                lp = arr[li]
                if isinstance(p, P.DictLeaf):
                    lp.negate = int(p.negate)
                    if spec.leaves[li].kind in (L.PA_LEAF_DICT_SET, L.PA_LEAF_MV_DICT_SET):
                        ids_ = p.ids if p.ids is not None else np.arange(p.lo, p.hi, dtype=np.int32)
                        lut = P.DictLeaf(L.PA_LEAF_DICT_SET, ids=ids_).lut_words(self.segs[si].column(leaves[li].column).cardinality)
                        self._keep.append(lut)
                        lp.lut = lut.ctypes.data_as(ctypes.POINTER(ctypes.c_uint32))
                    else:
                        lp.lo, lp.hi = p.lo, p.hi
                else:
                    lp.negate = int(p.negate)
                    lp.ilo = max(min(int(p.ilo), P.LONG_MAX), P.LONG_MIN)
                    lp.ihi = max(min(int(p.ihi), P.LONG_MAX), P.LONG_MIN)
                    lp.dlo, lp.dhi = float(p.dlo), float(p.dhi)
                    if p.kind == L.PA_LEAF_RAW_SET:
                        vals = np.ascontiguousarray(p.values)
                        self._keep.append(vals)
                        lp.values = vals.ctypes.data if len(vals) else None
                        lp.num_values = len(vals)
            rms = (ctypes.c_void_p * max(1, len(q.group_by)))()
            for j, rm in enumerate(self.remaps[si]):
                if rm is not None:
                    self._keep.append(rm)
                    rms[j] = rm.ctypes.data
            L.check(lib.pa_query_bind_segment(self.handle, si, g.handle, arr, rms), "pa_query_bind_segment")
            for i, vd in self.value_dicts.items():
                d = self.segs[si].column(names[self.pa_aggs[i][1]]).dictionary
                if d is vd or (len(d) == len(vd) and np.array_equal(d, vd)):
                    continue
                if not np.isin(d, vd).all():
                    raise ValueError("table-wide value dictionary misses values of a bound segment")
                rm = np.searchsorted(vd, d).astype(np.int32)
                self._keep.append(rm)
                L.check(lib.pa_query_bind_value_remap(self.handle, si, i, rm.ctypes.data), "pa_query_bind_value_remap")
        L.check(lib.pa_query_prepare(self.handle), "pa_query_prepare")
        self.num_keys = int(lib.pa_query_num_keys(self.handle))
        hashed, shifts = ctypes.c_int32(), (ctypes.c_int32 * max(1, len(q.group_by)))()
        L.check(lib.pa_query_key_layout(self.handle, ctypes.byref(hashed), shifts), "pa_query_key_layout")
        self.hashed = bool(hashed.value)
        self.key_shifts = list(shifts)[:len(q.group_by)]
        self.key_words = int(lib.pa_query_key_words(self.handle))
        self.strides = []
        s = 1
        for gd in self.global_dicts:
            self.strides.append(s)
            s *= len(gd) if gd is not None else 1

    def execute(self, stream=None):
        if not self.segs or self.match_none:
            if self.handle is not None:
                L.check(L.lib().pa_query_reset(self.handle, stream), "pa_query_reset")
            return
        L.check(L.lib().pa_query_execute(self.handle, stream), "pa_query_execute")
        self._scanned = True
        self.merged_stats = None

    def reset(self, stream=None):
        L.check(L.lib().pa_query_reset(self.handle, stream), "pa_query_reset")
        self._scanned = False
        self.merged_stats = None

    def scan(self, stream=None):
        if not self.segs or self.match_none:
            return
        L.check(L.lib().pa_query_scan(self.handle, stream), "pa_query_scan")
        self._scanned = True
        self.merged_stats = None

    def sections(self):
        lib = L.lib()
        out = []
        for i in range(lib.pa_query_num_sections(self.handle)):
            kind, n = ctypes.c_int32(), ctypes.c_int64()
            p = L.check_ptr(lib.pa_query_section(self.handle, i, ctypes.byref(kind), ctypes.byref(n)), "section")
            out.append((kind.value, p, n.value))
        return out

    def stats(self):
        a, b, c = ctypes.c_uint64(), ctypes.c_uint64(), ctypes.c_uint64()
        L.check(L.lib().pa_query_stats(self.handle, ctypes.byref(a), ctypes.byref(b), ctypes.byref(c)), "stats")
        out = {"staged_bytes": a.value, "num_docs": b.value, "num_wave_tiles": c.value}
        vals = [ctypes.c_int32() for _ in range(7)]
        L.check(L.lib().pa_query_plan(self.handle, *[ctypes.byref(v) for v in vals]), "plan")
        names = ("strategy", "steps", "dma_slots", "ring", "wg_per_cu", "grid", "lds_bytes")
        out["plan"] = {n: v.value for n, v in zip(names, vals)}
        code = out["plan"]["strategy"]
        out["plan"]["strategy"] = {0: "lds", 1: "global", 2: "partitioned", 4: "lane", 5: "lane", 6: "lane", 7: "lane",
                                    8: "lds_dense", 9: "lds_dense", 10: "lds_dense", 11: "lds_dense", 12: "lds_dense",
                                    14: "lds_dense", 15: "lds_dense"}[code]
        out["plan"]["variant"] = STRATEGY_VARIANTS.get(code, str(code))
        out["plan"]["eager_literals"] = int(L.lib().pa_query_num_eager_literals(self.handle))
        out["plan"]["lane_major"] = int(L.lib().pa_query_lane_major(self.handle))
        out["plan"]["dense_packed"] = int(L.lib().pa_query_dense_packed(self.handle))
        out["plan"]["count_free_emit"] = int(L.lib().pa_query_count_free_emit(self.handle))
        out["plan"]["partition_keys"] = int(L.lib().pa_query_partition_keys(self.handle))
        out["plan"]["limit_trimming"] = int(L.lib().pa_query_limit_trimming(self.handle))
        out["plan"]["results_invalid"] = int(L.lib().pa_query_results_invalid(self.handle))
        return out

    def fetch_arrays(self, stream=None, pooled=False):
        lib = L.lib()
        alloc = (lambda slot, n, dt: OUTPUT_POOL.array(slot, n, dt)) if pooled else (lambda slot, n, dt: np.empty(n, dt))
        cap = 1 if not self.query.group_by else min(self.num_keys, 1 << 16)
        if self.query.group_by and self.num_keys > 1 << 16:
            cap = max(1, L.check(lib.pa_query_fetch(self.handle, stream, 0, None, None, None), "pa_query_fetch"))
        kw = getattr(self, "key_words", 1)
        while True:
            keys = alloc("keys", cap * kw, np.int64)
            counts = alloc("counts", cap, np.int64)
            outs, ptrs = [], (ctypes.c_void_p * max(1, len(self.pa_aggs)))()
            for i, (t, _, log2m) in enumerate(self.pa_aggs):
                if t == L.PA_AGG_DISTINCTCOUNTHLL:
                    o = alloc(i, cap << log2m, np.uint8)
                elif t == L.PA_AGG_DISTINCTCOUNT:
                    o = alloc(i, cap * self._presence_stride(i), np.uint8)
                elif t == L.PA_AGG_VALUE_HISTOGRAM:
                    outs.append(None)
                    continue
                else:
                    o = alloc(i, cap, np.float64)
                outs.append(o)
                ptrs[i] = o.ctypes.data
            n = L.check(lib.pa_query_fetch(self.handle, stream, cap, keys.ctypes.data, counts.ctypes.data, ptrs),
                        "pa_query_fetch")
            if n <= cap:
                break
            cap = n
        outs = [None if o is None else
                o[: n << self.pa_aggs[i][2]] if self.pa_aggs[i][0] == L.PA_AGG_DISTINCTCOUNTHLL else
                (o[: n * self._presence_stride(i)] if self.pa_aggs[i][0] == L.PA_AGG_DISTINCTCOUNT else o[:n])
                for i, o in enumerate(outs)]
        return (keys[:n] if kw == 1 else keys[:2 * n].reshape(n, 2)), counts[:n], outs

    def _presence_stride(self, i):
        return (len(self.value_dicts[i]) + 15) & ~15

    def fetch_histograms(self, pi, num_groups, stream=None):
        lib = L.lib()
        vd = np.asarray(self.value_dicts[pi], dtype=np.float64)
        n = int(num_groups)
        ends = np.zeros(max(n, 1), dtype=np.int64)
        total = L.check(lib.pa_query_fetch_histogram(self.handle, stream, pi, n, 0, ends.ctypes.data, None, None),
                        "pa_query_fetch_histogram")
        ids = OUTPUT_POOL.array("hist_ids", max(total, 1), np.int32)
        cnt = OUTPUT_POOL.array("hist_counts", max(total, 1), np.int64)
        if total:
            L.check(lib.pa_query_fetch_histogram(self.handle, stream, pi, n, total, ends.ctypes.data, ids.ctypes.data,
                                                 cnt.ctypes.data), "pa_query_fetch_histogram")
        values, counts = vd[ids[:total]], cnt[:total].copy()
        starts = np.concatenate([[0], ends[:n]])
        return [ValueHistogram(values[starts[g]:starts[g + 1]], counts[starts[g]:starts[g + 1]]) for g in range(n)]

    def percentiles(self, stream=None):
        lib = L.lib()
        q = self.query
        by_acc = {}
        for ai, (a, pi) in enumerate(zip(q.aggregations, self.agg_map)):
            if a.function in Q.PERCENTILE_FUNCTIONS:
                by_acc.setdefault(pi, []).append(ai)
        if self.handle is None or not by_acc:
            return np.zeros(0, dtype=np.int64), {ai: np.zeros(0) for ais in by_acc.values() for ai in ais}
        n = L.check(lib.pa_query_fetch(self.handle, stream, 0, None, None, None), "pa_query_fetch")
        n = max(n, 0 if q.group_by else 1)
        keys = np.zeros(max(n, 1), dtype=np.int64)
        counts = np.zeros(max(n, 1), dtype=np.int64)
        if n:
            L.check(lib.pa_query_fetch(self.handle, stream, n, keys.ctypes.data, counts.ctypes.data, None),
                    "pa_query_fetch")
        out = {}
        for pi, ais in by_acc.items():
            ps = np.array([q.aggregations[ai].percentile for ai in ais], dtype=np.float64)
            ids = np.full(max(n, 1) * len(ps), -1, dtype=np.int32)
            if n:
                L.check(lib.pa_query_percentiles(self.handle, stream, pi, n, len(ps), ps.ctypes.data, ids.ctypes.data),
                        "pa_query_percentiles")
            ids = ids[:n * len(ps)].reshape(n, len(ps))
            vd = np.asarray(self.value_dicts[pi], dtype=np.float64)
            for j, ai in enumerate(ais):
                col = ids[:, j]
                out[ai] = np.where(col >= 0, vd[np.maximum(col, 0)], -np.inf)
        return keys[:n], out

    def key_values(self, keys):
        if not self.hashed:
            return [gd[(keys // st) % len(gd)] for gd, st in zip(self.global_dicts, self.strides)]
        kk = np.asarray(keys, dtype=np.int64)
        words = [kk.view(np.uint64)] if kk.ndim == 1 else [np.ascontiguousarray(kk[:, w]).view(np.uint64)
                                                           for w in range(kk.shape[1])]
        out = []
        for gd, raw, shw in zip(self.global_dicts, self.raw_group_by, self.key_shifts):
            k, sh = words[shw // 64], shw % 64
            if gd is not None:
                bits = max(1, int(len(gd) - 1).bit_length())
            else:
                bits = 32 if raw in ("INT", "FLOAT") else 64
            comp = (k >> np.uint64(sh)) & np.uint64((1 << bits) - 1) if bits < 64 else (k >> np.uint64(sh))
            if gd is not None:
                out.append(gd[comp.astype(np.int64)])
            elif raw == "INT":
                out.append(comp.astype(np.uint32).view(np.int32))
            elif raw == "FLOAT":
                out.append(comp.astype(np.uint32).view(np.float32))
            elif raw == "LONG":
                out.append(comp.view(np.int64))
            else:
                out.append(comp.view(np.float64))
        return out

    def torch_device(self):
        import torch
        return torch.device("cuda", self.device if self.device is not None else torch.cuda.current_device())

    def leaf_bitmaps(self, segment_index, stream=None):
        import torch
        lib = L.lib()
        nl = int(self.spec.num_leaves)
        n = self.segs[segment_index].num_docs
        if nl == 0:
            return np.zeros((0, n), dtype=bool)
        words = L.check(lib.pa_query_leaf_bitmap_words(self.handle, segment_index), "pa_query_leaf_bitmap_words")
        dev = self.torch_device()
        buf = torch.zeros(nl * words, dtype=torch.int32, device=dev)
        L.check(lib.pa_query_leaf_bitmaps(self.handle, segment_index, buf.data_ptr(), stream), "pa_query_leaf_bitmaps")
        torch.cuda.synchronize(dev)
        w = buf.cpu().numpy().view(np.uint8).reshape(nl, words * 4)
        return np.unpackbits(w, axis=1, bitorder="little")[:, :n].astype(bool)

    def fused_leap_counts(self, stream=None):
        lib = L.lib()
        if self.handle is None or not self.segs or not getattr(self, "_scanned", False):
            return None
        e = int(lib.pa_query_leap_leaf(self.handle))
        if e < 0:
            return None
        out = np.zeros((len(self.segs), 3), dtype=np.int64)
        L.check(lib.pa_query_leap_counts(self.handle, out.ctypes.data, stream), "pa_query_leap_counts")
        return e, 1 - e, out

    def execution_stats(self, stream=None, docs_total=None):
        from . import filter_stats as FS
        self.stats_replayed_segments = self.stats_gpu_segments = 0
        if self.match_none or self.handle is None or not self.segs:
            return 0, 0
        if getattr(self, "_stats_trees", None) is None:
            self._stats_trees = FS.operator_trees(self.query, self.segs, getattr(self, "leaf_params", None),
                                                  self.gsegs[0].column_ids)
        ops, roots, seg_tree = self._stats_trees
# ... 130 lines not shown
```

Measured before the change: 2365 billion rows/s.

## Add SWAR equality prefilter, nontemporal streaming loads, and fused accumulator reset

New measurement: 2435 billion rows/s (median of 6 runs). 1.03x the previous value.

```diff
diff --git a/include/pinot_amd.h b/include/pinot_amd.h
--- a/include/pinot_amd.h
+++ b/include/pinot_amd.h
@@ -251,6 +251,8 @@
 int32_t pa_query_lane_major(const pa_query* q);
 int32_t pa_query_dense_packed(const pa_query* q);
 int32_t pa_query_count_free_emit(const pa_query* q);
+int32_t pa_query_eq_prefilter(const pa_query* q);
+int32_t pa_query_stream_nt(const pa_query* q);
 int32_t pa_query_partition_keys(const pa_query* q);
 int pa_query_plan(const pa_query* q, int32_t* strategy, int32_t* steps, int32_t* dma_slots, int32_t* ring,
                   int32_t* wg_per_cu, int32_t* grid, int32_t* lds_bytes);
diff --git a/pinot_amd/_lib.py b/pinot_amd/_lib.py
--- a/pinot_amd/_lib.py
+++ b/pinot_amd/_lib.py
@@ -57,7 +57,8 @@
     "pa_query_create", "pa_query_set_tuning", "pa_query_results_invalid", "pa_query_bind_segment",
     "pa_query_bind_value_remap", "pa_query_prepare", "pa_query_num_keys",
     "pa_query_execute", "pa_query_reset", "pa_query_scan", "pa_query_num_eager_literals", "pa_query_lane_major",
-    "pa_query_dense_packed", "pa_query_count_free_emit", "pa_query_partition_keys",
+    "pa_query_dense_packed", "pa_query_count_free_emit", "pa_query_eq_prefilter", "pa_query_stream_nt",
+    "pa_query_partition_keys",
     "pa_query_accumulator_bytes", "pa_query_set_accumulator_buffer", "pa_query_num_sections", "pa_query_section",
     "pa_query_fetch", "pa_query_fetch_histogram", "pa_query_percentiles", "pa_query_matched_docs", "pa_query_key_layout", "pa_query_limit_trimming",
     "pa_query_num_groups_limit_reached", "pa_query_stats", "pa_query_leaf_bitmap_words", "pa_query_leaf_bitmaps",
@@ -146,6 +147,8 @@
         "pa_query_lane_major": (i32, [vp]),
         "pa_query_dense_packed": (i32, [vp]),
         "pa_query_count_free_emit": (i32, [vp]),
+        "pa_query_eq_prefilter": (i32, [vp]),
+        "pa_query_stream_nt": (i32, [vp]),
         "pa_query_partition_keys": (i32, [vp]),
         "pa_query_accumulator_bytes": (u64, [vp]),
         "pa_query_set_accumulator_buffer": (ctypes.c_int, [vp, vp, u64]),
diff --git a/pinot_amd/csrc/pa_capi.hip b/pinot_amd/csrc/pa_capi.hip
--- a/pinot_amd/csrc/pa_capi.hip
+++ b/pinot_amd/csrc/pa_capi.hip
@@ -152,6 +152,7 @@
   const int wpw = q->partitioned ? scan_waves(q->emit_strat) : scan_waves(q->strategy);
   const int64_t want = (total_tiles + wpw - 1) / wpw;
   q->grid = (int)std::max<int64_t>(1, std::min(max_wg, want));
+  if (q->tune.scan_grid > 0 && !q->partitioned) q->grid = (int)std::min<int64_t>(q->grid, q->tune.scan_grid);
 
   if (q->partitioned) {
     int64_t ct = 0;
@@ -211,7 +212,41 @@
 int pa_query_reset(pa_query* q, void* stream) {
   if (!q || !q->prepared) return fail(PA_EINVAL, "query not prepared");
   hipStream_t st = (hipStream_t)stream;
-  PA_HIP(hipMemsetAsync(q->external_acc ? q->external_acc : q->acc.p, 0, q->acc.n, st));
+  char* block = (char*)(q->external_acc ? q->external_acc : q->acc.p);
+  auto identity = [](const Section& sc, int64_t& v) {
+    if (sc.kind == PA_ACC_MIN_I64 || sc.kind == PA_ACC_KEYS_I64) v = INT64_MAX;
+    else if (sc.kind == PA_ACC_MAX_I64) v = INT64_MIN;
+    else return false;
+    return true;
+  };
+  const bool fused = q->tune.reset_fused < 0 ? q->acc.n <= kResetFusedMaxBytes : q->tune.reset_fused != 0;
+  if (fused) {
+    ResetArgs a{};
+    a.block = (int64_t*)block;
+    a.block_words = (int64_t)(q->acc.n / 8);
+    if (q->hq.leap_mode) {
+      a.header = (int64_t*)q->leap_buf.p;
+      a.header_words = (int64_t)(leap_header_bytes(q) / 8);
+    }
+    bool fits = true;
+    for (const Section& sc : q->sections) {
+      int64_t v;
+      if (!identity(sc, v)) continue;
+      if (a.num_sections == ResetArgs::kMaxSections) {
+        fits = false;
+        break;
+      }
+      a.sec[a.num_sections].first = ((char*)sc.ptr - block) / 8;
+      a.sec[a.num_sections].n = sc.n;
+      a.sec[a.num_sections].value = v;
+      ++a.num_sections;
+    }
+    if (fits) {
+      PA_HIP(launch_reset(a, st));
+      return PA_OK;
+    }
+  }
+  PA_HIP(hipMemsetAsync(block, 0, q->acc.n, st));
   if (q->hq.leap_mode) PA_HIP(hipMemsetAsync(q->leap_buf.p, 0, leap_header_bytes(q), st));
   for (const Section& sc : q->sections) {
     if (sc.kind == PA_ACC_MIN_I64 || sc.kind == PA_ACC_KEYS_I64) PA_HIP(launch_fill_i64((int64_t*)sc.ptr, sc.n, INT64_MAX, st));
@@ -412,6 +447,8 @@
 int32_t pa_query_num_eager_literals(const pa_query* q) { return q && q->prepared ? q->num_eager : -1; }
 
 int32_t pa_query_lane_major(const pa_query* q) { return q && q->prepared ? q->lane_major : -1; }
+int32_t pa_query_eq_prefilter(const pa_query* q) { return q && q->prepared ? q->eq_prefilter : -1; }
+int32_t pa_query_stream_nt(const pa_query* q) { return q && q->prepared ? q->stream_nt : -1; }
 int32_t pa_query_count_free_emit(const pa_query* q) { return q && q->prepared ? (q->pve.fn ? (q->pvh.fn ? 2 : 1) : 0) : -1; }
 int32_t pa_query_partition_keys(const pa_query* q) {
   if (!q || !q->prepared) return -1;
diff --git a/pinot_amd/csrc/pa_device.h b/pinot_amd/csrc/pa_device.h
--- a/pinot_amd/csrc/pa_device.h
+++ b/pinot_amd/csrc/pa_device.h
@@ -329,7 +329,8 @@
   int32_t num_docs;
   int32_t num_wtiles;
   uint32_t dummy_lo, dummy_hi;
-  int32_t pad0[2];
+  uint32_t flags;
+  int32_t pad0;
   struct {
     uint32_t lo, hi;
     int32_t nbits;
@@ -343,8 +344,12 @@
     int32_t flags;
     uint32_t lut_lo, lut_hi;
   } lf[kLmEager];
-  int32_t pad1[8];
-};
+  uint32_t eq_win_lo, eq_win_hi;
+  int32_t pad1[6];
+};
+constexpr uint32_t kLmEqPrefilter = 1u;
+constexpr uint32_t kLmStreamNt = 2u;
+constexpr int kEqPrefilterMaxNb = 24;
 static_assert(sizeof(LmSegPlan) == 256, "one dword per lane");
 
 __host__ __device__ inline int64_t f64_order_encode(double d) {
diff --git a/pinot_amd/csrc/pa_eq_any.h b/pinot_amd/csrc/pa_eq_any.h
--- /dev/null
+++ b/pinot_amd/csrc/pa_eq_any.h
@@ -0,0 +1,76 @@
+#pragma once
+#include <cstdint>
+
+#if defined(__HIPCC__) || defined(__CUDACC__)
+#define PA_EQ_HD __host__ __device__
+#else
+#define PA_EQ_HD
+#endif
+
+namespace pa {
+
+template <int NB>
+constexpr uint32_t eq_low_bits(int w) {
+  uint32_t m = 0;
+  for (int i = 0; i < 32; ++i) {
+    const int s = (i + 1) * NB - 1;
+    if ((s >> 5) == w) m |= 0x80000000u >> (s & 31);
+  }
+  return m;
+}
+template <int NB>
+constexpr uint32_t eq_high_bits(int w) {
+  uint32_t m = 0;
+  for (int i = 0; i < 32; ++i) {
+    const int s = i * NB;
+    if ((s >> 5) == w) m |= 0x80000000u >> (s & 31);
+  }
+  return m;
+}
+
+PA_EQ_HD inline uint64_t eq_pattern_window(int nb, uint32_t v) {
+  uint64_t w = 0;
+  for (int s = 0; s < 64; s += nb) {
+    const uint64_t f = (uint64_t)v << (64 - nb);
+    w |= f >> s;
+  }
+  return w;
+}
+
+template <int NB>
+PA_EQ_HD inline uint32_t eq_pattern_word(uint64_t window, int j) {
+  return (uint32_t)((window << ((32 * j) % NB)) >> 32);
+}
+
+#if defined(__HIP_DEVICE_COMPILE__)
+typedef uint64_t eq_borrow_t;
+#else
+typedef uint32_t eq_borrow_t;
+#endif
+
+template <int NB, int J, class Get>
+PA_EQ_HD inline void eq_any_word(Get& get, uint64_t window, eq_borrow_t& borrow, uint32_t& any) {
+  constexpr uint32_t L = eq_low_bits<NB>(J), H = eq_high_bits<NB>(J);
+  const uint32_t x = get(J) ^ eq_pattern_word<NB>(window, J);
+  uint32_t d;
+#if defined(__HIP_DEVICE_COMPILE__)
+  asm("v_subb_co_u32_e64 %[d], %[b], %[x], %[l], %[b]" : [d] "=v"(d), [b] "+s"(borrow) : [x] "v"(x), [l] "v"(L));
+#else
+  const uint64_t t = (uint64_t)x - (uint64_t)L - (uint64_t)borrow;
+  d = (uint32_t)t;
+  borrow = (uint32_t)(t >> 32) & 1u;
+#endif
+  any |= d & ~x & H;
+  if constexpr (J > 0) eq_any_word<NB, J - 1>(get, window, borrow, any);
+}
+
+template <int NB, class Get>
+PA_EQ_HD inline uint32_t eq_any(Get get, uint64_t window) {
+  static_assert(NB >= 1 && NB <= 32, "dictionary ids are 1..32 bits");
+  uint32_t any = 0;
+  eq_borrow_t borrow = 0;
+  eq_any_word<NB, NB - 1>(get, window, borrow, any);
+  return any;
+}
+
+}
diff --git a/pinot_amd/csrc/pa_host.h b/pinot_amd/csrc/pa_host.h
--- a/pinot_amd/csrc/pa_host.h
+++ b/pinot_amd/csrc/pa_host.h
@@ -131,6 +131,7 @@
 constexpr uint64_t kMaxHashSlots = uint64_t(1) << 28;
 constexpr uint64_t kWalkMaxBitmapBytes = uint64_t(4) << 30;
 constexpr size_t kLdsBudget = 160 * 1024;
+constexpr size_t kResetFusedMaxBytes = size_t(8) << 20;
 
 struct Section {
   int32_t kind;
@@ -213,6 +214,8 @@
   DevBuf fetch_blocks, fetch_stage;
   void* fetch_host = nullptr;
   int lane_major = 0;
+  int eq_prefilter = 0;
+  int stream_nt = 0;
   int dense_packed = 0;
   hipFunction_t jit_fn = nullptr;
   int jit_waves = 0, jit_grid = 0, jit_lds = 0, jit_nd = 16, jit_nseg = 0, jit_classes = 0, jit_slots = 0;
diff --git a/pinot_amd/csrc/pa_kernels.hip b/pinot_amd/csrc/pa_kernels.hip
--- a/pinot_amd/csrc/pa_kernels.hip
+++ b/pinot_amd/csrc/pa_kernels.hip
@@ -972,6 +972,20 @@
   for (int64_t i = blockIdx.x * (int64_t)blockDim.x + threadIdx.x; i < n; i += (int64_t)gridDim.x * blockDim.x) p[i] = v;
 }
 
+__global__ void __launch_bounds__(256) reset_kernel(ResetArgs a) {
+  const int64_t total = a.block_words + a.header_words;
+  for (int64_t i = blockIdx.x * (int64_t)blockDim.x + threadIdx.x; i < total; i += (int64_t)gridDim.x * blockDim.x) {
+    if (i >= a.block_words) {
+      a.header[i - a.block_words] = 0;
+      continue;
+    }
+    int64_t v = 0;
+    for (int k = 0; k < a.num_sections; ++k)
+      if ((uint64_t)(i - a.sec[k].first) < (uint64_t)a.sec[k].n) v = a.sec[k].value;
+    a.block[i] = v;
+  }
+}
+
 __global__ void gather_kernel(const void* src, int esize, int64_t per, const int64_t* keys, int64_t n, void* out) {
   const int64_t total = n * per;
   for (int64_t i = blockIdx.x * (int64_t)blockDim.x + threadIdx.x; i < total; i += (int64_t)gridDim.x * blockDim.x) {
@@ -1719,6 +1733,11 @@
   return hipGetLastError();
 }
 
+hipError_t launch_reset(const ResetArgs& a, hipStream_t s) {
+  reset_kernel<<<grid_for(a.block_words + a.header_words, 256), 256, 0, s>>>(a);
+  return hipGetLastError();
+}
+
 hipError_t launch_gather(const void* src, int esize, int64_t per, const int64_t* keys, int64_t n, void* out,
                          hipStream_t s) {
   gather_kernel<<<grid_for(n * per, 256), 256, 0, s>>>(src, esize, per, keys, n, out);
diff --git a/pinot_amd/csrc/pa_launch.h b/pinot_amd/csrc/pa_launch.h
--- a/pinot_amd/csrc/pa_launch.h
+++ b/pinot_amd/csrc/pa_launch.h
@@ -79,6 +79,19 @@
                                   uint32_t* lut, hipStream_t s);
 hipError_t launch_hll_lut_hashes(const int32_t* hashes, int32_t card, int32_t log2m, uint32_t* lut, hipStream_t s);
 hipError_t launch_fill_i64(int64_t* p, int64_t n, int64_t v, hipStream_t s);
+struct ResetArgs {
+  static constexpr int kMaxSections = 24;
+  int64_t* block;
+  int64_t block_words;
+  int64_t* header;
+  int64_t header_words;
+  int32_t num_sections;
+  struct {
+    int64_t first, n;
+    int64_t value;
+  } sec[kMaxSections];
+};
+hipError_t launch_reset(const ResetArgs& a, hipStream_t s);
 hipError_t launch_gather(const void* src, int esize, int64_t per, const int64_t* keys, int64_t n, void* out,
                          hipStream_t s);
 hipError_t launch_part_offsets(const DevQuery* hq, const PartScratch& ps, int G, int k, hipStream_t s);
diff --git a/pinot_amd/csrc/pa_plan_kernels.hip b/pinot_amd/csrc/pa_plan_kernels.hip
--- a/pinot_amd/csrc/pa_plan_kernels.hip
+++ b/pinot_amd/csrc/pa_plan_kernels.hip
@@ -1,4 +1,5 @@
 #include "pa_host.h"
+#include "pa_eq_any.h"
 
 
 TilePlan plan_tiles(const pa_query* q, const std::vector<DevSeg>& segs, int strat, bool use_lm, size_t acc_b,
@@ -979,6 +980,12 @@
       PA_HIP(hipMemcpy(q->dsegs_count.p, q->hsegs_count.data(), sizeof(DevSeg) * q->nseg, hipMemcpyHostToDevice));
   }
   q->hplans.assign(std::max(1, q->nseg), LmSegPlan{});
+  const bool std_lm = q->lane_major && !q->partitioned && !q->limit_mode &&
+                      (q->strategy == STRAT_LDS || q->strategy == STRAT_GLOBAL || q->strategy == STRAT_LANE ||
+                       q->strategy == STRAT_LANE_CNT || q->strategy == STRAT_LANE_RAW || q->strategy == STRAT_LANE_DICT);
+  constexpr uint64_t kCacheBytes = (uint64_t(8) * 4 + 256) << 20;
+  q->stream_nt = std_lm && (q->tune.stream_nt < 0 ? q->staged_bytes > kCacheBytes : q->tune.stream_nt != 0) ? 1 : 0;
+  q->eq_prefilter = 0;
   if (q->lane_major) {
     for (int si = 0; si < q->nseg; ++si) {
       const DevSeg& d = q->hsegs[si];
@@ -1008,6 +1015,19 @@
         P.lf[li].lut_lo = (uint32_t)(uintptr_t)L.lut;
         P.lf[li].lut_hi = (uint32_t)((uint64_t)(uintptr_t)L.lut >> 32);
       }
+      if (q->stream_nt) P.flags |= kLmStreamNt;
+      if (std_lm && (q->tune.eq_prefilter < 0 ? q->stream_nt != 0 : q->tune.eq_prefilter != 0) && q->num_eager == 1) {
+        const DevLeaf& L = d.leaves[0];
+        const int nb = L.nbits;
+        if (L.kind == PA_LEAF_DICT_RANGE && !L.negate && L.clause_end && nb >= 1 && nb <= kEqPrefilterMaxNb &&
+            (uint32_t)L.span == (uint32_t)((uint64_t(1) << (32 - nb)) - 1)) {
+          const uint64_t win = eq_pattern_window(nb, (uint32_t)L.lo >> (32 - nb));
+          P.eq_win_lo = (uint32_t)win;
+          P.eq_win_hi = (uint32_t)(win >> 32);
+          P.flags |= kLmEqPrefilter;
+          q->eq_prefilter = 1;
+        }
+      }
     }
   }
   rc = dev_alloc(q->dplans, sizeof(LmSegPlan) * q->hplans.size());
diff --git a/pinot_amd/csrc/pa_scan.h b/pinot_amd/csrc/pa_scan.h
--- a/pinot_amd/csrc/pa_scan.h
+++ b/pinot_amd/csrc/pa_scan.h
@@ -3,6 +3,7 @@
 #include "pa_device.h"
 #include "pa_launch.h"
 #include "pa_keys.h"
+#include "pa_eq_any.h"
 
 namespace pa {
 
@@ -62,35 +63,42 @@
 #define WG_RLX __ATOMIC_RELAXED, __HIP_MEMORY_SCOPE_WORKGROUP
 
 
+#define PA_DMA16_ASM(MOD)                      \
+  "s_mov_b32 %0, m0\n\t"                       \
+  "s_mov_b32 m0, %2\n\t"                       \
+  "s_nop 0\n\t"                                \
+  "global_load_lds_dwordx4 %1, off" MOD "\n\t" \
+  "s_mov_b32 m0, %0"
+#define PA_DMA16_MASKED_ASM(MOD)               \
+  "s_mov_b64 %1, exec\n\t"                     \
+  "s_mov_b64 exec, %4\n\t"                     \
+  "s_mov_b32 %0, m0\n\t"                       \
+  "s_mov_b32 m0, %3\n\t"                       \
+  "s_nop 0\n\t"                                \
+  "global_load_lds_dwordx4 %2, off" MOD "\n\t" \
+  "s_mov_b32 m0, %0\n\t"                       \
+  "s_mov_b64 exec, %1"
+
+template <bool NT = false>
 __device__ __forceinline__ void dma16(const void* src, uint32_t lds_base) {
   uint32_t keep;
   lds_base = (uint32_t)__builtin_amdgcn_readfirstlane((int)lds_base);
-  asm volatile(
-      "s_mov_b32 %0, m0\n\t"
-      "s_mov_b32 m0, %2\n\t"
-      "s_nop 0\n\t"
-      "global_load_lds_dwordx4 %1, off\n\t"
-      "s_mov_b32 m0, %0"
-      : "=&s"(keep)
-      : "v"(src), "s"(lds_base));
-}
-
+  if constexpr (NT) asm volatile(PA_DMA16_ASM(" nt") : "=&s"(keep) : "v"(src), "s"(lds_base));
+  else asm volatile(PA_DMA16_ASM("") : "=&s"(keep) : "v"(src), "s"(lds_base));
+}
+
+template <bool NT = false>
 __device__ __forceinline__ void dma16_masked(const void* src, uint32_t lds_base, uint64_t mask) {
   uint32_t keep;
   uint64_t save;
   lds_base = (uint32_t)__builtin_amdgcn_readfirstlane((int)lds_base);
-  asm volatile(
-      "s_mov_b64 %1, exec\n\t"
-      "s_mov_b64 exec, %4\n\t"
-      "s_mov_b32 %0, m0\n\t"
-      "s_mov_b32 m0, %3\n\t"
-      "s_nop 0\n\t"
-      "global_load_lds_dwordx4 %2, off\n\t"
-      "s_mov_b32 m0, %0\n\t"
-      "s_mov_b64 exec, %1"
-      : "=&s"(keep), "=&s"(save)
-      : "v"(src), "s"(lds_base), "s"(mask));
-}
+  if constexpr (NT)
+    asm volatile(PA_DMA16_MASKED_ASM(" nt") : "=&s"(keep), "=&s"(save) : "v"(src), "s"(lds_base), "s"(mask));
+  else
+    asm volatile(PA_DMA16_MASKED_ASM("") : "=&s"(keep), "=&s"(save) : "v"(src), "s"(lds_base), "s"(mask));
+}
+#undef PA_DMA16_ASM
+#undef PA_DMA16_MASKED_ASM
 
 template <int STEPS>
 __device__ __forceinline__ void stage_tile(const DevSeg* __restrict__ seg, int64_t wt, uint32_t* img, int lane,
@@ -2421,6 +2429,24 @@
   }
 }
 
+__device__ __forceinline__ uint32_t eq_any_lm(int nb, uint32_t region_lds, int lane, uint64_t window) {
+  asm volatile("" : "+s"(window));
+  switch (nb) {
+#define PA_EQ_CASE(N)                                                                                        \
+  case N: {                                                                                                  \
+    const lds_u32_t* p = (const lds_u32_t*)(uintptr_t)(region_lds + (uint32_t)lane * (uint32_t)(N * 4));     \
+    return eq_any<N>([p](int j) -> uint32_t { return p[j]; }, window);                                       \
+  }
+    PA_EQ_CASE(1) PA_EQ_CASE(2) PA_EQ_CASE(3) PA_EQ_CASE(4) PA_EQ_CASE(5) PA_EQ_CASE(6) PA_EQ_CASE(7) PA_EQ_CASE(8)
+    PA_EQ_CASE(9) PA_EQ_CASE(10) PA_EQ_CASE(11) PA_EQ_CASE(12) PA_EQ_CASE(13) PA_EQ_CASE(14) PA_EQ_CASE(15)
+    PA_EQ_CASE(16) PA_EQ_CASE(17) PA_EQ_CASE(18) PA_EQ_CASE(19) PA_EQ_CASE(20) PA_EQ_CASE(21) PA_EQ_CASE(22)
+    PA_EQ_CASE(23) PA_EQ_CASE(24)
+#undef PA_EQ_CASE
+    default: return 1u;
+  }
+}
+static_assert(kEqPrefilterMaxNb == 24, "eq_any_lm compiles the widths 1..kEqPrefilterMaxNb");
+
 __device__ __forceinline__ void stage_tile_lm(uint32_t ip, int64_t wt, uint32_t img_lds, int lane, const int D) {
   const int ns = (int)rl(ip, 0);
   int issued = 0;
@@ -2517,6 +2543,7 @@
   const void* dummy;
 };
 
+template <bool NT = false>
 __device__ __forceinline__ void lm_wait_issue(const LmIssue& I, uint32_t& slot_off, int R, int D, int64_t younger,
                                               uint32_t dst0, int64_t it, uint32_t lane_off) {
   if (R == 2) vm_wait_token<0>(slot_off);
@@ -2527,10 +2554,10 @@
     if (c < I.nst) {
       const char* src = I.base[c] + it * I.stride[c] + lane_off;
       const uint32_t dst = dst0 + I.off[c];
-      for (int k = 0; k < I.nfull[c]; ++k) dma16(src + 1024 * k, dst + 1024 * k);
+      for (int k = 0; k < I.nfull[c]; ++k) dma16<NT>(src + 1024 * k, dst + 1024 * k);
       issued += I.nfull[c];
       if (I.tail[c]) {
-        dma16_masked(src + 1024 * I.nfull[c], dst + 1024 * I.nfull[c], I.tail[c]);
+        dma16_masked<NT>(src + 1024 * I.nfull[c], dst + 1024 * I.nfull[c], I.tail[c]);
         ++issued;
       }
     }
@@ -2685,19 +2712,28 @@
             const uint32_t off0 = 4u * rl(pp, 26), lo0 = rl(pp, 27), hi0 = rl(pp, 28);
             const bool neg0 = (rl(pp, 29) & 1u) != 0;
             const int64_t full_tiles = (int64_t)(int32_t)rl(pp, 2) / kWTileDocs;
+            const uint32_t lmf = rl(pp, 6);
+            const bool eq0 = (lmf & kLmEqPrefilter) != 0, nt = (lmf & kLmStreamNt) != 0;
+            const uint64_t eq_win = ((uint64_t)rl(pp, 57) << 32) | rl(pp, 56);
             while (t < seg_end && ti < issue_end) {
               uint32_t slot_off = (uint32_t)(pslot * img_dw);
-              lm_wait_issue(I, slot_off, R, D, ti - (t + 1), ring_lds + 4u * (uint32_t)(islot * img_dw), ti - ifirst,
-                            16u * (uint32_t)lane);
+              if (nt)
+                lm_wait_issue<true>(I, slot_off, R, D, ti - (t + 1), ring_lds + 4u * (uint32_t)(islot * img_dw),
+                                    ti - ifirst, 16u * (uint32_t)lane);
+              else
+                lm_wait_issue(I, slot_off, R, D, ti - (t + 1), ring_lds + 4u * (uint32_t)(islot * img_dw), ti - ifirst,
+                              16u * (uint32_t)lane);
               ++ti;
               islot = islot + 1 == R ? 0 : islot + 1;
               if (t - seg_first < full_tiles) {
-                uint32_t m = leaf_lm_any(nb0, PA_LEAF_DICT_RANGE, ring_lds + 4u * slot_off + off0, lane, lo0, hi0,
-                                         nullptr);
-                if (neg0) m = ~m;
-                if (__ballot(m != 0) != 0)
-                  matched += tile_survivors<STRAT, 32, 1>(q, seg, ring + slot_off, (t - seg_first) * kWTileDocs, m,
-                                                          lane, acc.lds, *acc.ps, la);
+                if (!eq0 || __ballot(eq_any_lm(nb0, ring_lds + 4u * slot_off + off0, lane, eq_win) != 0) != 0) {
+                  uint32_t m = leaf_lm_any(nb0, PA_LEAF_DICT_RANGE, ring_lds + 4u * slot_off + off0, lane, lo0, hi0,
+                                           nullptr);
+                  if (neg0) m = ~m;
+                  if (__ballot(m != 0) != 0)
+                    matched += tile_survivors<STRAT, 32, 1>(q, seg, ring + slot_off, (t - seg_first) * kWTileDocs, m,
+                                                            lane, acc.lds, *acc.ps, la);
+                }
               } else {
                 process_tile_lm<STRAT>(q, seg, pp, t - seg_first, ring + slot_off, ring_lds + 4u * slot_off, lane, acc,
                                        matched, la);
@@ -2706,10 +2742,15 @@
               ++t;
             }
           } else {
+            const bool nt = (rl(pp, 6) & kLmStreamNt) != 0;
             while (t < seg_end && ti < issue_end) {
               uint32_t slot_off = (uint32_t)(pslot * img_dw);
-              lm_wait_issue(I, slot_off, R, D, ti - (t + 1), ring_lds + 4u * (uint32_t)(islot * img_dw), ti - ifirst,
-                            16u * (uint32_t)lane);
+              if (nt)
+                lm_wait_issue<true>(I, slot_off, R, D, ti - (t + 1), ring_lds + 4u * (uint32_t)(islot * img_dw),
+                                    ti - ifirst, 16u * (uint32_t)lane);
+              else
+                lm_wait_issue(I, slot_off, R, D, ti - (t + 1), ring_lds + 4u * (uint32_t)(islot * img_dw), ti - ifirst,
+                              16u * (uint32_t)lane);
               ++ti;
               islot = islot + 1 == R ? 0 : islot + 1;
               process_tile_lm<STRAT>(q, seg, pp, t - seg_first, ring + slot_off, ring_lds + 4u * slot_off, lane, acc,
diff --git a/pinot_amd/csrc/pa_tuning.h b/pinot_amd/csrc/pa_tuning.h
--- a/pinot_amd/csrc/pa_tuning.h
+++ b/pinot_amd/csrc/pa_tuning.h
@@ -32,7 +32,15 @@
                                                                       \
   X(walk_tab, 1, 0, 1, 0)                                                                                              \
                \
-  X(debug_emit, 0, 0, 127, 1)
+  X(debug_emit, 0, 0, 127, 1)                                                                                          \
+                                \
+  X(eq_prefilter, -1, 0, 1, 0)                                                                                         \
+                                                                                            \
+  X(stream_nt, -1, 0, 1, 0)                                                                                            \
+        \
+  X(scan_grid, -1, 1, 4096, 0)                                                                                         \
+                                                                    \
+  X(reset_fused, -1, 0, 1, 0)
 
 struct Tuning {
 #define X(name, def, lo, hi, inv) int32_t name = def;
diff --git a/pinot_amd/engine.py b/pinot_amd/engine.py
--- a/pinot_amd/engine.py
+++ b/pinot_amd/engine.py
@@ -513,6 +513,8 @@
         out["plan"]["lane_major"] = int(L.lib().pa_query_lane_major(self.handle))
         out["plan"]["dense_packed"] = int(L.lib().pa_query_dense_packed(self.handle))
         out["plan"]["count_free_emit"] = int(L.lib().pa_query_count_free_emit(self.handle))
+        out["plan"]["eq_prefilter"] = int(L.lib().pa_query_eq_prefilter(self.handle))
+        out["plan"]["stream_nt"] = int(L.lib().pa_query_stream_nt(self.handle))
         out["plan"]["partition_keys"] = int(L.lib().pa_query_partition_keys(self.handle))
         out["plan"]["limit_trimming"] = int(L.lib().pa_query_limit_trimming(self.handle))
         out["plan"]["results_invalid"] = int(L.lib().pa_query_results_invalid(self.handle))
```
